# bd4sur/Nano

Hardware: AMD Instinct MI355X
Metric: decode_tokens_per_sec (higher is better)
Workload: dtype i8

## Files before the change

include/nano_mi355x.h:

```cpp
#ifndef NANO_MI355X_H
#define NANO_MI355X_H

#include <stddef.h>
#include <stdint.h>

#ifdef __cplusplus
extern "C" {
#endif

#define NANO_ARCH_NANO  0u
#define NANO_ARCH_QWEN2 2u
#define NANO_ARCH_QWEN3 3u

#define NANO_QUANT_F32 0x00u
#define NANO_QUANT_Q80 0x80u
#define NANO_QUANT_Q4K 0x42u

#define NANO_HIP_OK        0
#define NANO_HIP_EINVAL   -1
#define NANO_HIP_ERUNTIME -2
#define NANO_HIP_ENODEV   -3
#define NANO_HIP_ENOMEM   -4

#define NANO_MAX_BATCH 64u
// ... 117 lines not shown
    uint32_t chunk;
    uint32_t want_frag;
    uint32_t pool_rows;
    uint32_t pt_stride;
    const float *q;
    const float *k;
    const float *vraw;
    const uint32_t *pos;
    const float *q_norm, *k_norm;
    const float *rope_cos, *rope_sin;
    const uint32_t *pt_rows;
    void *k_cache, *v_cache;
    float *out;
    int8_t *xf;
    float *xsf;
    uint32_t *plan;
} NanoAttnDecodeDesc;
int nano_hip_op_attention_decode(int device, const NanoAttnDecodeDesc *d);
int nano_hip_op_swiglu(int device, float *hb, const float *hb2, uint32_t n);
int nano_hip_op_exact_rmsnorm(int device, float *out, const float *x, const float *w, uint32_t n);
typedef struct NanoExactAttnDesc {
    uint32_t n_head, n_kv_head, hd, S;
    uint32_t range;
    uint32_t is_causal;
    uint32_t long_form;
    uint32_t _pad;
    const float *q;
    const float *k_cache, *v_cache;
    float *out;
} NanoExactAttnDesc;
int nano_hip_op_exact_attention(int device, const NanoExactAttnDesc *d);

int nano_hip_op_argmax(int device, const float *x, uint32_t n, uint32_t *idx);

typedef struct NanoFusedGemvDesc {
    uint32_t quant;
    uint32_t gs;
    uint32_t kind;
    uint32_t n, nb, nseg;
    uint32_t rows[3];
    const void *w[3];
    const float *ws[3];
    const float *x;
    const float *norm_w;
    const float *attn_part;
    const float *attn_ml;
    uint32_t attn_nsplit, attn_n_head, attn_hd;
    uint32_t use_gemm;
    uint32_t ordered;
    uint32_t *route_out;
    float *out;
} NanoFusedGemvDesc;
int nano_hip_op_fused_gemv(int device, const NanoFusedGemvDesc *d);

typedef struct NanoBlobShare NanoBlobShare;
int nano_hip_blob_share(NanoBlobShare **out, const void *host_params, size_t bytes, int root_device, const int *devices, int n_devices);
const void *nano_hip_blob_ptr(const NanoBlobShare *s, int i);
void nano_hip_blob_stats(const NanoBlobShare *s, double *upload_s, double *share_s, char *how, size_t how_cap);
void nano_hip_blob_done(NanoBlobShare *s, int i);
void nano_hip_blob_release(NanoBlobShare *s);
int nano_hip_model_device(const NanoHipModel *m);

int nano_hip_stamps_begin(NanoHipModel *m);
int nano_hip_stamps_read(NanoHipModel *m, unsigned long long *out, uint32_t *kinds, uint32_t cap_launches, uint32_t *n_launches);

#ifdef __cplusplus
}
#endif
#endif
```

nano_amd/binding.py:

```python
from __future__ import annotations

import ctypes as C
import os
from typing import Optional, Sequence

import numpy as np

HERE = os.path.dirname(os.path.abspath(__file__))
LIB_PATH = os.environ.get("NANO_LIB") or os.path.join(HERE, "lib", "libnano_mi355x.so")

f32p = np.ctypeslib.ndpointer(dtype=np.float32, flags="C_CONTIGUOUS")
i8p = np.ctypeslib.ndpointer(dtype=np.int8, flags="C_CONTIGUOUS")
u8p = np.ctypeslib.ndpointer(dtype=np.uint8, flags="C_CONTIGUOUS")
u32p = np.ctypeslib.ndpointer(dtype=np.uint32, flags="C_CONTIGUOUS")


class NanoModelDesc(C.Structure):
    _fields_ = [(n, C.c_uint32) for n in (
        "arch", "block_size", "vocab_size", "n_layer", "n_embd", "n_head", "n_kv_head", "n_hidden",
        "is_shared_classifier", "head_dim", "quant_type", "group_size")]


class NanoFusedGemvDesc(C.Structure):
    _fields_ = [("quant", C.c_uint32), ("gs", C.c_uint32), ("kind", C.c_uint32), ("n", C.c_uint32), ("nb", C.c_uint32), ("nseg", C.c_uint32),
# ... 365 lines not shown
    q = np.empty(x.size, np.int8); s = np.empty(x.size // gs, np.float32)
    check(lib().nano_hip_op_quantize_q80(device, x, x.size, gs, q, s)); return q, s


def op_matmul_q80(xq, xs, wq, ws, n, d, gs, device=0):
    out = np.empty(d, np.float32)
    check(lib().nano_hip_op_matmul_q80(device, out, np.ascontiguousarray(xq), np.ascontiguousarray(xs),
                                       np.ascontiguousarray(wq), np.ascontiguousarray(ws), n, d, gs)); return out


def op_quantize_q4k(x, device=0):
    x = np.ascontiguousarray(x, np.float32)
    out = np.zeros(((x.size + 255) // 256) * 160, np.uint8)
    check(lib().nano_hip_op_quantize_q4k(device, x, x.size, out)); return out


def op_matmul_q4k(x_blocks, w_blocks, n, d, device=0):
    out = np.empty(d, np.float32)
    check(lib().nano_hip_op_matmul_q4k(device, out, np.ascontiguousarray(x_blocks), np.ascontiguousarray(w_blocks), n, d)); return out


def op_fused_gemv(quant, kind, n, weights, x=None, norm_w=None, *, gs=0, nb=1, resid=None, attn=None, use_gemm=False, ordered=False,
                  want_route=False, device=0):
    d = NanoFusedGemvDesc()
    d.quant, d.gs, d.kind, d.n, d.nb, d.nseg = quant, gs, kind, n, nb, len(weights)
    keep = []
    for i, (w, ws, rows) in enumerate(weights):
        w = np.ascontiguousarray(w); keep.append(w)
        d.rows[i] = rows; d.w[i] = w.ctypes.data
        if ws is not None:
            ws = np.ascontiguousarray(ws, np.float32); keep.append(ws); d.ws[i] = ws.ctypes.data
    rows_total = weights[0][2] if kind == 2 else sum(r for _, _, r in weights)
    if x is not None:
        x = np.ascontiguousarray(x, np.float32); keep.append(x); d.x = x.ctypes.data
    if norm_w is not None:
        norm_w = np.ascontiguousarray(norm_w, np.float32); keep.append(norm_w); d.norm_w = norm_w.ctypes.data
    if attn is not None:
        part, ml, n_head, hd = attn
        part = np.ascontiguousarray(part, np.float32); ml = np.ascontiguousarray(ml, np.float32); keep += [part, ml]
        d.attn_part, d.attn_ml = part.ctypes.data, ml.ctypes.data
        d.attn_nsplit, d.attn_n_head, d.attn_hd = part.shape[-2], n_head, hd
    out = np.zeros((nb, rows_total), np.float32) if resid is None else np.array(resid, np.float32, copy=True).reshape(nb, rows_total)
    d.use_gemm = 1 if use_gemm else 0
    d.ordered = 1 if ordered else 0
    route = C.c_uint32(0xffffffff)
    d.route_out = C.cast(C.pointer(route), C.c_void_p)
    d.out = out.ctypes.data
    check(lib().nano_hip_op_fused_gemv(device, C.byref(d)))
    if want_route:
        return out, (ROUTE_NAMES[route.value] if route.value < len(ROUTE_NAMES) else "?")
    return out


def op_attention_decode(q, k, pos, k_cache, v_cache, *, n_head, n_kv_head, hd, n_layer, layer, S, range_hint, rope_cos, rope_sin,
                        rope_qwen3, q_norm=None, k_norm=None, vraw=None, kv_half=False, chunk=False, nsplit=0, want_frag=False,
                        pt_rows=None, pool_rows=0, device=0):
    d = NanoAttnDecodeDesc()
    q = np.ascontiguousarray(q, np.float32); k = np.ascontiguousarray(k, np.float32); pos = np.ascontiguousarray(pos, np.uint32)
    nb_ = q.shape[0]
    cdt = np.float16 if kv_half else np.float32
    kc = np.array(k_cache, cdt, copy=True, order="C"); vc = np.array(v_cache, cdt, copy=True, order="C")
    rope_cos = np.ascontiguousarray(rope_cos, np.float32); rope_sin = np.ascontiguousarray(rope_sin, np.float32)
    out = np.zeros((nb_, n_head * hd), np.float32)
    plan = np.zeros((2, len(ATTN_PLAN_FIELDS)), np.uint32)
    keep = [q, k, pos, kc, vc, rope_cos, rope_sin, out, plan]
    d.nb, d.n_head, d.n_kv_head, d.hd, d.n_layer, d.layer, d.S = nb_, n_head, n_kv_head, hd, n_layer, layer, S
    d.range_hint, d.nsplit, d.rope_qwen3, d.kv_half, d.chunk, d.want_frag = range_hint, nsplit, int(rope_qwen3), int(kv_half), int(chunk), int(want_frag)
    d.q, d.k, d.pos, d.k_cache, d.v_cache, d.out, d.plan = (x.ctypes.data for x in (q, k, pos, kc, vc, out, plan))
    d.rope_cos, d.rope_sin = rope_cos.ctypes.data, rope_sin.ctypes.data
    if q_norm is not None:
        q_norm = np.ascontiguousarray(q_norm, np.float32); k_norm = np.ascontiguousarray(k_norm, np.float32); keep += [q_norm, k_norm]
        d.q_norm, d.k_norm = q_norm.ctypes.data, k_norm.ctypes.data
    if vraw is not None:
        vraw = np.ascontiguousarray(vraw, np.float32); keep.append(vraw); d.vraw = vraw.ctypes.data
    if pt_rows is not None:
        pt_rows = np.ascontiguousarray(pt_rows, np.uint32); keep.append(pt_rows)
        d.pt_rows, d.pt_stride, d.pool_rows = pt_rows.ctypes.data, pt_rows.shape[-1], pool_rows
    xf = xsf = None
    if want_frag:
        tiles, ng = (nb_ + 15) // 16, n_head * hd // 64
        xf = np.zeros((tiles, ng, 1024), np.int8); xsf = np.zeros((tiles, ng, 16), np.float32); keep += [xf, xsf]
        d.xf, d.xsf = xf.ctypes.data, xsf.ctypes.data
    check(lib().nano_hip_op_attention_decode(device, C.byref(d)))
    plans = [dict(zip(ATTN_PLAN_FIELDS, (int(v) for v in row))) for row in plan]
    res = {"out": out, "k_cache": kc, "v_cache": vc, "plan": plans if chunk else plans[0]}
    if want_frag:
        res["xf"], res["xsf"] = xf, xsf
    return res


def op_rope(head, fcr, fci, qwen3, device=0):
    h = np.array(head, np.float32, copy=True)
    check(lib().nano_hip_op_rope(device, h, h.size, np.ascontiguousarray(fcr, np.float32), np.ascontiguousarray(fci, np.float32), int(qwen3))); return h


def op_attention(q, k_cache, v_cache, n_head, n_kv_head, head_dim, device=0):
    rng = k_cache.shape[0]
    out = np.empty(n_head * head_dim, np.float32)
    check(lib().nano_hip_op_attention(device, out, np.ascontiguousarray(q, np.float32), np.ascontiguousarray(k_cache, np.float32),
                                      np.ascontiguousarray(v_cache, np.float32), n_head, n_kv_head, head_dim, rng)); return out


def op_exact_rmsnorm(x, w, device=0):
    x = np.ascontiguousarray(x, np.float32); w = np.ascontiguousarray(w, np.float32)
    out = np.empty_like(x)
    check(lib().nano_hip_op_exact_rmsnorm(device, out, x, w, x.size)); return out
# ... 132 lines not shown
```

nano_amd/csrc/gemv_common.h:

```cpp
#pragma once
#define NANO_GEMV_COMMON_H 1
#include <stdlib.h>
#include "device_common.h"
#include "kernels.h"

namespace nano {

namespace {

#define DPP_I(v, ctrl) __builtin_amdgcn_update_dpp(0, (v), (ctrl), 0xF, 0xF, true)
#define DPP_F(v, ctrl) __int_as_float(__builtin_amdgcn_update_dpp(0, __float_as_int(v), (ctrl), 0xF, 0xF, true))

template <int W> __device__ __forceinline__ int dpp_group_sum(int v) {
    if (W >= 2) v += DPP_I(v, 0xB1);
    if (W >= 4) v += DPP_I(v, 0x4E);
    if (W >= 8) v += DPP_I(v, 0x141);
    if (W >= 16) v += DPP_I(v, 0x140);
    return v;
}
template <int W> __device__ __forceinline__ float dpp_group_max(float v) {
    if (W >= 2) v = fmaxf(v, DPP_F(v, 0xB1));
    if (W >= 4) v = fmaxf(v, DPP_F(v, 0x4E));
    if (W >= 8) v = fmaxf(v, DPP_F(v, 0x141));
    if (W >= 16) v = fmaxf(v, DPP_F(v, 0x140));
    if (W >= 32) v = fmaxf(v, __shfl_xor(v, 16, 64));
    if (W >= 64) v = fmaxf(v, __shfl_xor(v, 32, 64));
    return v;
}
__device__ __forceinline__ float dpp_wave_sum(float v) {
    v += DPP_F(v, 0xB1); v += DPP_F(v, 0x4E); v += DPP_F(v, 0x141); v += DPP_F(v, 0x140);
    const float r0 = __int_as_float(__builtin_amdgcn_readlane(__float_as_int(v), 0));
    const float r1 = __int_as_float(__builtin_amdgcn_readlane(__float_as_int(v), 16));
    const float r2 = __int_as_float(__builtin_amdgcn_readlane(__float_as_int(v), 32));
    const float r3 = __int_as_float(__builtin_amdgcn_readlane(__float_as_int(v), 48));
    return (r0 + r1) + (r2 + r3);
}

typedef int i32x4 __attribute__((ext_vector_type(4)));
constexpr uint32_t OOB = 0x7ffffff0u;
__device__ __forceinline__ __amdgpu_buffer_rsrc_t mkrsrc(const void *p, uint32_t bytes) {
    return __builtin_amdgcn_make_buffer_rsrc(const_cast<void *>(p), 0, (int)bytes, 0x00020000);
}
__device__ __forceinline__ int4 bload_w(__amdgpu_buffer_rsrc_t r, uint32_t off) {
    const i32x4 v = __builtin_amdgcn_raw_buffer_load_b128(r, (int)off, 0, 2);
    return make_int4(v.x, v.y, v.z, v.w);
}
__device__ __forceinline__ float4 bload_f4(__amdgpu_buffer_rsrc_t r, uint32_t off) {
    const i32x4 v = __builtin_amdgcn_raw_buffer_load_b128(r, (int)off, 0, 0);
    return make_float4(__int_as_float(v.x), __int_as_float(v.y), __int_as_float(v.z), __int_as_float(v.w));
}
__device__ __forceinline__ float bload_f(__amdgpu_buffer_rsrc_t r, uint32_t off) {
    return __uint_as_float(__builtin_amdgcn_raw_buffer_load_b32(r, (int)off, 0, 0));
}

enum : uint32_t { F_NORM = 1u, F_PRE = 2u, F_COMBINE = 4u };

enum : int { R_GENERIC = 0, R_NORM_STORE = 1, R_RESID = 2, R_RESID_COMBINE = 3, R_NORM_SWIGLU = 4 };
struct GemvDev;
template <int ROLE> __device__ __forceinline__ bool has_flag(const GemvDev &a, uint32_t f);
template <int ROLE> __device__ __forceinline__ uint32_t role_epi(const GemvDev &a);

struct GemvDev {
    const int8_t *w[3]; const float *ws[3]; float *out[3];
    uint32_t rows[3], out_bstride[3], out_pstride[3];
    uint32_t n, ng, rw, log2_tiles, nchunk, magic_nchunk, units, epi, flags, nb;
    uint32_t tpw, magic_rw, wg_c0, wg_c1;
    const float *xin; const float *norm_w; const uint32_t *pos;
    uint32_t xin_bstride, nthr;
    const int8_t *xq_in; const float *xs_in;
    const float *attn_part; const float *attn_ml;
    uint32_t attn_nsplit, attn_n_head, attn_hd, ntiles;
    float *tile_max;
    const float *resid_add; uint32_t resid_add_bstride;
    uint32_t early;
    unsigned long long *stamps;
    uint32_t dbg;
    uint32_t canon;
    uint32_t *err;
};

template <int ROLE> __device__ __forceinline__ bool has_flag(const GemvDev &a, uint32_t f) {
    if (ROLE == R_GENERIC) return (a.flags & f) != 0;
    if (f == F_NORM) return ROLE == R_NORM_STORE || ROLE == R_NORM_SWIGLU;
    if (f == F_COMBINE) return ROLE == R_RESID_COMBINE;
    return false;
}
template <int ROLE> __device__ __forceinline__ uint32_t role_epi(const GemvDev &a) {
    if (ROLE == R_GENERIC) return a.epi;
    if (ROLE == R_NORM_STORE) return GEMV_EPI_STORE;
    if (ROLE == R_NORM_SWIGLU) return GEMV_EPI_SWIGLU;
    return GEMV_EPI_RESID;
}

template <int B, int NV>
struct Staged {
    float4 x[B][NV];
    float4 nw[NV];
    float4 pv[B == 1 ? NV : 1][B == 1 ? 8 : 1];
    float ml_m, ml_l;
};
template <int B>
struct Staged<B, 0> {};

template <int ROLE, int B, int NV>
__device__ __forceinline__ void stage_issue(const GemvDev &a, Staged<B, NV> &r) {
    if constexpr (NV == 0) { (void)a; (void)r; return; } else {
    const uint32_t tid = threadIdx.x, nthr = a.nthr, n = a.n;
    const bool plain = !has_flag<ROLE>(a, F_PRE) && !has_flag<ROLE>(a, F_COMBINE);
    const __amdgpu_buffer_rsrc_t rx = mkrsrc(a.xin, plain ? ((a.nb - 1) * a.xin_bstride + n) * 4u : 0u);
    const __amdgpu_buffer_rsrc_t rn = mkrsrc(a.norm_w, has_flag<ROLE>(a, F_NORM) ? n * 4u : 0u);
#pragma unroll
    for (int j = 0; j < NV; j++) {
        const uint32_t i = (tid + (uint32_t)j * nthr) * 4u;
        const uint32_t off = (i < n) ? i * 4u : OOB;
        if (plain) {
#pragma unroll
            for (int b = 0; b < B; b++) r.x[b][j] = bload_f4(rx, (b < (int)a.nb) ? off + (uint32_t)b * a.xin_bstride * 4u : OOB);
        }
        if (has_flag<ROLE>(a, F_NORM)) r.nw[j] = (NANO_STAMPS && (a.dbg & 1u)) ? make_float4(1.f, 1.f, 1.f, 1.f) : bload_f4(rn, off);
    }
    if constexpr (B == 1) {
      if (has_flag<ROLE>(a, F_COMBINE)) {
        const uint32_t ns = a.attn_nsplit, nh = a.attn_n_head;
        const __amdgpu_buffer_rsrc_t rp = mkrsrc(a.attn_part, ns * n * 4u);
        const __amdgpu_buffer_rsrc_t rm = mkrsrc(a.attn_ml, nh * ns * 8u);
#pragma unroll
        for (int j = 0; j < NV; j++) {
            const uint32_t i = (tid + (uint32_t)j * nthr) * 4u;
#pragma unroll
            for (int sp = 0; sp < 8; sp++) r.pv[j][sp] = bload_f4(rp, (i < n && (uint32_t)sp < ns) ? ((uint32_t)sp * n + i) * 4u : OOB);
        }
        const uint32_t sp = tid & 7u, h = tid >> 3;
        const uint32_t mo = (h < nh && sp < ns) ? (h * ns + sp) * 8u : OOB;
        r.ml_m = bload_f(rm, mo);
        r.ml_l = bload_f(rm, mo == OOB ? OOB : mo + 4u);
      }
    }
    }
}

template <int ROLE, int B, int NV>
__device__ __forceinline__ void stage_issue_nw(const GemvDev &a, Staged<B, NV> &r) {
    if constexpr (NV == 0) { (void)a; (void)r; return; } else {
    const uint32_t tid = threadIdx.x, nthr = a.nthr, n = a.n;
    const __amdgpu_buffer_rsrc_t rn = mkrsrc(a.norm_w, has_flag<ROLE>(a, F_NORM) ? n * 4u : 0u);
#pragma unroll
    for (int j = 0; j < NV; j++) {
        const uint32_t i = (tid + (uint32_t)j * nthr) * 4u;
        if (has_flag<ROLE>(a, F_NORM)) r.nw[j] = bload_f4(rn, (i < n) ? i * 4u : OOB);
    }
    }
}

template <int B, bool PRE>
__device__ __forceinline__ void combine_weights(const GemvDev &a, float *wgt , float pm, float pl) {
    const uint32_t tid = threadIdx.x, nthr = a.nthr;
    const uint32_t ns = a.attn_nsplit, nh = a.attn_n_head;
    for (uint32_t t = tid; t < (uint32_t)B * nh * 8u; t += nthr) {
        const uint32_t s = t & 7u, h = (t >> 3) % nh, b = (t >> 3) / nh;
        float m = -INFINITY, l = 0.0f;
        if constexpr (PRE) { m = pm; l = pl; (void)s; (void)h; (void)b; (void)ns; }
        else if (s < ns && b < a.nb) { const float *ml = a.attn_ml + (((size_t)b * nh + h) * ns + s) * 2; m = ml[0]; l = ml[1]; }
        const bool live = l > 0.0f;
        float M = live ? m : -INFINITY;
        M = fmaxf(M, DPP_F(M, 0xB1)); M = fmaxf(M, DPP_F(M, 0x4E)); M = fmaxf(M, DPP_F(M, 0x141));
        const float e = live ? expf(m - M) : 0.0f;
        float L = l * e;
        L += DPP_F(L, 0xB1); L += DPP_F(L, 0x4E); L += DPP_F(L, 0x141);
        wgt[t] = e / L;
        if constexpr (PRE) break;
    }
    __syncthreads();
}
__device__ __forceinline__ float4 combine4(const GemvDev &a, uint32_t b, uint32_t i, const float *wgt) {
    const uint32_t ns = a.attn_nsplit, n = a.n;
    const float *part = a.attn_part + (size_t)b * ns * n + i;
    const float *wg = wgt + ((size_t)b * a.attn_n_head + i / a.attn_hd) * 8u;
    float4 o[8];
#pragma unroll
    for (int s = 0; s < 8; s++) o[s] = ((uint32_t)s < ns) ? *reinterpret_cast<const float4 *>(part + (size_t)s * n) : make_float4(0.f, 0.f, 0.f, 0.f);
    float4 acc = make_float4(0.f, 0.f, 0.f, 0.f);
#pragma unroll
    for (int s = 0; s < 8; s++) {
        const float w = wg[s];
        acc.x += o[s].x * w; acc.y += o[s].y * w; acc.z += o[s].z * w; acc.w += o[s].w * w;
    }
    return acc;
}

__device__ __forceinline__ float finish_epi(uint32_t epi, float v0, float v1, float old) {
    if (epi == GEMV_EPI_STORE) return v0;
    if (epi == GEMV_EPI_RESID) return old + v0;
    float h = v0;
    h *= (1.0f / (1.0f + expf(-h)));
    h *= v1;
    return h;
}

static GemvDev to_dev(const GemvArgs &a) {
    GemvDev d{};
    for (int i = 0; i < 3; i++) {
        const bool live = i < (int)a.nseg;
        d.w[i] = live ? reinterpret_cast<const int8_t *>(a.seg[i].w) : nullptr;
        d.ws[i] = live ? a.seg[i].ws : nullptr;
        d.out[i] = live ? a.seg[i].out : nullptr;
        d.rows[i] = live ? a.seg[i].rows : 0;
        d.out_bstride[i] = live ? a.seg[i].out_bstride : 0;
        d.out_pstride[i] = live ? a.seg[i].out_pstride : 0;
    }
    if (a.epi == GEMV_EPI_SWIGLU) { d.rows[1] = 0; d.rows[2] = 0; }
    d.n = a.n; d.ng = a.gs ? a.n / a.gs : 0;
    d.nchunk = (a.n + 1023) / 1024;
    d.magic_nchunk = (65536 + d.nchunk - 1) / d.nchunk;
    d.epi = a.epi; d.nb = a.nb;
    d.flags = (a.norm_w ? F_NORM : 0) | (a.xq_in ? F_PRE : 0) | (a.attn_part ? F_COMBINE : 0);
    d.xin = a.xin; d.norm_w = a.norm_w; d.pos = a.pos; d.xin_bstride = a.xin_bstride;
    d.xq_in = a.xq_in; d.xs_in = a.xs_in;
    d.attn_part = a.attn_part; d.attn_ml = a.attn_ml; d.attn_nsplit = a.attn_nsplit; d.attn_n_head = a.attn_n_head; d.attn_hd = a.attn_hd;
    d.tile_max = a.tile_max;
    d.resid_add = a.resid_add; d.resid_add_bstride = a.resid_add_bstride;
    d.stamps = a.stamps;
    d.canon = q80_canonical(a) ? 1u : 0u;
    d.err = a.err;
#if NANO_STAMPS
    { static const uint32_t dbg = getenv("NANO_DBG") ? (uint32_t)strtoul(getenv("NANO_DBG"), nullptr, 0) : 0u; d.dbg = dbg; }
#endif
    return d;
}

}

}
```

nano_amd/csrc/gemv_f32.hip:

```cpp
#include "gemv_common.h"

namespace nano {

namespace {

template <int ROLE, int B, int NV>
__device__ __forceinline__ void stage_finish_f32(const GemvDev &a, Staged<B, NV> &r, float *xf, float *red, uint32_t n4) {
    const uint32_t tid = threadIdx.x, nthr = a.nthr, n = a.n;
    const uint32_t lane = tid & 63u, wid = tid >> 6, NW = nthr >> 6;
    const bool norm = has_flag<ROLE>(a, F_NORM), comb = has_flag<ROLE>(a, F_COMBINE);
    float *wgt = red + B * 16;
    if constexpr (NV == 0) {
        if (comb) combine_weights<B, false>(a, wgt, 0.0f, 0.0f);
        for (uint32_t b = 0; b < a.nb; b++) {
            const float *x = a.xin + (size_t)b * a.xin_bstride;
            float ss = 1.0f;
            if (norm) {
                float acc = 0.0f;
                for (uint32_t i = tid * 4u; i < n; i += nthr * 4u) {
                    const float4 v = comb ? combine4(a, b, i, wgt) : *reinterpret_cast<const float4 *>(x + i);
                    acc += v.x * v.x; acc += v.y * v.y; acc += v.z * v.z; acc += v.w * v.w;
                }
                acc = dpp_wave_sum(acc);
                __syncthreads();
                if (lane == 0) red[wid] = acc;
                __syncthreads();
                float t = 0.0f;
                for (uint32_t w = 0; w < NW; w++) t += red[w];
                t /= (float)n; t += 1e-5f;
                ss = 1.0f / sqrtf(t);
            }
            for (uint32_t i = tid * 4u; i < n; i += nthr * 4u) {
                float4 v = comb ? combine4(a, b, i, wgt) : *reinterpret_cast<const float4 *>(x + i);
                if (norm) {
                    const float4 w = *reinterpret_cast<const float4 *>(a.norm_w + i);
                    v.x = w.x * (ss * v.x); v.y = w.y * (ss * v.y); v.z = w.z * (ss * v.z); v.w = w.w * (ss * v.w);
                }
                *reinterpret_cast<float4 *>(xf + b * n4 + i) = v;
            }
        }
        __syncthreads();
    } else {
        if (comb) {
            if constexpr (B == 1) {
                const bool pre_ml = a.attn_n_head * 8u <= nthr;
                if (pre_ml) combine_weights<B, true>(a, wgt, r.ml_m, r.ml_l); else combine_weights<B, false>(a, wgt, 0.0f, 0.0f);
#pragma unroll
                for (int j = 0; j < NV; j++) {
                    const uint32_t i = (tid + (uint32_t)j * nthr) * 4u;
                    const float *wg = wgt + (size_t)((i < n ? i : 0u) / a.attn_hd) * 8u;
                    float4 acc = make_float4(0.f, 0.f, 0.f, 0.f);
#pragma unroll
                    for (int sp = 0; sp < 8; sp++) {
                        const float w = wg[sp];
                        acc.x += r.pv[j][sp].x * w; acc.y += r.pv[j][sp].y * w; acc.z += r.pv[j][sp].z * w; acc.w += r.pv[j][sp].w * w;
                    }
                    r.x[0][j] = acc;
                }
            } else {
                combine_weights<B, false>(a, wgt, 0.0f, 0.0f);
#pragma unroll
                for (int b = 0; b < B; b++)
#pragma unroll
                    for (int j = 0; j < NV; j++) {
                        const uint32_t i = (tid + (uint32_t)j * nthr) * 4u;
                        r.x[b][j] = (i < n && b < (int)a.nb) ? combine4(a, b, i, wgt) : make_float4(0.f, 0.f, 0.f, 0.f);
                    }
            }
        }
        float ss[B];
#pragma unroll
        for (int b = 0; b < B; b++) ss[b] = 1.0f;
        if (norm) {
#pragma unroll
            for (int b = 0; b < B; b++) {
                float acc = 0.0f;
#pragma unroll
                for (int j = 0; j < NV; j++) {
                    acc += r.x[b][j].x * r.x[b][j].x; acc += r.x[b][j].y * r.x[b][j].y;
                    acc += r.x[b][j].z * r.x[b][j].z; acc += r.x[b][j].w * r.x[b][j].w;
                }
                acc = dpp_wave_sum(acc);
                if (lane == 0) red[b * 16 + wid] = acc;
            }
            __syncthreads();
#pragma unroll
            for (int b = 0; b < B; b++) {
                float t = 0.0f;
                for (uint32_t w = 0; w < NW; w++) t += red[b * 16 + w];
                t /= (float)n; t += 1e-5f;
                ss[b] = 1.0f / sqrtf(t);
            }
        }
#pragma unroll
        for (int j = 0; j < NV; j++) {
            const uint32_t i = (tid + (uint32_t)j * nthr) * 4u;
#pragma unroll
            for (int b = 0; b < B; b++) {
                float4 v = r.x[b][j];
                if (norm) {
                    v.x = r.nw[j].x * (ss[b] * v.x); v.y = r.nw[j].y * (ss[b] * v.y);
                    v.z = r.nw[j].z * (ss[b] * v.z); v.w = r.nw[j].w * (ss[b] * v.w);
                }
                if (i < n) *reinterpret_cast<float4 *>(xf + b * n4 + i) = v;
            }
        }
        __syncthreads();
    }
}

__device__ __forceinline__ float4 bload_wf(__amdgpu_buffer_rsrc_t r, uint32_t off) {
    const i32x4 v = __builtin_amdgcn_raw_buffer_load_b128(r, (int)off, 0, 2);
    return make_float4(__int_as_float(v.x), __int_as_float(v.y), __int_as_float(v.z), __int_as_float(v.w));
}

template <int ROLE, int B, int NV, int UPW>
__global__ __launch_bounds__(1024) void gemv_f32_slab_kernel(const GemvDev a) {
    extern __shared__ __attribute__((aligned(16))) unsigned char smem[];
#define F32_A a
// ... 55 lines not shown
    if (want > 16) want = 16;
    if (nw < want) nw = want;
    if (nw * 64 < rw * (uint32_t)B) nw = (rw * (uint32_t)B + 63) / 64;
    if (nw < 2) nw = 2;
    uint32_t upw = (units + nw - 1) / nw;
    while (upw > 4 && nw < 16) { nw++; upw = (units + nw - 1) / nw; }
    return F32Plan{rw, nw, upw, (a.n + 256 * nw - 1) / (256 * nw)};
}

template <int ROLE, int B, int NV, int UPW>
static hipError_t launch_f32_t(const GemvDev &d, const F32Plan &p, uint32_t rows, hipStream_t st) {
    const uint32_t nmat = d.epi == GEMV_EPI_SWIGLU ? 2 : 1;
    const size_t n4 = (d.n + 3) & ~3u, pc = (d.nchunk + 3) & ~3u;
    const size_t lds = (B * n4 + B * 16 + ((d.flags & F_COMBINE) ? (size_t)B * d.attn_n_head * 8 : 0) + (size_t)B * nmat * p.rw * pc) * 4;
    auto kern = &gemv_f32_slab_kernel<ROLE, B, NV, UPW>;
    if (lds > 64 * 1024) (void)hipFuncSetAttribute(reinterpret_cast<const void *>(kern), hipFuncAttributeMaxDynamicSharedMemorySize, (int)lds);
    GemvDev dd = d; dd.nthr = 64 * p.nw;
    hipLaunchKernelGGL(kern, dim3((rows + p.rw - 1) / p.rw), dim3(64 * p.nw), lds, st, dd);
    return hipGetLastError();
}
template <int ROLE, int B>
static hipError_t launch_f32_r(const GemvDev &d, const F32Plan &p, uint32_t rows, hipStream_t st) {
    if (p.upw > 4) return hipErrorInvalidValue;
#define F32_GO(NV_, UPW_) do { if constexpr (B * NV_ <= 8) return launch_f32_t<ROLE, B, NV_, UPW_>(d, p, rows, st); } while (0)
    int nv = p.nv <= 1 ? 1 : p.nv <= 2 ? 2 : p.nv <= 4 ? 4 : 0;
    const int upw = p.upw <= 1 ? 1 : p.upw <= 2 ? 2 : 4;
    if (B * nv > 8) nv = 0;
    if (nv == 1) { if (upw == 1) F32_GO(1, 1); if (upw == 2) F32_GO(1, 2); F32_GO(1, 4); }
    if (nv == 2) { if (upw == 1) F32_GO(2, 1); if (upw == 2) F32_GO(2, 2); F32_GO(2, 4); }
    if (nv == 4) { if (upw == 1) F32_GO(4, 1); if (upw == 2) F32_GO(4, 2); F32_GO(4, 4); }
    if (upw == 1) F32_GO(0, 1);
    if (upw == 2) F32_GO(0, 2);
    F32_GO(0, 4);
    return hipErrorInvalidValue;
#undef F32_GO
}
template <int B>
static hipError_t launch_f32_b(const GemvArgs &a, hipStream_t st) {
    GemvDev d = to_dev(a);
    d.tile_max = nullptr;
    const F32Plan p = plan_f32(a, B);
    d.nchunk = (a.n + 255) / 256;
    d.magic_nchunk = (65536 + d.nchunk - 1) / d.nchunk;
    d.rw = p.rw;
    uint32_t l2 = 0; while ((1u << l2) < p.rw / 4) l2++;
    d.log2_tiles = l2;
    d.units = (p.rw / 4) * d.nchunk * (d.epi == GEMV_EPI_SWIGLU ? 2 : 1);
    uint32_t rows = 0;
    if (a.epi == GEMV_EPI_SWIGLU) rows = a.seg[0].rows; else for (uint32_t s = 0; s < a.nseg; s++) rows += a.seg[s].rows;
    if constexpr (B == 1) {
        const uint32_t f = d.flags;
        if (f == F_NORM && d.epi == GEMV_EPI_STORE) return launch_f32_r<R_NORM_STORE, B>(d, p, rows, st);
        if (f == 0 && d.epi == GEMV_EPI_RESID) return launch_f32_r<R_RESID, B>(d, p, rows, st);
        if (f == F_COMBINE && d.epi == GEMV_EPI_RESID) return launch_f32_r<R_RESID_COMBINE, B>(d, p, rows, st);
        if (f == F_NORM && d.epi == GEMV_EPI_SWIGLU) return launch_f32_r<R_NORM_SWIGLU, B>(d, p, rows, st);
    }
    return launch_f32_r<R_GENERIC, B>(d, p, rows, st);
}

static bool f32_fused_shape(const GemvArgs &ga, const AttnArgs &aa, F32Plan &p) {
    if (ga.nb != 1 || ga.nseg != 3 || ga.epi != GEMV_EPI_STORE || !ga.norm_w || ga.xq_in || ga.attn_part || ga.tile_max || ga.resid_add || ga.n % 4u) return false;
    if (ga.seg[0].out_pstride || ga.seg[1].out_pstride) return false;
    for (uint32_t s2 = 0; s2 < 3; s2++) if (ga.seg[s2].rows % 4u) return false;
    p = plan_f32(ga, 1);
    if (p.nw > 4u || p.upw > 4u || ga.n > 1024u) return false;
    p.nw = 4u; p.nv = 1u;
    const uint32_t units = (p.rw / 4) * ((ga.n + 255) / 256);
    p.upw = (units + 3u) / 4u;
    if (p.upw > 4u) return false;
    return fused_attn_side_ok_plain(aa, ga.seg[0].rows, ga.seg[1].rows, ga.seg[2].rows);
}

}

bool qkv_attn_fused_f32_supports(const GemvArgs &ga, const AttnArgs &aa) { F32Plan p; return f32_fused_shape(ga, aa, p); }

hipError_t launch_qkv_attn_fused_f32(const GemvArgs &ga, const AttnArgs &aa, unsigned long long *hand, uint32_t *tick, uint32_t layer1, hipStream_t st) {
    F32Plan p;
    if (!hand || !tick || !layer1 || layer1 > 127u || !f32_fused_shape(ga, aa, p)) return hipErrorInvalidValue;
    GemvDev d = to_dev(ga);
    d.tile_max = nullptr;
    d.nchunk = (ga.n + 255) / 256;
    d.magic_nchunk = (65536 + d.nchunk - 1) / d.nchunk;
    d.rw = p.rw;
    uint32_t l2 = 0; while ((1u << l2) < p.rw / 4) l2++;
    d.log2_tiles = l2;
    d.units = (p.rw / 4) * d.nchunk;
    d.nthr = 256;
    uint32_t rows = 0;
    for (uint32_t s2 = 0; s2 < 3; s2++) rows += ga.seg[s2].rows;
    const uint32_t ngemv = (rows + p.rw - 1) / p.rw;
    AttnArgs a = aa;
    { uint32_t k2 = 0; while ((1u << k2) < a.n_kv_head) k2++; a.kv_log2 = k2; }
    { const uint32_t kv_mul = a.n_head / a.n_kv_head; uint32_t k2 = 0; while ((1u << k2) < kv_mul) k2++; a.kvmul_log2 = k2; }
    SlabHand h{};
    h.buf = hand; h.tick = tick; h.layer1 = layer1;
    h.base[0] = 0; h.base[1] = a.q_dim; h.base[2] = a.q_dim + a.kv_dim;
    const size_t n4 = (d.n + 3) & ~3u, pc = (d.nchunk + 3) & ~3u;
    const size_t lds_g = (n4 + 16 + (size_t)p.rw * pc) * 4;
    const size_t hd4 = (a.hd + 3) & ~3u, lds_a = (hd4 + hd4 + 4 + 4 + 4 * hd4 + hd4) * sizeof(float);
    const size_t lds = lds_g > lds_a ? lds_g : lds_a;
    if (lds > 64 * 1024) return hipErrorInvalidValue;
    F32FusedArgs fa{};
    fa.g = d; fa.a = a; fa.hand = h; fa.n_attn = a.n_head * a.nsplit; fa.head_wgs = a.n_head; fa.ngemv = ngemv;
    fa.wait16 = 1u;
    const int upw = p.upw <= 1 ? 1 : p.upw <= 2 ? 2 : 4;
#define F32F_GO(UPW_) do { if (a.hd <= 32u) hipLaunchKernelGGL((f32_qkv_attn_fused_kernel<1, UPW_, 1>), dim3(fa.n_attn + ngemv), dim3(256), lds, st, fa); \
// ... 20 lines not shown
```

nano_amd/csrc/gemv_q4k.hip:

```cpp
#include <float.h>

#include "gemv_q4k_impl.h"

namespace nano {

__global__ __launch_bounds__(256) void quantize_q4k_kernel(const float *x, uint32_t n, uint8_t *blocks) {
    __shared__ float tmp[16];
    __shared__ uint8_t nibs[256];
    const int t = threadIdx.x;
    const uint32_t bpl = (n + 255) / 256;
    for (uint32_t j = 0; j < bpl; j++) {
        const uint32_t d = (n >= (j + 1) * 256) ? 256 : (n - j * 256);
        const bool valid = (uint32_t)t < d;
        const float v = valid ? x[(size_t)j * d + t] : 0.0f;
        Q4kBlockHdr hdr; float sq, bq;
        const uint32_t nib = q4k_quantize_block_coop(v, valid, tmp, hdr, sq, bq);
        nibs[t] = (uint8_t)nib;
        __syncthreads();
        uint8_t *blk = blocks + (size_t)j * 160;
        if (t < 128) blk[32 + t] = (uint8_t)((nibs[2 * t] & 0x0f) | (nibs[2 * t + 1] << 4));
        if (t == 0) {
            uint32_t *w = reinterpret_cast<uint32_t *>(blk);
            w[0] = 0x42u; w[1] = d; w[2] = 0u;
            w[3] = __float_as_uint(hdr.s_scale); w[4] = __float_as_uint(hdr.s_bias);
// ... 211 lines not shown
    if (lds > 64 * 1024) (void)hipFuncSetAttribute(reinterpret_cast<const void *>(kern), hipFuncAttributeMaxDynamicSharedMemorySize, (int)lds);
    GemvDev dd = d; dd.nthr = p.nthr;
    { const uint32_t GT = ((d.n + 255) / 256) * 8; dd.magic_nchunk = (uint32_t)(((1ull << 32) + GT - 1) / GT); dd.log2_tiles = 0; while ((1u << dd.log2_tiles) < p.rw) dd.log2_tiles++;
      dd.units = ((p.rw * GT) % 64u == 0u && p.nthr % 64u == 0u) ? 1u : 0u; }
    hipLaunchKernelGGL(kern, dim3((rows + p.rw - 1) / p.rw), dim3(p.nthr), lds, st, dd);
    return hipGetLastError();
}
template <int ROLE, int B>
static hipError_t launch_q4k_r(const GemvDev &d, const Q4kPlan &p, uint32_t rows, hipStream_t st) {
    if (p.ipt > 4) return hipErrorInvalidValue;
#define Q4K_GO(NV_, IPT_) do { if constexpr (B * NV_ <= 8) return launch_q4k_t<ROLE, B, NV_, IPT_>(d, p, rows, st); } while (0)
    int nv = p.nv <= 1 ? 1 : p.nv <= 2 ? 2 : p.nv <= 4 ? 4 : 0;
    const int ipt = p.ipt <= 1 ? 1 : p.ipt <= 2 ? 2 : 4;
    if (B * nv > 8) nv = 0;
    if (nv == 1) { if (ipt == 1) Q4K_GO(1, 1); if (ipt == 2) Q4K_GO(1, 2); Q4K_GO(1, 4); }
    if (nv == 2) { if (ipt == 1) Q4K_GO(2, 1); if (ipt == 2) Q4K_GO(2, 2); Q4K_GO(2, 4); }
    if (nv == 4) { if (ipt == 1) Q4K_GO(4, 1); if (ipt == 2) Q4K_GO(4, 2); Q4K_GO(4, 4); }
    if (ipt == 1) Q4K_GO(0, 1);
    if (ipt == 2) Q4K_GO(0, 2);
    Q4K_GO(0, 4);
    return hipErrorInvalidValue;
#undef Q4K_GO
}
}
bool gemv_q4k_chunk_takes(const GemvArgs &a) {
    if (a.nb <= 1) return gemv_q4k_chunk_supports(a);
    if (a.nb > 8 || !gemv_q4k_chunk_supports(a)) return false;
    return a.nb >= 5u || route_is_wide(a) || gemv_q4k_fit_batch(a) < a.nb;
}

uint32_t gemv_q4k_partials(const GemvArgs &a) {
    if (a.nb == 1 && gemv_q4k_chunk_supports(a)) return gemv_q4k_chunk_partials(a);
    if (a.nb > 1 && gemv_q4k_chunk_takes(a)) return 0;
    if (!a.tile_max || a.epi != GEMV_EPI_STORE || a.nseg != 1 || a.nb == 0 || a.nb > 8 || a.seg[0].out_pstride) return 0;
    const int B = a.nb <= 1 ? 1 : a.nb <= 2 ? 2 : a.nb <= 4 ? 4 : 8;
    const Q4kPlan p = plan_q4k(a, B);
    return (a.seg[0].rows + p.rw - 1) / p.rw;
}
namespace {
template <int B>
static hipError_t launch_q4k_b(const GemvArgs &a, hipStream_t st) {
    GemvDev d = to_dev(a);
    if (a.x4_in) { d.flags |= F_PRE; d.xq_in = reinterpret_cast<const int8_t *>(a.x4_in); }
    const Q4kPlan p = plan_q4k(a, B);
    d.rw = p.rw;
    uint32_t rows = 0;
    if (a.epi == GEMV_EPI_SWIGLU) rows = a.seg[0].rows; else for (uint32_t s = 0; s < a.nseg; s++) rows += a.seg[s].rows;
    d.ntiles = gemv_q4k_partials(a);
    if (!d.ntiles || d.ntiles != (rows + p.rw - 1) / p.rw) { d.tile_max = nullptr; d.ntiles = 0; }
    if constexpr (B == 1) {
        const uint32_t f = d.flags;
        if (f == F_NORM && d.epi == GEMV_EPI_STORE) return launch_q4k_r<R_NORM_STORE, B>(d, p, rows, st);
        if (f == 0 && d.epi == GEMV_EPI_RESID) return launch_q4k_r<R_RESID, B>(d, p, rows, st);
        if (f == F_COMBINE && d.epi == GEMV_EPI_RESID) return launch_q4k_r<R_RESID_COMBINE, B>(d, p, rows, st);
        const uint32_t GT = ((d.n + 255) / 256) * 8;
        if (f == F_NORM && d.epi == GEMV_EPI_SWIGLU && (p.rw * GT) % 64u == 0u && p.nthr % 64u == 0u) return launch_q4k_r<R_NORM_SWIGLU, B>(d, p, rows, st);
    }
    return launch_q4k_r<R_GENERIC, B>(d, p, rows, st);
}

}

uint32_t gemv_q4k_fit_batch(const GemvArgs &a) {
    for (uint32_t c = 8; c > 1; c >>= 1)
        if (q4k_lds_bytes(a.n, a.epi, a.attn_part != nullptr, a.attn_n_head, plan_q4k(a, (int)c).rw, c) <= 160 * 1024) return c;
    return 1;
}

hipError_t launch_gemv_q4k(GemvArgs &a, uint32_t max_wg, hipStream_t st) {
    (void)max_wg;
    if (a.nb >= 1 && a.nb <= 8 && gemv_q4k_chunk_takes(a)) return launch_gemv_q4k_chunk(a, st);
    if (a.nb == 0 || a.nb > 8 || a.n % 4 || a.nseg == 0 || a.nseg > 3) return hipErrorInvalidValue;
    if (a.attn_part && (a.norm_w || a.attn_nsplit > 8 || a.attn_hd % 4)) return hipErrorInvalidValue;
    if (a.epi != GEMV_EPI_SWIGLU && a.nseg > 1)
        for (uint32_t s = 0; s < a.nseg; s++) if (a.seg[s].rows % 4) return hipErrorInvalidValue;
    if (a.nb <= 1) return launch_q4k_b<1>(a, st);
    if (a.nb <= 2) return launch_q4k_b<2>(a, st);
    if (a.nb <= 4) return launch_q4k_b<4>(a, st);
    return launch_q4k_b<8>(a, st);
}

}
```

nano_amd/csrc/gemv_q4k_chunk.hip:

```cpp
#include "gemv_q4k_impl.h"
#include <hip/hip_ext.h>

namespace nano {

extern hipEvent_t g_q80_probe_start, g_q80_probe_stop;

namespace {

template <int ROLE, int NV, int D, bool LOOP, int NB = 1>
__global__ __launch_bounds__(1024) void gemv_q4k_chunk_kernel(const GemvDev a) {
    static_assert(NB == 1 || (ROLE == R_GENERIC && NV == 1), "several sequences: activations arrive quantized (q4k_quant_rows_kernel), generic role");
    extern __shared__ __attribute__((aligned(16))) unsigned char smem[];
#define CHUNK_A a
#define CHUNK_BID blockIdx.x
#define CHUNK_HAND 0
#define CHUNK_HANDV (SlabHand{})
#define CHUNK_PTAG 0u
#include "gemv_q4k_chunk_body.inc"
#undef CHUNK_A
#undef CHUNK_BID
#undef CHUNK_HAND
#undef CHUNK_HANDV
#undef CHUNK_PTAG
}
// ... 108 lines not shown
}

template <int ROLE, int NV, int D, bool LOOP>
hipError_t launch_chunk_t(const GemvDev &d, const ChunkPlan &p, hipStream_t st) {
    auto kern = &gemv_q4k_chunk_kernel<ROLE, NV, D, LOOP>;
    if (p.lds > 64 * 1024) (void)hipFuncSetAttribute(reinterpret_cast<const void *>(kern), hipFuncAttributeMaxDynamicSharedMemorySize, (int)p.lds);
    hipEvent_t e0 = LOOP ? g_q80_probe_start : nullptr, e1 = LOOP ? g_q80_probe_stop : nullptr;
    if (e0 && e1) {
        g_q80_probe_start = g_q80_probe_stop = nullptr;
        hipExtLaunchKernelGGL(kern, dim3(p.grid), dim3(p.nthr), (uint32_t)p.lds, st, e0, e1, 0, d);
    } else hipLaunchKernelGGL(kern, dim3(p.grid), dim3(p.nthr), p.lds, st, d);
    return hipGetLastError();
}
template <int ROLE, int NV>
hipError_t launch_chunk_d(const GemvDev &d, const ChunkPlan &p, hipStream_t st) {
    if (p.loop) return launch_chunk_t<ROLE, NV, 8, true>(d, p, st);
    if (p.d == 1) return launch_chunk_t<ROLE, NV, 1, false>(d, p, st);
    if (p.d == 2) return launch_chunk_t<ROLE, NV, 2, false>(d, p, st);
    if (p.d == 4) return launch_chunk_t<ROLE, NV, 4, false>(d, p, st);
    return launch_chunk_t<ROLE, NV, 8, false>(d, p, st);
}
template <int ROLE>
hipError_t launch_chunk_r(const GemvDev &d, const ChunkPlan &p, hipStream_t st) {
    if (p.nv <= 1) return launch_chunk_d<ROLE, 1>(d, p, st);
    if (p.nv <= 2) return launch_chunk_d<ROLE, 2>(d, p, st);
    return launch_chunk_d<ROLE, 4>(d, p, st);
}
template <int D, bool LOOP, int NB>
hipError_t launch_chunk_nb_t(const GemvDev &d, const ChunkPlan &p, hipStream_t st) {
    auto kern = &gemv_q4k_chunk_kernel<R_GENERIC, 1, D, LOOP, NB>;
    if (p.lds > 64 * 1024) (void)hipFuncSetAttribute(reinterpret_cast<const void *>(kern), hipFuncAttributeMaxDynamicSharedMemorySize, (int)p.lds);
    hipLaunchKernelGGL(kern, dim3(p.grid), dim3(p.nthr), p.lds, st, d);
    return hipGetLastError();
}
template <int NB>
hipError_t launch_chunk_nb(const GemvDev &d, const ChunkPlan &p, hipStream_t st) {
    if (p.loop) return launch_chunk_nb_t<8, true, NB>(d, p, st);
    if (p.d == 1) return launch_chunk_nb_t<1, false, NB>(d, p, st);
    if (p.d == 2) return launch_chunk_nb_t<2, false, NB>(d, p, st);
    if (p.d == 4) return launch_chunk_nb_t<4, false, NB>(d, p, st);
    return launch_chunk_nb_t<8, false, NB>(d, p, st);
}
template <int ROLE, int NV>
hipError_t launch_quant_rows_t(const GemvDev &d, XGroup *out, uint32_t nb, size_t lds, hipStream_t st) {
    auto kern = &q4k_quant_rows_kernel<ROLE, NV>;
    if (lds > 64 * 1024) (void)hipFuncSetAttribute(reinterpret_cast<const void *>(kern), hipFuncAttributeMaxDynamicSharedMemorySize, (int)lds);
    hipLaunchKernelGGL(kern, dim3(nb), dim3(d.nthr), lds, st, d, out);
    return hipGetLastError();
}
template <int NV>
hipError_t launch_quant_rows_r(const GemvDev &d, XGroup *out, uint32_t nb, size_t lds, hipStream_t st) {
    if (d.flags == F_NORM) return launch_quant_rows_t<R_NORM_STORE, NV>(d, out, nb, lds, st);
    if (d.flags == 0) return launch_quant_rows_t<R_RESID, NV>(d, out, nb, lds, st);
    if (d.flags == F_COMBINE) return launch_quant_rows_t<R_RESID_COMBINE, NV>(d, out, nb, lds, st);
    return launch_quant_rows_t<R_GENERIC, NV>(d, out, nb, lds, st);
}

}

bool gemv_q4k_chunk_supports(const GemvArgs &a) {
    ChunkPlan p;
    if (a.nb <= 1) return plan_chunk(a, p);
    GemvArgs one = a; one.nb = 1;
    return a.q4_scratch && (size_t)a.nb * (a.n >> 5) * sizeof(XGroup) <= a.q4_scratch_bytes && plan_chunk(one, p) && plan_chunk(a, p);
}
bool gemv_q4k_chunk_loops(const GemvArgs &a) { ChunkPlan p; return a.nb == 1 && plan_chunk(a, p) && p.loop; }
uint32_t gemv_q4k_chunk_partials(const GemvArgs &a) {
    ChunkPlan p;
    if (a.nb != 1 || !a.tile_max || a.epi != GEMV_EPI_STORE || a.nseg != 1 || a.seg[0].out_pstride || !plan_chunk(a, p)) return 0;
    return p.grid;
}

static hipError_t launch_gemv_q4k_chunk_batched(GemvArgs &a, hipStream_t st) {
    if (!gemv_q4k_chunk_supports(a)) return hipErrorInvalidValue;
    ChunkPlan p1, p;
    GemvArgs one = a; one.nb = 1;
    if (!plan_chunk(one, p1) || !plan_chunk(a, p)) return hipErrorInvalidValue;
    const uint32_t bpl = a.n >> 8, GT = bpl * 8u;
    XGroup *xg = reinterpret_cast<XGroup *>(a.q4_scratch);
    {
        GemvDev q = to_dev(a);
        q.nthr = p1.nthr; q.tile_max = nullptr;
        const size_t lds = (size_t)GT * sizeof(XGroup) + (16 + (a.attn_part ? (size_t)a.attn_n_head * 8 : 0)) * 4 + 16;
        const hipError_t e = p1.nv <= 1 ? launch_quant_rows_r<1>(q, xg, a.nb, lds, st) : p1.nv <= 2 ? launch_quant_rows_r<2>(q, xg, a.nb, lds, st) : launch_quant_rows_r<4>(q, xg, a.nb, lds, st);
        if (e != hipSuccess) return e;
    }
    GemvArgs g = a;
    g.norm_w = nullptr; g.attn_part = nullptr; g.attn_ml = nullptr; g.tile_max = nullptr;
    GemvDev d = to_dev(g);
    d.flags = F_PRE; d.xq_in = reinterpret_cast<const int8_t *>(xg);
    d.rw = p.rw; d.nthr = p.nthr; d.units = p.rounds;
    d.magic_nchunk = (uint32_t)(((1ull << 32) + bpl - 1) / bpl);
    const uint32_t nseg = a.epi == GEMV_EPI_SWIGLU ? 1u : a.nseg;
    d.wg_c0 = nseg > 1 ? p.wg[0] : 0xffffffffu;
    d.wg_c1 = nseg > 2 ? p.wg[0] + p.wg[1] : 0xffffffffu;
    d.ntiles = 0;
    if (a.nb <= 2) return launch_chunk_nb<2>(d, p, st);
    if (a.nb <= 4) return launch_chunk_nb<4>(d, p, st);
    return launch_chunk_nb<8>(d, p, st);
}

static bool q4k_fused_shape(const GemvArgs &ga, const AttnArgs &aa, ChunkPlan &p) {
    if (ga.nb != 1 || ga.nseg != 3 || ga.epi != GEMV_EPI_STORE || !ga.norm_w || ga.xq_in || ga.x4_in || ga.attn_part || ga.tile_max || ga.resid_add) return false;
    if (ga.seg[0].out_pstride || ga.seg[1].out_pstride) return false;
    if (ga.n > 1024u || !plan_chunk(ga, p, 4u) || p.loop || p.nthr != 256u || p.nv != 1u) return false;
    if (p.lds > 64u * 1024u) return false;
    return fused_attn_side_ok(aa, ga.seg[0].rows, ga.seg[1].rows, ga.seg[2].rows);
}
bool qkv_attn_fused_q4k_supports(const GemvArgs &ga, const AttnArgs &aa) { ChunkPlan p; return q4k_fused_shape(ga, aa, p); }

hipError_t launch_qkv_attn_fused_q4k(const GemvArgs &ga, const AttnArgs &aa, unsigned long long *hand, uint32_t *tick, uint32_t layer1, hipStream_t st) {
    ChunkPlan p;
    if (!hand || !tick || !layer1 || layer1 > 127u || !q4k_fused_shape(ga, aa, p)) return hipErrorInvalidValue;
    GemvDev d = to_dev(ga);
    d.tile_max = nullptr; d.ntiles = 0;
    const uint32_t bpl = ga.n >> 8;
    d.rw = p.rw; d.nthr = p.nthr; d.units = p.rounds;
    d.magic_nchunk = (uint32_t)(((1ull << 32) + bpl - 1) / bpl);
    d.wg_c0 = p.wg[0]; d.wg_c1 = p.wg[0] + p.wg[1];
    AttnArgs a = aa;
    { uint32_t l2 = 0; while ((1u << l2) < a.n_kv_head) l2++; a.kv_log2 = l2; }
    { const uint32_t kv_mul = a.n_head / a.n_kv_head; uint32_t l2 = 0; while ((1u << l2) < kv_mul) l2++; a.kvmul_log2 = l2; }
    SlabHand h{};
    h.buf = hand; h.tick = tick; h.layer1 = layer1;
    h.base[0] = 0; h.base[1] = a.q_dim; h.base[2] = a.q_dim + a.kv_dim;
    const size_t hd4 = a.hd, lds_a = (hd4 + hd4 + 4 + 4 + 4 * hd4 + hd4 + 4 + 4 * 8 * hd4) * sizeof(float);
    const size_t lds = p.lds > lds_a ? p.lds : lds_a;
    Q4FusedArgs fa{};
    fa.g = d; fa.a = a; fa.hand = h; fa.n_attn = a.n_head * a.nsplit; fa.head_wgs = a.n_head; fa.ngemv = p.grid;
    fa.wait16 = 0u;
#define Q4F_GO(NV_, D_) do { hipLaunchKernelGGL((q4k_qkv_attn_fused_kernel<NV_, D_>), dim3(fa.n_attn + fa.ngemv), dim3(p.nthr), lds, st, fa); return hipGetLastError(); } while (0)
#define Q4F_NV(NV_) do { if (p.d == 1) Q4F_GO(NV_, 1); if (p.d == 2) Q4F_GO(NV_, 2); if (p.d == 4) Q4F_GO(NV_, 4); Q4F_GO(NV_, 8); } while (0)
    if (p.nv <= 1) Q4F_NV(1);
    if (p.nv <= 2) Q4F_NV(2);
    Q4F_NV(4);
#undef Q4F_NV
#undef Q4F_GO
}

hipError_t launch_gemv_q4k_chunk(GemvArgs &a, hipStream_t st) {
    if (a.nb > 1) return launch_gemv_q4k_chunk_batched(a, st);
    ChunkPlan p;
    if (!plan_chunk(a, p)) return hipErrorInvalidValue;
    GemvDev d = to_dev(a);
    if (a.x4_in) { d.flags |= F_PRE; d.xq_in = reinterpret_cast<const int8_t *>(a.x4_in); }
    const uint32_t bpl = a.n >> 8;
    d.rw = p.rw; d.nthr = p.nthr; d.units = p.rounds;
    d.magic_nchunk = (uint32_t)(((1ull << 32) + bpl - 1) / bpl);
    const uint32_t nseg = a.epi == GEMV_EPI_SWIGLU ? 1u : a.nseg;
    d.wg_c0 = nseg > 1 ? p.wg[0] : 0xffffffffu;
    d.wg_c1 = nseg > 2 ? p.wg[0] + p.wg[1] : 0xffffffffu;
    d.ntiles = gemv_q4k_chunk_partials(a);
    if (!d.ntiles) d.tile_max = nullptr;
    const uint32_t f = d.flags;
    if (f == F_NORM && d.epi == GEMV_EPI_STORE) return launch_chunk_r<R_NORM_STORE>(d, p, st);
    if (f == 0 && d.epi == GEMV_EPI_RESID) return launch_chunk_r<R_RESID>(d, p, st);
    if (f == F_COMBINE && d.epi == GEMV_EPI_RESID) return launch_chunk_r<R_RESID_COMBINE>(d, p, st);
    if (f == F_NORM && d.epi == GEMV_EPI_SWIGLU) return launch_chunk_r<R_NORM_SWIGLU>(d, p, st);
    return launch_chunk_r<R_GENERIC>(d, p, st);
}

}
```

nano_amd/csrc/gemv_q4k_impl.h:

```cpp
#pragma once
#include <float.h>

#include "gemv_common.h"

namespace nano {

typedef unsigned int u32x2_q __attribute__((ext_vector_type(2)));

struct XGroup {
    uint32_t pk[4];
    float sq, bq;
    int sumq;
    int _pad;
};

struct Q4kBlockHdr { float s_scale, s_bias; uint32_t sb[3]; };

__device__ __forceinline__ uint32_t q4k_quantize_block_coop(float v, bool valid, float *tmp ,
                                                            Q4kBlockHdr &hdr, float &sq_f, float &bq_f) {
    const int t = threadIdx.x, g = t >> 5;
    float lo = valid ? v : FLT_MAX;
    float hi = valid ? v : FLT_TRUE_MIN;
    lo = (lo < FLT_MAX) ? lo : FLT_MAX;
    hi = (hi > FLT_TRUE_MIN) ? hi : FLT_TRUE_MIN;
    for (int o = 16; o > 0; o >>= 1) {
        lo = fminf(lo, __shfl_xor(lo, o, 64));
        hi = fmaxf(hi, __shfl_xor(hi, o, 64));
    }
    const float gsc = (lo <= 0.0f) ? div_const<15>(hi - lo) : div_const<15>(hi);
    const float gbi = (lo <= 0.0f) ? (-lo) : 0.0f;
    uint32_t nib = 0;
    if (valid && gsc != 0.0f) nib = (uint32_t)(nearest_int_magic((v + gbi) / gsc) & 0x0f);
    __syncthreads();
    if ((t & 31) == 0) { tmp[g] = gsc; tmp[8 + g] = gbi; }
    __syncthreads();
    float smax = FLT_TRUE_MIN, bmax = FLT_TRUE_MIN;
#pragma unroll
    for (int k = 0; k < 8; k++) { if (tmp[k] > smax) smax = tmp[k]; if (tmp[8 + k] > bmax) bmax = tmp[8 + k]; }
    const float s_scale = div_const<63>(smax), s_bias = div_const<63>(bmax);
    uint32_t s6[8], b6[8];
#pragma unroll
    for (int k = 0; k < 8; k++) {
        s6[k] = (s_scale == 0.0f) ? 0u : (uint32_t)(nearest_int_magic(tmp[k] / s_scale) & 0x3f);
        b6[k] = (s_bias == 0.0f) ? 0u : (uint32_t)(nearest_int_magic(tmp[8 + k] / s_bias) & 0x3f);
    }
    hdr.s_scale = s_scale; hdr.s_bias = s_bias;
    hdr.sb[0] = hdr.sb[1] = hdr.sb[2] = 0;
#pragma unroll
    for (int i = 0; i < 4; i++) {
        hdr.sb[0] |= ((((s6[4 + i] & 0x30) << 2) | (s6[i] & 0x3f)) & 0xffu) << (8 * i);
        hdr.sb[1] |= ((((b6[4 + i] & 0x30) << 2) | (b6[i] & 0x3f)) & 0xffu) << (8 * i);
        hdr.sb[2] |= ((((b6[4 + i] & 0x0f) << 4) | (s6[4 + i] & 0x0f)) & 0xffu) << (8 * i);
    }
    sq_f = (float)s6[g] * s_scale;
    bq_f = (float)b6[g] * s_bias;
    return nib;
}

namespace {

template <int ROLE, int B, int NV>
__device__ __forceinline__ void stage_xn(const GemvDev &a, Staged<B, NV> &r, float *xn, float *red, uint32_t n4, bool keep) {
    const uint32_t tid = threadIdx.x, nthr = a.nthr, n = a.n;
    const uint32_t lane = tid & 63u, wid = tid >> 6, NW = nthr >> 6;
    const bool norm = has_flag<ROLE>(a, F_NORM), comb = has_flag<ROLE>(a, F_COMBINE);
    float *wgt = red + B * 16;
    if constexpr (NV == 0) {
        if (comb) combine_weights<B, false>(a, wgt, 0.0f, 0.0f);
        for (uint32_t b = 0; b < a.nb; b++) {
            const float *x = a.xin + (size_t)b * a.xin_bstride;
            float ss = 1.0f;
            if (norm) {
                float acc = 0.0f;
                for (uint32_t i = tid * 4u; i < n; i += nthr * 4u) {
                    const float4 v = comb ? combine4(a, b, i, wgt) : *reinterpret_cast<const float4 *>(x + i);
                    acc += v.x * v.x; acc += v.y * v.y; acc += v.z * v.z; acc += v.w * v.w;
                }
                acc = dpp_wave_sum(acc);
                __syncthreads();
                if (lane == 0) red[wid] = acc;
                __syncthreads();
                float t = 0.0f;
                for (uint32_t w = 0; w < NW; w++) t += red[w];
                t /= (float)n; t += 1e-5f;
                ss = 1.0f / sqrtf(t);
            }
            for (uint32_t i = tid * 4u; i < n; i += nthr * 4u) {
                float4 v = comb ? combine4(a, b, i, wgt) : *reinterpret_cast<const float4 *>(x + i);
                if (norm) {
                    const float4 w = *reinterpret_cast<const float4 *>(a.norm_w + i);
                    v.x = w.x * (ss * v.x); v.y = w.y * (ss * v.y); v.z = w.z * (ss * v.z); v.w = w.w * (ss * v.w);
                }
                *reinterpret_cast<float4 *>(xn + b * n4 + i) = v;
            }
        }
        __syncthreads();
    } else {
        if (comb) {
            if constexpr (B == 1) {
                const bool pre_ml = a.attn_n_head * 8u <= nthr;
                if (pre_ml) combine_weights<B, true>(a, wgt, r.ml_m, r.ml_l); else combine_weights<B, false>(a, wgt, 0.0f, 0.0f);
#pragma unroll
                for (int j = 0; j < NV; j++) {
                    const uint32_t i = (tid + (uint32_t)j * nthr) * 4u;
                    const float *wg = wgt + (size_t)((i < n ? i : 0u) / a.attn_hd) * 8u;
                    float4 acc = make_float4(0.f, 0.f, 0.f, 0.f);
#pragma unroll
                    for (int sp = 0; sp < 8; sp++) {
                        const float w = wg[sp];
                        acc.x += r.pv[j][sp].x * w; acc.y += r.pv[j][sp].y * w; acc.z += r.pv[j][sp].z * w; acc.w += r.pv[j][sp].w * w;
                    }
                    r.x[0][j] = acc;
                }
            } else {
                combine_weights<B, false>(a, wgt, 0.0f, 0.0f);
#pragma unroll
                for (int b = 0; b < B; b++)
#pragma unroll
                    for (int j = 0; j < NV; j++) {
                        const uint32_t i = (tid + (uint32_t)j * nthr) * 4u;
                        r.x[b][j] = (i < n && b < (int)a.nb) ? combine4(a, b, i, wgt) : make_float4(0.f, 0.f, 0.f, 0.f);
                    }
            }
        }
        float ss[B];
#pragma unroll
        for (int b = 0; b < B; b++) ss[b] = 1.0f;
        if (norm) {
#pragma unroll
            for (int b = 0; b < B; b++) {
                float acc = 0.0f;
#pragma unroll
                for (int j = 0; j < NV; j++) {
                    acc += r.x[b][j].x * r.x[b][j].x; acc += r.x[b][j].y * r.x[b][j].y;
                    acc += r.x[b][j].z * r.x[b][j].z; acc += r.x[b][j].w * r.x[b][j].w;
                }
                acc = dpp_wave_sum(acc);
                if (lane == 0) red[b * 16 + wid] = acc;
            }
            __syncthreads();
#pragma unroll
            for (int b = 0; b < B; b++) {
                float t = 0.0f;
                for (uint32_t w = 0; w < NW; w++) t += red[b * 16 + w];
                t /= (float)n; t += 1e-5f;
                ss[b] = 1.0f / sqrtf(t);
            }
        }
#pragma unroll
        for (int j = 0; j < NV; j++) {
            const uint32_t i = (tid + (uint32_t)j * nthr) * 4u;
#pragma unroll
            for (int b = 0; b < B; b++) {
                float4 v = r.x[b][j];
                if (norm) {
                    v.x = r.nw[j].x * (ss[b] * v.x); v.y = r.nw[j].y * (ss[b] * v.y);
                    v.z = r.nw[j].z * (ss[b] * v.z); v.w = r.nw[j].w * (ss[b] * v.w);
                }
                if (keep) r.x[b][j] = v;
                else if (i < n) *reinterpret_cast<float4 *>(xn + b * n4 + i) = v;
            }
        }
        if (!keep) __syncthreads();
    }
}

template <int B, int NV, bool SYNC = true>
__device__ __forceinline__ void quantize_q4k_regs(const GemvDev &a, const Staged<B, NV> &r, XGroup *xg) {
    if constexpr (NV == 0) { (void)a; (void)r; (void)xg; } else {
    const uint32_t tid = threadIdx.x, nthr = a.nthr, n = a.n, GT = (n >> 8) * 8u;
#pragma unroll
    for (int j = 0; j < NV; j++) {
        const uint32_t i = (tid + (uint32_t)j * nthr) * 4u;
        const bool valid = i < n;
// ... 135 lines not shown
```

nano_amd/csrc/gemv_q80_impl.h:

```cpp
#include <string.h>
#include <stdio.h>
#include "gemv_common.h"
#include "gemv_q80_host.h"

namespace nano {

namespace {


__device__ __forceinline__ void quant_store4(float4 v, float scale, int8_t *dst) {
    const int q0 = q80_quant1(v.x, scale), q1 = q80_quant1(v.y, scale), q2 = q80_quant1(v.z, scale), q3 = q80_quant1(v.w, scale);
    *reinterpret_cast<uint32_t *>(dst) = (uint32_t)(q0 & 0xff) | ((uint32_t)(q1 & 0xff) << 8) | ((uint32_t)(q2 & 0xff) << 16) | ((uint32_t)(q3 & 0xff) << 24);
}

template <int ROLE, int GS, int B, int NV>
__device__ __forceinline__ void stage_finish(const GemvDev &a, Staged<B, NV> &r, int8_t *xq, float *xs, float *red, uint32_t n16, uint32_t ng4) {
    const uint32_t tid = threadIdx.x, nthr = a.nthr, n = a.n, ng = a.ng;
    const uint32_t lane = tid & 63u, wid = tid >> 6, NW = nthr >> 6;
    if (has_flag<ROLE>(a, F_PRE)) {
        for (uint32_t b = 0; b < a.nb; b++) {
            for (uint32_t i = tid * 16u; i < n; i += nthr * 16u) *reinterpret_cast<int4 *>(xq + b * n16 + i) = *reinterpret_cast<const int4 *>(a.xq_in + (size_t)b * n16 + i);
            for (uint32_t i = tid; i < ng; i += nthr) xs[b * ng4 + i] = a.xs_in[(size_t)b * ng + i];
        }
        __syncthreads();
        return;
    }
    const bool norm = has_flag<ROLE>(a, F_NORM), comb = has_flag<ROLE>(a, F_COMBINE);
    float *wgt = red + B * 16;
    if constexpr (NV == 0) {
        if (comb) combine_weights<B, false>(a, wgt, 0.0f, 0.0f);
        for (uint32_t b = 0; b < a.nb; b++) {
            const float *x = a.xin + (size_t)b * a.xin_bstride;
            float ss = 1.0f;
            if (norm) {
                float acc = 0.0f;
                for (uint32_t i = tid * 4u; i < n; i += nthr * 4u) {
                    const float4 v = comb ? combine4(a, b, i, wgt) : *reinterpret_cast<const float4 *>(x + i);
                    acc += v.x * v.x; acc += v.y * v.y; acc += v.z * v.z; acc += v.w * v.w;
                }
                acc = dpp_wave_sum(acc);
                __syncthreads();
                if (lane == 0) red[wid] = acc;
                __syncthreads();
                float t = 0.0f;
                for (uint32_t w = 0; w < NW; w++) t += red[w];
                t /= (float)n; t += 1e-5f;
                ss = 1.0f / sqrtf(t);
            }
            for (uint32_t i = tid * 4u; i < n; i += nthr * 4u) {
                float4 v = comb ? combine4(a, b, i, wgt) : *reinterpret_cast<const float4 *>(x + i);
                if (norm) {
                    const float4 w = *reinterpret_cast<const float4 *>(a.norm_w + i);
                    v.x = w.x * (ss * v.x); v.y = w.y * (ss * v.y); v.z = w.z * (ss * v.z); v.w = w.w * (ss * v.w);
                }
                float m = fmaxf(fmaxf(fabsf(v.x), fabsf(v.y)), fmaxf(fabsf(v.z), fabsf(v.w)));
                m = dpp_group_max<GS / 4>(m);
                const float scale = div_const<127>(m);
                quant_store4(v, scale, xq + b * n16 + i);
                if ((tid % (GS / 4)) == 0) xs[b * ng4 + i / GS] = scale;
            }
        }
        __syncthreads();
    } else {
        if (comb) {
            if constexpr (B == 1) {
                const bool pre_ml = a.attn_n_head * 8u <= nthr;
                if (pre_ml) combine_weights<B, true>(a, wgt, r.ml_m, r.ml_l); else combine_weights<B, false>(a, wgt, 0.0f, 0.0f);
#pragma unroll
                for (int j = 0; j < NV; j++) {
                    const uint32_t i = (tid + (uint32_t)j * nthr) * 4u;
                    const float *wg = wgt + (size_t)((i < n ? i : 0u) / a.attn_hd) * 8u;
                    float4 acc = make_float4(0.f, 0.f, 0.f, 0.f);
#pragma unroll
                    for (int sp = 0; sp < 8; sp++) {
                        const float w = wg[sp];
                        acc.x += r.pv[j][sp].x * w; acc.y += r.pv[j][sp].y * w; acc.z += r.pv[j][sp].z * w; acc.w += r.pv[j][sp].w * w;
                    }
                    r.x[0][j] = acc;
                }
            } else {
                combine_weights<B, false>(a, wgt, 0.0f, 0.0f);
#pragma unroll
                for (int b = 0; b < B; b++)
#pragma unroll
                    for (int j = 0; j < NV; j++) {
                        const uint32_t i = (tid + (uint32_t)j * nthr) * 4u;
                        r.x[b][j] = (i < n && b < (int)a.nb) ? combine4(a, b, i, wgt) : make_float4(0.f, 0.f, 0.f, 0.f);
                    }
            }
        }
        float ss[B];
#pragma unroll
        for (int b = 0; b < B; b++) ss[b] = 1.0f;
        if (norm) {
#pragma unroll
            for (int b = 0; b < B; b++) {
                float acc = 0.0f;
#pragma unroll
                for (int j = 0; j < NV; j++) {
                    acc += r.x[b][j].x * r.x[b][j].x; acc += r.x[b][j].y * r.x[b][j].y;
                    acc += r.x[b][j].z * r.x[b][j].z; acc += r.x[b][j].w * r.x[b][j].w;
                }
                acc = dpp_wave_sum(acc);
                if (lane == 0) red[b * 16 + wid] = acc;
            }
            __syncthreads();
#pragma unroll
            for (int b = 0; b < B; b++) {
                float t = 0.0f;
                for (uint32_t w = 0; w < NW; w++) t += red[b * 16 + w];
                t /= (float)n; t += 1e-5f;
                ss[b] = 1.0f / sqrtf(t);
            }
        }
        NANO_STAMP(a.stamps, 2, ss[0] + r.x[0][0].x);
#pragma unroll
        for (int j = 0; j < NV; j++) {
            const uint32_t i = (tid + (uint32_t)j * nthr) * 4u;
#pragma unroll
            for (int b = 0; b < B; b++) {
                float4 v = r.x[b][j];
                if (norm) {
                    v.x = r.nw[j].x * (ss[b] * v.x); v.y = r.nw[j].y * (ss[b] * v.y);
                    v.z = r.nw[j].z * (ss[b] * v.z); v.w = r.nw[j].w * (ss[b] * v.w);
                }
                float m = fmaxf(fmaxf(fabsf(v.x), fabsf(v.y)), fmaxf(fabsf(v.z), fabsf(v.w)));
                m = dpp_group_max<GS / 4>(m);
                const float scale = div_const<127>(m);
                if (i < n) {
                    quant_store4(v, scale, xq + b * n16 + i);
                    if ((tid % (GS / 4)) == 0) xs[b * ng4 + i / GS] = scale;
                }
            }
        }
        __syncthreads();
    }
}


template <int NQ> __device__ __forceinline__ float fold_row(const float *p) {
// ... 50 lines not shown
}
__device__ __forceinline__ float fold_row_canon_any(const float *p, uint32_t ng) {
    float v = 0.0f;
    for (uint32_t g0 = 0; g0 < ng; g0 += 16) {
        float4 t[4];
#pragma unroll
        for (int q = 0; q < 4; q++) t[q] = (g0 + 4u * (uint32_t)q < ng) ? *reinterpret_cast<const float4 *>(p + g0 + 4 * q) : make_float4(0.f, 0.f, 0.f, 0.f);
        float s = t[0].x; s += t[0].y; s += t[0].z; s += t[0].w;
        if (g0 + 4 < ng) { s += t[1].x; s += t[1].y; s += t[1].z; s += t[1].w; }
        v = g0 == 0 ? s : v + s;
        if (g0 + 8 < ng) {
            s = t[2].x; s += t[2].y; s += t[2].z; s += t[2].w;
            if (g0 + 12 < ng) { s += t[3].x; s += t[3].y; s += t[3].z; s += t[3].w; }
            v += s;
        }
    }
    return v;
}
template <int NQ> __device__ __forceinline__ void fold_row2_canon(const float *p0, const float *p1, float &v0, float &v1) {
    static_assert(NQ % 2 == 0, "whole units");
    float4 t[NQ], u[NQ];
#pragma unroll
    for (int q = 0; q < NQ; q++) { t[q] = *reinterpret_cast<const float4 *>(p0 + 4 * q); u[q] = *reinterpret_cast<const float4 *>(p1 + 4 * q); }
    __builtin_amdgcn_sched_barrier(0);
    float s0[NQ / 2], s1[NQ / 2];
    unit_sums<NQ / 2>(t, s0); unit_sums<NQ / 2>(u, s1);
    v0 = s0[0]; v1 = s1[0];
#pragma unroll
    for (int k = 1; k < NQ / 2; k++) { v0 = fadd(v0, s0[k]); v1 = fadd(v1, s1[k]); }
}
__device__ __forceinline__ void fold_row2_canon_ng(const float *p0, const float *p1, uint32_t ng, float &v0, float &v1) {
    if (ng == 16u) { fold_row2_canon<4>(p0, p1, v0, v1); return; }
    v0 = fold_row_canon_any(p0, ng); v1 = fold_row_canon_any(p1, ng);
}
__device__ __forceinline__ float fold_row_canon_ng(const float *p, uint32_t ng) {
    if (ng == 16u) return fold_row_canon<4>(p);
    if (ng == 32u) return fold_row_canon<8>(p);
    if (ng == 48u) return fold_row_canon<12>(p);
    return fold_row_canon_any(p, ng);
}

__device__ __forceinline__ float wave_fold_canon16(float p) {
    const float p1 = DPP_F(p, 0x104), p2 = DPP_F(p, 0x108), p3 = DPP_F(p, 0x10C);
    float s = fadd(p, p1); s = fadd(s, p2); s = fadd(s, p3);
    const uint32_t sb = __float_as_uint(s);
    const float c = __uint_as_float(__builtin_amdgcn_permlane16_swap(sb, sb, false, false)[0]);
    s = fadd(c, p); s = fadd(s, p1); s = fadd(s, p2); s = fadd(s, p3);
    const uint32_t tb = __float_as_uint(s);
    const float s0 = __uint_as_float(__builtin_amdgcn_permlane32_swap(tb, tb, false, false)[0]);
    return fadd(s0, s);
}
constexpr int WF_LANE0 = 48;

template <int ROLE, int GS, int B, int NV, int UPW, int EARLY = 0, int WF = 0>
__global__ __launch_bounds__(1024) void gemv_q80_slab_kernel(const GemvDev a) {
    extern __shared__ __attribute__((aligned(16))) unsigned char smem[];
#define SLAB_EARLY EARLY
#define SLAB_WF WF
#define SLAB_A a
#define SLAB_BID blockIdx.x
#define SLAB_HAND 0
#define SLAB_HANDV (SlabHand{})
#define SLAB_PTAG 0u
#define SLAB_XHAND 0
#define SLAB_XHANDV (SlabHand{})
#define SLAB_CTAG 0u
#define SLAB_PART 0
#include "gemv_q80_slab_body.inc"
#undef SLAB_A
#undef SLAB_BID
#undef SLAB_HAND
#undef SLAB_HANDV
#undef SLAB_PTAG
#undef SLAB_XHAND
#undef SLAB_XHANDV
#undef SLAB_CTAG
#undef SLAB_PART
#undef SLAB_EARLY
#undef SLAB_WF
}

#if NANO_Q80_GS == 64
}
}
#include "attn_impl.h"
namespace nano {
namespace {
struct FusedArgs { GemvDev g; AttnArgs a; SlabHand hand; uint32_t n_attn, head_wgs, wait16, ngemv; };
template <int NV, int UPW>
__global__ __launch_bounds__(256) void qkv_attn_fused_kernel(const FusedArgs fa) {
#define SLAB_WF 0
#include "qkv_attn_fused_body.inc"
#undef SLAB_WF
}
template <int NV, int UPW>
__global__ __launch_bounds__(256) void qkv_attn_fused_wf_kernel(const FusedArgs fa) {
#define SLAB_WF 1
#include "qkv_attn_fused_body.inc"
#undef SLAB_WF
}

struct Wo13Args { GemvDev wo; GemvDev w13; SlabHand hand; uint32_t wo_wgs, wait16; };
template <int ROLE_A, int NV_A, int UPW_A, int NV_B, int UPW_B, int NT, int WF = 0>
__global__ __launch_bounds__(NT) void wo_w13_fused_kernel(const Wo13Args fa) {
    extern __shared__ __attribute__((aligned(16))) unsigned char smem[];
    constexpr int GS = 64, B = 1;
    const uint2 tk_ = hand_tick(fa.hand);
    {
        constexpr int ROLE = ROLE_A, NV = NV_A, UPW = UPW_A;
#define SLAB_BID blockIdx.x
#define SLAB_A fa.wo
#define SLAB_HAND 1
#define SLAB_HANDV fa.hand
#define SLAB_PTAG hand_ptag(tk_, fa.hand)
#define SLAB_XHAND 0
#define SLAB_XHANDV (SlabHand{})
#define SLAB_CTAG 0u
#define SLAB_PART 1
#include "gemv_q80_slab_body.inc"
#undef SLAB_PART
        auto wo_rest = [&]() __attribute__((always_inline)) {
#define SLAB_PART 2
#include "gemv_q80_slab_body.inc"
#undef SLAB_PART
        };
#undef SLAB_A
#undef SLAB_HAND
#undef SLAB_HANDV
#undef SLAB_PTAG
#undef SLAB_XHAND
#undef SLAB_XHANDV
#undef SLAB_CTAG
        {
            constexpr int ROLE = R_NORM_SWIGLU, NV = NV_B, UPW = UPW_B;
#define SLAB_A fa.w13
#define SLAB_HAND 0
#define SLAB_HANDV (SlabHand{})
#define SLAB_PTAG 0u
#define SLAB_XHAND 1
#define SLAB_XHANDV fa.hand
#define SLAB_CTAG hand_ctag(tk_, fa.hand)
#define SLAB_XHAND_WAIT (blockIdx.x >= fa.wo_wgs ? fa.wait16 : 0u)
#define SLAB_XHAND_NAP 2
#define SLAB_WF WF
#define SLAB_PART 1
#include "gemv_q80_slab_body.inc"
#undef SLAB_PART
            if (blockIdx.x < fa.wo_wgs) wo_rest();
            __syncthreads();
#define SLAB_PART 2
#include "gemv_q80_slab_body.inc"
#undef SLAB_PART
#undef SLAB_A
#undef SLAB_HAND
#undef SLAB_HANDV
#undef SLAB_PTAG
#undef SLAB_XHAND
#undef SLAB_XHANDV
#undef SLAB_CTAG
#undef SLAB_XHAND_WAIT
#undef SLAB_XHAND_NAP
#undef SLAB_WF
        }
#undef SLAB_BID
    }
}

#endif

template <int ROLE, int GS, int B, int NV>
__global__ __launch_bounds__(256) void gemv_q80_stream_kernel(const GemvDev a) {
    extern __shared__ __attribute__((aligned(16))) unsigned char smem[];
    constexpr int LPG = GS / 16, GC = 1024 / GS, F = GC / 4;
    static_assert(F >= 1, "group size too large for the stream kernel");
    const uint32_t n = a.n, ng = a.ng;
    const int tid = threadIdx.x, lane = tid & 63;
    const int wid = __builtin_amdgcn_readfirstlane(tid >> 6);
    const uint32_t n16 = (n + 15) & ~15u, ng4 = (ng + 3) & ~3u;
// ... 121 lines not shown
    if (nseg > 1) for (uint32_t s = 0; s < nseg; s++) align |= a.seg[s].rows;
    const uint32_t rows = total_rows(a);
    uint32_t rw = 4;
    while (rw < 32 && (align % (rw * 2)) == 0 && (rw * 2 / 4) * nchunk <= 4 && rows / (rw * 2) >= 128) rw *= 2;
    while (rw < 64 && (align % (rw * 2)) == 0 && rows / (rw * 2) >= 256) rw *= 2;
    {
        const uint32_t ng = a.n / a.gs, pitch = ((ng + 47) / 64) * 64 + 16;
        while (rw > 4 && (size_t)B * nmat * rw * pitch * 4 > 64 * 1024) rw /= 2;
        while (rw > 4 && (rw / 4) * nchunk * nmat > 64) rw /= 2;
    }
    if (B == 1 && nseg == 1) {
        const uint32_t cus = a.cus ? a.cus : 256u, c = (rows + cus - 1) / cus;
        if (c >= 5 && c < rw && rows / rw < cus && ((c + 3) / 4) * nchunk * nmat <= 64) rw = c;
    }
    uint32_t large_nw = 0;
    if (B <= 2 && (uint64_t)rows * a.n * nmat >= (8u << 20)) {
        const uint32_t cus = a.cus ? a.cus : 256u;
        uint32_t best = 0, best_cost = ~0u;
        const uint32_t ng = a.n / a.gs, pitch = (1024 / a.gs == 16) ? (((ng + 47) / 64) * 64 + 16) : (((ng + 3) & ~3u) + 4);
        for (uint32_t c = 4; c <= 64; c++) {
            const uint32_t tpw = (c + 3) / 4;
            if (tpw * nchunk * nmat > 64) break;
            if ((size_t)B * nmat * tpw * 4 * pitch * 4 > 96 * 1024) break;
            uint32_t wgs = 0;
            if (nseg > 1) for (uint32_t s2 = 0; s2 < nseg; s2++) wgs += (a.seg[s2].rows + c - 1) / c; else wgs = (rows + c - 1) / c;
            uint32_t cost = ((wgs + cus - 1) / cus) * c * 100u;
            if (wgs > cus) cost += cost * 15u / 100u;
            if (cost <= best_cost) { best_cost = cost; best = c; }
        }
        if (best) {
            rw = best;
            const uint32_t u = ((rw + 3) / 4) * nchunk * nmat;
            large_nw = u / 2 < 8 ? 8 : (u / 2 > 16 ? 16 : u / 2);
        }
    }
    const uint32_t units = ((rw + 3) / 4) * nchunk * nmat;
    uint32_t nw = units < 4 ? units : 4;
    const uint32_t want_div = B == 1 ? 384u : 512u;
    uint32_t want = (a.n * (uint32_t)(B > 2 ? B / 2 : 1) + want_div - 1) / want_div;
    if (want > 16) want = 16;
    if (nw < want) nw = want;
    if (nw * 64 < rw * (uint32_t)B) nw = (rw * (uint32_t)B + 63) / 64;
    if (nw < 2) nw = 2;
    uint32_t upw = (units + nw - 1) / nw;
    while (upw > 4 && nw < 16) { nw++; upw = (units + nw - 1) / nw; }
    if (large_nw) { nw = large_nw; upw = (units + nw - 1) / nw; while (upw > 4 && nw < 16) { nw++; upw = (units + nw - 1) / nw; } }
    SlabPlan p{rw, nw, upw, (a.n + 256 * nw - 1) / (256 * nw)};
    return p;
}

static bool slab_wave_fold(const GemvDev &d) {
    return d.n == 1024u && d.ng == 16u && !d.early && (d.epi == GEMV_EPI_STORE || (d.epi == GEMV_EPI_SWIGLU && !d.out_pstride[0]));
}
template <int ROLE, int GS, int B, int NV, int UPW>
static hipError_t launch_slab_t(const GemvDev &d, const SlabPlan &p, uint32_t nwg, hipStream_t st) {
    const uint32_t nmat = d.epi == GEMV_EPI_SWIGLU ? 2 : 1;
    const size_t n16 = (d.n + 15) & ~15u, ng4 = (d.ng + 3) & ~3u;
    const size_t pitch = (1024 / GS == 16) ? (((d.ng + 47) / 64) * 64 + 16) : (ng4 + 4);
    const size_t lds = B * n16 + B * ng4 * 4 + B * 64 + ((d.flags & F_COMBINE) ? (size_t)B * d.attn_n_head * 32 : 0) + (size_t)B * nmat * (d.tpw * 4) * pitch * 4;
    GemvDev dd = d; dd.nthr = 64 * p.nw;
    if constexpr (GS == 64 && B <= 2 && UPW >= 2 && NV >= 1) if (d.early) {
        auto kern = &gemv_q80_slab_kernel<ROLE, GS, B, NV, UPW, 1>;
        if (lds > 64 * 1024) (void)hipFuncSetAttribute(reinterpret_cast<const void *>(kern), hipFuncAttributeMaxDynamicSharedMemorySize, (int)lds);
        hipLaunchKernelGGL(kern, dim3(nwg), dim3(64 * p.nw), lds, st, dd);
        return hipGetLastError();
    }
    if constexpr (GS == 64 && B == 1 && (ROLE == R_NORM_STORE || ROLE == R_NORM_SWIGLU) && (NV == 1 || NV == 2)) if (slab_wave_fold(d)) {
        if (ROLE == R_NORM_SWIGLU) dd.units = (d.rw + 1) / 2;
        hipLaunchKernelGGL((gemv_q80_slab_kernel<ROLE, GS, B, NV, UPW, 0, 1>), dim3(nwg), dim3(64 * p.nw), n16 + ng4 * 4 + 64, st, dd);
        return hipGetLastError();
    }
    auto kern = &gemv_q80_slab_kernel<ROLE, GS, B, NV, UPW>;
    if (lds > 64 * 1024) (void)hipFuncSetAttribute(reinterpret_cast<const void *>(kern), hipFuncAttributeMaxDynamicSharedMemorySize, (int)lds);
    hipLaunchKernelGGL(kern, dim3(nwg), dim3(64 * p.nw), lds, st, dd);
    return hipGetLastError();
}
template <int ROLE, int GS, int B>
static hipError_t launch_slab_r(const GemvDev &d, const SlabPlan &p, uint32_t rows, hipStream_t st) {
    if (p.upw > 4) return hipErrorInvalidValue;
#define SLAB_GO(NV_, UPW_) do { if constexpr (B * NV_ <= 8) return launch_slab_t<ROLE, GS, B, NV_, UPW_>(d, p, rows, st); } while (0)
    int nv = p.nv <= 1 ? 1 : p.nv <= 2 ? 2 : p.nv <= 4 ? 4 : 0;
    const int upw = p.upw <= 1 ? 1 : p.upw <= 2 ? 2 : 4;
    if (B * nv > 8) nv = 0;
    if (nv == 1) { if (upw == 1) SLAB_GO(1, 1); if (upw == 2) SLAB_GO(1, 2); SLAB_GO(1, 4); }
    if (nv == 2) { if (upw == 1) SLAB_GO(2, 1); if (upw == 2) SLAB_GO(2, 2); SLAB_GO(2, 4); }
    if (nv == 4) { if (upw == 1) SLAB_GO(4, 1); if (upw == 2) SLAB_GO(4, 2); SLAB_GO(4, 4); }
    if (upw == 1) SLAB_GO(0, 1);
    if (upw == 2) SLAB_GO(0, 2);
    SLAB_GO(0, 4);
    return hipErrorInvalidValue;
#undef SLAB_GO
}
template <int GS, int B>
static hipError_t launch_slab_b(GemvDev &d, const GemvArgs &a, hipStream_t st) {
    const SlabPlan p = plan_slab(a, B);
    d.rw = p.rw;
    d.early = (B <= 2 && p.upw >= 2 && (uint64_t)total_rows(a) * a.n * (a.epi == GEMV_EPI_SWIGLU ? 2 : 1) >= (8u << 20)) ? 1u : 0u;
    d.tpw = (p.rw + 3) / 4;
    d.magic_rw = 65536u / p.rw + 1u;
    d.log2_tiles = 0;
    const bool sw = d.epi == GEMV_EPI_SWIGLU;
    d.units = d.tpw * d.nchunk * (sw ? 2 : 1);
    uint32_t wg[3] = {0, 0, 0};
    const uint32_t nseg = sw ? 1u : a.nseg;
    for (uint32_t s2 = 0; s2 < nseg; s2++) wg[s2] = (a.seg[s2].rows + p.rw - 1) / p.rw;
    d.wg_c0 = nseg > 1 ? wg[0] : 0xffffffffu;
    d.wg_c1 = nseg > 2 ? wg[0] + wg[1] : 0xffffffffu;
    const uint32_t rows = wg[0] + wg[1] + wg[2];
    if constexpr (B == 1) if (GS != 64 || d.canon) {
        const uint32_t f = d.flags;
        if (f == F_NORM && d.epi == GEMV_EPI_STORE) return launch_slab_r<R_NORM_STORE, GS, B>(d, p, rows, st);
        if (f == 0 && d.epi == GEMV_EPI_RESID) return launch_slab_r<R_RESID, GS, B>(d, p, rows, st);
        if (f == F_COMBINE && d.epi == GEMV_EPI_RESID) return launch_slab_r<R_RESID_COMBINE, GS, B>(d, p, rows, st);
        if (f == F_NORM && d.epi == GEMV_EPI_SWIGLU) return launch_slab_r<R_NORM_SWIGLU, GS, B>(d, p, rows, st);
    }
    return launch_slab_r<R_GENERIC, GS, B>(d, p, rows, st);
}

template <int ROLE, int GS, int B>
static hipError_t launch_stream_r(GemvDev &d, hipStream_t st) {
    d.ntiles = STREAM_WGS * 4; d.nthr = 256;
    const size_t n16 = (d.n + 15) & ~15u, ng4 = (d.ng + 3) & ~3u;
    const size_t lds = B * n16 + B * ng4 * 4 + B * 64 + 4 * 16 * (1024 / GS) * 4;
    const uint32_t nv = (d.n + 1023) / 1024;
    hipEvent_t e0 = g_q80_probe_start, e1 = g_q80_probe_stop;
    g_q80_probe_start = g_q80_probe_stop = nullptr;
#define STREAM_GO(NV_) do { if (e0 && e1) hipExtLaunchKernelGGL((gemv_q80_stream_kernel<ROLE, GS, B, NV_>), dim3(STREAM_WGS), dim3(256), (uint32_t)lds, st, e0, e1, 0, d); \
                            else hipLaunchKernelGGL((gemv_q80_stream_kernel<ROLE, GS, B, NV_>), dim3(STREAM_WGS), dim3(256), lds, st, d); } while (0)
    bool done = false;
    if (nv <= 1) { STREAM_GO(1); done = true; }
    if constexpr (B <= 4) { if (!done && nv <= 2) { STREAM_GO(2); done = true; } }
    if constexpr (B <= 2) { if (!done && nv <= 4) { STREAM_GO(4); done = true; } }
    if (!done) { STREAM_GO(0); }
#undef STREAM_GO
    return hipGetLastError();
}
template <int GS, int B>
static hipError_t launch_stream_b(GemvDev &d, hipStream_t st) {
    if (d.flags == F_NORM) return launch_stream_r<R_NORM_STORE, GS, B>(d, st);
    return launch_stream_r<R_GENERIC, GS, B>(d, st);
}

#if NANO_Q80_GS == 64
static bool fused_shape(const GemvArgs &ga, const AttnArgs &aa, SlabPlan &p) {
    if (ga.gs != 64 || ga.nb != 1 || ga.nseg != 3 || ga.epi != GEMV_EPI_STORE || !ga.norm_w || ga.xq_in || ga.attn_part || ga.tile_max || ga.resid_add) return false;
    if (ga.n % 64u || ga.n > 4096u || use_stream(ga) || !q80_canonical(ga)) return false;
    if (ga.seg[0].out_pstride || ga.seg[1].out_pstride) return false;
    p = plan_slab(ga, 1);
    if (p.nw != 4u || p.upw > 4u || !(p.nv == 1u || p.nv == 2u || p.nv == 4u)) return false;
    if (!fused_attn_side_ok(aa, ga.seg[0].rows, ga.seg[1].rows, ga.seg[2].rows)) return false;
    return true;
}

struct Wo13Plan { SlabPlan a, b; uint32_t nw, nv_a, upw_a, wa, wb; int sig; };
static bool wo13_shape(const GemvArgs &wo, const GemvArgs &w13, Wo13Plan &q) {
    if (wo.gs != 64 || w13.gs != 64 || wo.nb != 1 || w13.nb != 1 || !q80_canonical(wo) || !q80_canonical(w13)) return false;
    if (wo.nseg != 1 || wo.epi != GEMV_EPI_RESID || wo.norm_w || wo.xq_in || wo.tile_max || wo.resid_add || wo.seg[0].out_pstride) return false;
    if (wo.attn_part && (wo.attn_nsplit > 8u || wo.attn_hd % 4u)) return false;
    if (w13.nseg != 2 || w13.epi != GEMV_EPI_SWIGLU || !w13.norm_w || w13.xq_in || w13.attn_part || w13.tile_max || w13.resid_add) return false;
    if (use_stream(wo) || use_stream(w13) || w13.n != wo.seg[0].rows || w13.xin != wo.seg[0].out || w13.n % 4u) return false;
    q.a = plan_slab(wo, 1); q.b = plan_slab(w13, 1);
    q.nw = q.b.nw;
    const uint32_t units_a = ((q.a.rw + 3) / 4) * ((wo.n + 1023) / 1024);
    q.upw_a = (units_a + q.nw - 1) / q.nw;
    q.nv_a = (wo.n / 4 + 64 * q.nw - 1) / (64 * q.nw);
    q.wa = (wo.seg[0].rows + q.a.rw - 1) / q.a.rw; q.wb = (w13.seg[0].rows + q.b.rw - 1) / q.b.rw;
    const uint32_t cus = w13.cus ? w13.cus : 256u;
    if (q.wa > q.wb || q.wb > cus) return false;
    if (q.a.rw > 64 * q.nw || q.b.rw > 64 * q.nw) return false;
    q.sig = 0;
    if (q.nw == 4u && q.nv_a == 2u && q.upw_a == 1u && q.b.nv == 1u && q.b.upw == 2u) q.sig = 1;
    if (q.sig == 1) {
        const uint32_t units_b = ((q.b.rw + 3) / 4) * ((w13.n + 1023) / 1024) * 2u;
        if ((units_a + 7u) / 8u == 1u && (wo.n / 4 + 511u) / 512u == 1u && (units_b + 7u) / 8u == 1u && (w13.n / 4 + 511u) / 512u == 1u) { q.sig = 3; q.nw = 8u; }
    }
    return q.sig != 0;
}
static void slab_dev_fill(GemvDev &d, const GemvArgs &a, const SlabPlan &p, uint32_t nthr) {
    d.tile_max = nullptr;
    d.rw = p.rw; d.tpw = (p.rw + 3) / 4; d.magic_rw = 65536u / p.rw + 1u; d.log2_tiles = 0;
    d.units = d.tpw * d.nchunk * (a.epi == GEMV_EPI_SWIGLU ? 2u : 1u);
    d.wg_c0 = 0xffffffffu; d.wg_c1 = 0xffffffffu;
    d.nthr = nthr;
}
static size_t slab_lds(const GemvDev &d, bool table = true) {
    const uint32_t nmat = d.epi == GEMV_EPI_SWIGLU ? 2 : 1;
    const size_t n16 = (d.n + 15) & ~15u, ng4 = (d.ng + 3) & ~3u, pitch = ((d.ng + 47) / 64) * 64 + 16;
    return n16 + ng4 * 4 + 64 + ((d.flags & F_COMBINE) ? (size_t)d.attn_n_head * 32 : 0) + (table ? (size_t)nmat * (d.tpw * 4) * pitch * 4 : 0);
}

#endif

template <int GS, int B>
static hipError_t launch_b(const GemvArgs &a, hipStream_t st) {
    GemvDev d = to_dev(a);
    if (use_stream(a)) return launch_stream_b<GS, B>(d, st);
    d.tile_max = nullptr;
    return launch_slab_b<GS, B>(d, a, st);
}
template <int GS>
static hipError_t launch_gs(const GemvArgs &a, hipStream_t st) {
    if (a.nb <= 1) return launch_b<GS, 1>(a, st);
    if (a.nb <= 2) return launch_b<GS, 2>(a, st);
    if (a.nb <= 4) return launch_b<GS, 4>(a, st);
    return launch_b<GS, 8>(a, st);
}

}

hipError_t NANO_Q80_ENTRY(const GemvArgs &a, hipStream_t st) { return launch_gs<NANO_Q80_GS>(a, st); }

// ... 8 lines not shown
    d.rw = p.rw; d.tpw = (p.rw + 3) / 4; d.magic_rw = 65536u / p.rw + 1u; d.log2_tiles = 0;
    d.units = d.tpw * d.nchunk;
    uint32_t wg[3];
    for (uint32_t s2 = 0; s2 < 3; s2++) wg[s2] = (ga.seg[s2].rows + p.rw - 1) / p.rw;
    d.wg_c0 = wg[0]; d.wg_c1 = wg[0] + wg[1];
    const uint32_t ngemv = wg[0] + wg[1] + wg[2];
    d.nthr = 256;
    AttnArgs a = aa;
    { uint32_t l2 = 0; while ((1u << l2) < a.n_kv_head) l2++; a.kv_log2 = l2; }
    { const uint32_t kv_mul = a.n_head / a.n_kv_head; uint32_t l2 = 0; while ((1u << l2) < kv_mul) l2++; a.kvmul_log2 = l2; }
    SlabHand h{};
    h.buf = hand; h.tick = tick; h.layer1 = layer1;
    h.base[0] = 0; h.base[1] = a.q_dim; h.base[2] = a.q_dim + a.kv_dim;
    const uint32_t n_attn = a.n_head * a.nsplit;
    const size_t n16 = (d.n + 15) & ~15u, ng4 = (d.ng + 3) & ~3u, pitch = ((d.ng + 47) / 64) * 64 + 16;
    const bool wf = slab_wave_fold(d);
    const size_t lds_g = n16 + ng4 * 4 + 64 + (wf ? 0 : (size_t)(d.tpw * 4) * pitch * 4);
    const size_t hd4 = a.hd, lds_a = (hd4 + hd4 + 4 + 4 + 4 * hd4 + hd4 + 4 + 4 * 8 * hd4) * sizeof(float);
    const size_t lds = lds_g > lds_a ? lds_g : lds_a;
    if (lds > 64 * 1024) return hipErrorInvalidValue;
    const int upw = p.upw <= 1 ? 1 : p.upw <= 2 ? 2 : 4;
    FusedArgs fa{};
    fa.g = d; fa.a = a; fa.hand = h; fa.n_attn = n_attn; fa.head_wgs = a.n_head; fa.ngemv = ngemv;
    fa.wait16 = 1u;
#define FUSED_GO(NV_, UPW_) do { if (wf && NV_ == 1) hipLaunchKernelGGL((qkv_attn_fused_wf_kernel<1, UPW_>), dim3(n_attn + ngemv), dim3(256), lds, st, fa); \
                                 else hipLaunchKernelGGL((qkv_attn_fused_kernel<NV_, UPW_>), dim3(n_attn + ngemv), dim3(256), lds, st, fa); return hipGetLastError(); } while (0)
#define FUSED_NV(NV_) do { if (upw == 1) FUSED_GO(NV_, 1); if (upw == 2) FUSED_GO(NV_, 2); FUSED_GO(NV_, 4); } while (0)
    if (p.nv == 1u) FUSED_NV(1);
    if (p.nv == 2u) FUSED_NV(2);
    FUSED_NV(4);
#undef FUSED_NV
#undef FUSED_GO
}

bool wo_w13_fused_supports(const GemvArgs &wo, const GemvArgs &w13) { Wo13Plan q; return wo13_shape(wo, w13, q); }

hipError_t launch_wo_w13_fused(const GemvArgs &wo, const GemvArgs &w13, unsigned long long *hand, uint32_t *tick, uint32_t layer1, hipStream_t st) {
    Wo13Plan q;
    if (!hand || !tick || !layer1 || layer1 > 127u || !wo13_shape(wo, w13, q)) return hipErrorInvalidValue;
    Wo13Args fa{};
    fa.wo = to_dev(wo); fa.w13 = to_dev(w13);
    slab_dev_fill(fa.wo, wo, q.a, 64 * q.nw); slab_dev_fill(fa.w13, w13, q.b, 64 * q.nw);
    fa.wo_wgs = q.wa;
    fa.wait16 = 4u;
    SlabHand h{};
    h.buf = hand; h.tick = tick; h.layer1 = layer1;
    h.base[0] = 0; h.base[1] = 0; h.base[2] = 0;
    fa.hand = h;
    const bool wf = slab_wave_fold(fa.w13);
    if (wf) fa.w13.units = (fa.w13.rw + 1) / 2;
    const size_t la = slab_lds(fa.wo), lb = slab_lds(fa.w13, !wf), lds = la > lb ? la : lb;
    if (lds > 64 * 1024) return hipErrorInvalidValue;
    const bool comb = (fa.wo.flags & F_COMBINE) != 0;
#define WO13_GO(RA_, NVA_, UA_, NVB_, UB_, NT_) do { if (wf) hipLaunchKernelGGL((wo_w13_fused_kernel<RA_, NVA_, UA_, NVB_, UB_, NT_, 1>), dim3(q.wb), dim3(NT_), lds, st, fa); \
                                                     else hipLaunchKernelGGL((wo_w13_fused_kernel<RA_, NVA_, UA_, NVB_, UB_, NT_>), dim3(q.wb), dim3(NT_), lds, st, fa); return hipGetLastError(); } while (0)
    if (q.sig == 1) { if (comb) WO13_GO(R_RESID_COMBINE, 2, 1, 1, 2, 256); WO13_GO(R_RESID, 2, 1, 1, 2, 256); }
    if (comb) WO13_GO(R_RESID_COMBINE, 1, 1, 1, 1, 512);
    WO13_GO(R_RESID, 1, 1, 1, 1, 512);
#undef WO13_GO
}
#endif

}
```

nano_amd/csrc/gemv_q80_slab_body.inc:

```
#ifndef SLAB_WF
#define SLAB_WF 0
#define SLAB_WF_DEFAULTED 1
#endif
#ifndef SLAB_EARLY
#define SLAB_EARLY 0
#define SLAB_EARLY_DEFAULTED 1
#endif
#ifndef SLAB_XHAND_WAIT
#define SLAB_XHAND_WAIT 0u
#define SLAB_XHAND_NAP 0
#define SLAB_XHAND_WAIT_DEFAULTED 1
#endif
#define SLAB_ISSUE_UNIT(k) do { \
      if constexpr (WFPAIR_) { \
         \
         \
        const uint32_t u = (uint32_t)wid + (uint32_t)k * NW; \
        const bool live = u < SLAB_A.units; \
        const __amdgpu_buffer_rsrc_t rw0_ = mkrsrc(w0, live ? rows0 * n : 0u), rw1_ = mkrsrc(SLAB_A.w[1], live ? rows0 * n : 0u); \
        const __amdgpu_buffer_rsrc_t rs0_ = mkrsrc(ws0, live ? rows0 * ng * 4u : 0u), rs1_ = mkrsrc(SLAB_A.ws[1], live ? rows0 * ng * 4u : 0u); \
        const uint32_t lrow = lrow0 + u * 2u, base = lrow * n + (uint32_t)lane * 16u; \
        _Pragma("unroll") \
        for (int r = 0; r < TR; r++) wv[k][r] = bload_w(r < 2 ? rw0_ : rw1_, (u * 2u + (uint32_t)(r & 1) < RW) ? base + (uint32_t)(r & 1) * n : OOB); \
        const uint32_t r_ = (uint32_t)lane & 3u, rr_ = r_ & 1u; \
        const uint32_t so_ = (u * 2u + rr_ < RW) ? ((lrow + rr_) * ng + ((uint32_t)lane >> 2)) * 4u : OOB; \
        const float s0_ = bload_f(rs0_, r_ < 2u ? so_ : OOB), s1_ = bload_f(rs1_, r_ < 2u ? OOB : so_); \
        sv[k][0] = __uint_as_float(__float_as_uint(s0_) | __float_as_uint(s1_)); \
      } else { \
        const uint32_t u = (uint32_t)wid + (uint32_t)k * NW; \
        const uint32_t t = (u * SLAB_A.magic_nchunk) >> 16; \
        const uint32_t c = u - t * SLAB_A.nchunk; \
        const uint32_t mat = t >= TPW ? 1u : 0u, tl = t - mat * TPW; \
        const bool live = u < SLAB_A.units; \
        const __amdgpu_buffer_rsrc_t rw_ = mkrsrc(mat ? SLAB_A.w[1] : w0, live ? rows0 * n : 0u); \
        const __amdgpu_buffer_rsrc_t rs_ = mkrsrc(mat ? SLAB_A.ws[1] : ws0, live ? rows0 * ng * 4u : 0u); \
        const uint32_t lrow = lrow0 + tl * TR; \
        const uint32_t col = (c << 10) + (uint32_t)lane * 16u; \
        const uint32_t base = (col < n) ? lrow * n + col : OOB; \
        _Pragma("unroll") \
        for (int r = 0; r < TR; r++) wv[k][r] = bload_w(rw_, base + ((tl * TR + (uint32_t)r < RW) ? (uint32_t)r * n : OOB)); \
        const uint32_t g = c * GC + (uint32_t)lane / LPG; \
        _Pragma("unroll") \
        for (int s = 0; s < NS; s++) { \
            const uint32_t r = ((uint32_t)lane % LPG) + s * LPG; \
            sv[k][s] = bload_f(rs_, (r < TR && tl * TR + r < RW && g < ng) ? ((lrow + r) * ng + g) * 4u : OOB); \
        } \
      } \
    } while (0)
#if SLAB_PART != 2
    constexpr int TR = 4;
    constexpr int LPG = GS / 16, GC = 1024 / GS;
    constexpr int NS = (TR + LPG - 1) / LPG;
    const int tid = threadIdx.x, lane = tid & 63;
    const int wid = __builtin_amdgcn_readfirstlane(tid >> 6);
    const int NW = (int)(SLAB_A.nthr >> 6);
    constexpr bool WF_ = (SLAB_WF) != 0, WFPAIR_ = WF_ && ROLE == R_NORM_SWIGLU;
    static_assert(!WF_ || (GS == 64 && B == 1 && (SLAB_EARLY) == 0 && (ROLE == R_NORM_STORE || ROLE == R_NORM_SWIGLU)), "SLAB_WF: one-chunk rows of the rmsnorm roles");
    const uint32_t n = WF_ ? 1024u : SLAB_A.n, ng = WF_ ? 16u : SLAB_A.ng;
    const uint32_t n16 = (n + 15) & ~15u, ng4 = (ng + 3) & ~3u;
    const uint32_t PITCH = (GC == 16) ? (((ng + 47) / 64) * 64 + 16) : (ng4 + 4);
    const uint32_t RW = SLAB_A.rw, TPW = SLAB_A.tpw, RWP = TPW * TR;
    const uint32_t epi = role_epi<ROLE>(SLAB_A);
    const bool swiglu = epi == GEMV_EPI_SWIGLU;
    const uint32_t nmat = swiglu ? 2 : 1;
    int8_t *xq = reinterpret_cast<int8_t *>(smem);
    float *xs = reinterpret_cast<float *>(smem + B * n16);
    float *red = xs + B * ng4;
    float *P = red + B * 16 + (has_flag<ROLE>(SLAB_A, F_COMBINE) ? B * SLAB_A.attn_n_head * 8 : 0);

    karg_touch(SLAB_A.out[0]); karg_touch(SLAB_A.out_bstride[0]); karg_touch(SLAB_A.out_pstride[0]); karg_touch(SLAB_A.rows[0]); karg_touch(SLAB_A.magic_rw); karg_touch(SLAB_A.nb);
    if (!(ROLE == R_RESID || ROLE == R_RESID_COMBINE || ROLE == R_NORM_SWIGLU)) {
        karg_touch(SLAB_A.out[1]); karg_touch(SLAB_A.out[2]); karg_touch(SLAB_A.out_bstride[1]); karg_touch(SLAB_A.out_bstride[2]);
        karg_touch(SLAB_A.out_pstride[1]); karg_touch(SLAB_A.out_pstride[2]); karg_touch(SLAB_A.rows[1]); karg_touch(SLAB_A.rows[2]);
    }
    karg_touch(SLAB_A.pos); karg_touch(SLAB_A.canon);
    if (ROLE == R_GENERIC || ROLE == R_RESID || ROLE == R_RESID_COMBINE) { karg_touch(SLAB_A.resid_add); karg_touch(SLAB_A.resid_add_bstride); }
    NANO_STAMP(SLAB_A.stamps, 0, tid);
    Staged<B, NV> sx;
    if constexpr (SLAB_XHAND) stage_issue_nw<ROLE, B, NV>(SLAB_A, sx);
    else if (!(NANO_STAMPS && (SLAB_A.dbg & 2u))) stage_issue<ROLE, B, NV>(SLAB_A, sx);

    constexpr bool ONESEG = ROLE == R_RESID || ROLE == R_RESID_COMBINE || ROLE == R_NORM_SWIGLU;
    const int sel = (ONESEG || swiglu) ? 0 : (int)(SLAB_BID >= SLAB_A.wg_c0) + (int)(SLAB_BID >= SLAB_A.wg_c1);
    const int8_t *w0 = sel == 0 ? SLAB_A.w[0] : sel == 1 ? SLAB_A.w[1] : SLAB_A.w[2];
    const float *ws0 = sel == 0 ? SLAB_A.ws[0] : sel == 1 ? SLAB_A.ws[1] : SLAB_A.ws[2];
    float *out0 = sel == 0 ? SLAB_A.out[0] : sel == 1 ? SLAB_A.out[1] : SLAB_A.out[2];
    const uint32_t rows0 = sel == 0 ? SLAB_A.rows[0] : sel == 1 ? SLAB_A.rows[1] : SLAB_A.rows[2];
    const uint32_t obs = sel == 0 ? SLAB_A.out_bstride[0] : sel == 1 ? SLAB_A.out_bstride[1] : SLAB_A.out_bstride[2];
    const uint32_t ops = sel == 0 ? SLAB_A.out_pstride[0] : sel == 1 ? SLAB_A.out_pstride[1] : SLAB_A.out_pstride[2];
    const uint32_t lrow0 = (SLAB_BID - (sel == 0 ? 0u : sel == 1 ? SLAB_A.wg_c0 : SLAB_A.wg_c1)) * RW;

    int4 wv[UPW][TR];
    float sv[UPW][NS];
    constexpr uint32_t early_ = (uint32_t)(SLAB_EARLY);
    static_assert(SLAB_PART == 0 || early_ == 0u, "SLAB_EARLY: the whole body only");
#pragma unroll
    for (int k = 0; k < UPW; k++) { if (early_ == 0u || (uint32_t)k < early_) SLAB_ISSUE_UNIT(k); }
    if (!SLAB_XHAND && NANO_STAMPS && (SLAB_A.dbg & 2u)) stage_issue<ROLE, B, NV>(SLAB_A, sx);
    const int fb = (int)(((uint32_t)tid * SLAB_A.magic_rw) >> 16);
    const int frl = tid - fb * (int)RW;
    const bool fold_live = tid < (int)(RW * B) && fb < (int)SLAB_A.nb && lrow0 + frl < rows0;
    uint32_t opos = 0;
    if constexpr (WF_) {
        if constexpr (ROLE == R_NORM_STORE) opos = __float_as_uint(bload_f(mkrsrc(SLAB_A.pos, ops ? 4u : 0u), ((uint32_t)lane & ~3u) == (uint32_t)WF_LANE0 ? 0u : OOB));
    } else
    if (ops && fold_live) opos = SLAB_A.pos[fb];
    float oldv = 0.0f;
    if (epi == GEMV_EPI_RESID && fold_live) oldv = out0[(size_t)fb * obs + lrow0 + frl];
    float addv = 0.0f;
    const bool has_add = epi == GEMV_EPI_RESID && SLAB_A.resid_add != nullptr;
    if (has_add && fold_live) addv = SLAB_A.resid_add[(size_t)fb * SLAB_A.resid_add_bstride + lrow0 + frl];

    NANO_STAMP(SLAB_A.stamps, 1, oldv);
#endif
#if SLAB_PART != 1
    if constexpr (SLAB_XHAND) {
        static_assert(!SLAB_XHAND || B == 1, "granule activations: one sequence");
        const unsigned long long *hb_ = SLAB_XHANDV.buf;
        const uint32_t ctag_ = SLAB_CTAG;
        bool got_ = false;
        for (uint32_t w_ = 0; w_ < SLAB_XHAND_WAIT; w_++) __builtin_amdgcn_s_sleep(16);
        for (uint32_t spin_ = 0; spin_ < (1u << 14) && !got_; spin_++) {
            if (spin_) __builtin_amdgcn_s_sleep(SLAB_XHAND_NAP);
            if ((spin_ & 63u) == 63u && hand_aborted(SLAB_XHANDV)) break;
            got_ = true;
#pragma unroll
            for (int j = 0; j < NV; j++) {
                const uint32_t i = ((uint32_t)tid + (uint32_t)j * SLAB_A.nthr) * 4u;
                if (i < n) {
                    const unsigned long long g0_ = __hip_atomic_load(hb_ + i, __ATOMIC_RELAXED, __HIP_MEMORY_SCOPE_AGENT);
                    const unsigned long long g1_ = __hip_atomic_load(hb_ + i + 1, __ATOMIC_RELAXED, __HIP_MEMORY_SCOPE_AGENT);
                    const unsigned long long g2_ = __hip_atomic_load(hb_ + i + 2, __ATOMIC_RELAXED, __HIP_MEMORY_SCOPE_AGENT);
                    const unsigned long long g3_ = __hip_atomic_load(hb_ + i + 3, __ATOMIC_RELAXED, __HIP_MEMORY_SCOPE_AGENT);
                    got_ = got_ && (uint32_t)(g0_ >> 32) == ctag_ && (uint32_t)(g1_ >> 32) == ctag_ && (uint32_t)(g2_ >> 32) == ctag_ && (uint32_t)(g3_ >> 32) == ctag_;
                    sx.x[0][j] = make_float4(__uint_as_float((uint32_t)g0_), __uint_as_float((uint32_t)g1_), __uint_as_float((uint32_t)g2_), __uint_as_float((uint32_t)g3_));
                } else sx.x[0][j] = make_float4(0.f, 0.f, 0.f, 0.f);
            }
        }
        if (!got_) hand_give_up(SLAB_XHANDV, SLAB_A.err);
    }
    stage_finish<ROLE, GS, B, NV>(SLAB_A, sx, xq, xs, red, n16, ng4);
    if constexpr (early_ != 0u) {
#pragma unroll
        for (int k = 1; k < UPW; k++) { if ((uint32_t)k >= early_) SLAB_ISSUE_UNIT(k); }
    }
    NANO_STAMP(SLAB_A.stamps, 3, xs[0]);

    if constexpr (WF_) {
    float pw_[UPW];
    const int4 xv_ = *reinterpret_cast<const int4 *>(xq + lane * 16);
    const float xsc_ = xs[lane >> 2];
    asm volatile("" :: "v"(xsc_));
#pragma unroll
    for (int k = 0; k < UPW; k++) {
        int iv[TR];
#pragma unroll
        for (int r = 0; r < TR; r++) {
            int d = __builtin_amdgcn_sdot4(wv[k][r].x, xv_.x, 0, false);
            d = __builtin_amdgcn_sdot4(wv[k][r].y, xv_.y, d, false);
            d = __builtin_amdgcn_sdot4(wv[k][r].z, xv_.z, d, false);
            d = __builtin_amdgcn_sdot4(wv[k][r].w, xv_.w, d, false);
            iv[r] = dpp_group_sum<LPG>(d);
        }
        int v = iv[0];
#pragma unroll
        for (int q = 1; q < TR; q++) v = (q == (lane & 3)) ? iv[q] : v;
        pw_[k] = ((float)v * sv[k][0]) * xsc_;
    }
    NANO_STAMP(SLAB_A.stamps, 4, pw_[UPW - 1]);
    NANO_STAMP(SLAB_A.stamps, 5, pw_[UPW - 1]);
#pragma unroll
    for (int k = 0; k < UPW; k++) {
        const uint32_t u = (uint32_t)wid + (uint32_t)k * NW;
        if (u < SLAB_A.units) {
            const float v0 = wave_fold_canon16(pw_[k]);
            const float v1 = WFPAIR_ ? DPP_F(v0, 0x102) : 0.0f;
            const uint32_t rl_ = WFPAIR_ ? u * 2u + ((uint32_t)lane & 1u) : u * (uint32_t)TR + ((uint32_t)lane & 3u);
            const bool mine_ = WFPAIR_ ? ((uint32_t)lane & ~1u) == (uint32_t)WF_LANE0 : ((uint32_t)lane & ~3u) == (uint32_t)WF_LANE0;
            if (mine_ && rl_ < RW && lrow0 + rl_ < rows0) {
                float *dst = out0 + (size_t)opos * ops + lrow0 + rl_;
                const float val = finish_epi(epi, v0, v1, 0.0f);
                if constexpr (SLAB_HAND == 1)
                    __hip_atomic_store(SLAB_HANDV.buf + (sel == 0 ? SLAB_HANDV.base[0] : sel == 1 ? SLAB_HANDV.base[1] : SLAB_HANDV.base[2]) + lrow0 + rl_,
                                       ((unsigned long long)(SLAB_PTAG) << 32) | (unsigned long long)__float_as_uint(val), __ATOMIC_RELAXED, __HIP_MEMORY_SCOPE_AGENT);
                if (NANO_STAMPS && (SLAB_A.dbg & 4u)) *dst = val; else __hip_atomic_store(dst, val, __ATOMIC_RELAXED, __HIP_MEMORY_SCOPE_AGENT);
            }
        }
    }
    } else {
#pragma unroll
    for (int k = 0; k < UPW; k++) {
        const uint32_t u = (uint32_t)wid + (uint32_t)k * NW;
        if (u < SLAB_A.units) {
            const uint32_t t = (u * SLAB_A.magic_nchunk) >> 16;
            const uint32_t c = u - t * SLAB_A.nchunk;
            const uint32_t mat = t >= TPW ? 1u : 0u, tl = t - mat * TPW;
            const uint32_t col = (c << 10) + (uint32_t)lane * 16u;
            const uint32_t g = c * GC + (uint32_t)lane / LPG;
#pragma unroll
            for (int b = 0; b < B; b++) {
                if (b < (int)SLAB_A.nb) {
                    const int4 xv = (col < n) ? *reinterpret_cast<const int4 *>(xq + b * n16 + col) : make_int4(0, 0, 0, 0);
                    int iv[TR];
#pragma unroll
                    for (int r = 0; r < TR; r++) {
                        int d = __builtin_amdgcn_sdot4(wv[k][r].x, xv.x, 0, false);
                        d = __builtin_amdgcn_sdot4(wv[k][r].y, xv.y, d, false);
                        d = __builtin_amdgcn_sdot4(wv[k][r].z, xv.z, d, false);
                        d = __builtin_amdgcn_sdot4(wv[k][r].w, xv.w, d, false);
                        iv[r] = dpp_group_sum<LPG>(d);
                    }
                    const float xsc = (g < ng) ? xs[b * ng4 + g] : 0.0f;
#pragma unroll
                    for (int s = 0; s < NS; s++) {
                        const uint32_t r = ((uint32_t)lane % LPG) + s * LPG;
                        int v = iv[0];
#pragma unroll
                        for (int q = 1; q < TR; q++) v = (q == (int)r) ? iv[q] : v;
                        if (r < TR && g < ng)
                            P[(((size_t)b * nmat + mat) * RWP + tl * TR + r) * PITCH + g] = ((float)v * sv[k][s]) * xsc;
                    }
                }
            }
        }
    }
    NANO_STAMP(SLAB_A.stamps, 4, wv[UPW - 1][TR - 1].w);
    __syncthreads();
    NANO_STAMP(SLAB_A.stamps, 5, P[0]);

    constexpr bool PFOLD = early_ != 0u && GS == 64;
    bool pfold_ = false;
    if constexpr (PFOLD) {
        pfold_ = (ROLE != R_GENERIC || SLAB_A.canon) && (ng & 7u) == 0u;
        if (pfold_) {
            const uint32_t nu_ = ng >> 3, rows_ = RW * (uint32_t)B * nmat, items_ = rows_ * nu_;
            for (uint32_t it = (uint32_t)tid; it < items_; it += SLAB_A.nthr) {
                const uint32_t rr_ = it / nu_, u_ = it - rr_ * nu_;
                const uint32_t bm_ = rr_ / RW, rl_ = rr_ - bm_ * RW;
                float *pu_ = P + ((size_t)bm_ * RWP + rl_) * PITCH + 8u * u_;
                const float4 t0_ = *reinterpret_cast<const float4 *>(pu_), t1_ = *reinterpret_cast<const float4 *>(pu_ + 4);
                pu_[0] = unit_sum(t0_, t1_);
            }
            __syncthreads();
        }
    }
    if (tid < (int)(RW * B)) {
        float v0 = 0.0f, v1 = 0.0f;
        const float *p0 = P + (((size_t)fb * nmat) * RWP + frl) * PITCH;
        const float *p1 = p0 + (size_t)RWP * PITCH;
        constexpr bool ROLE_CANON = ROLE != R_GENERIC && GS == 64;
        if (PFOLD && pfold_) {
            const uint32_t nu_ = ng >> 3;
            v0 = p0[0];
            for (uint32_t u_ = 1; u_ < nu_; u_++) v0 = fadd(v0, p0[8u * u_]);
// ... 15 lines not shown
                float4 t[4], u[4];
#pragma unroll
                for (int q = 0; q < 4; q++) { t[q] = *reinterpret_cast<const float4 *>(p0 + g0 + 4 * q); if (swiglu) u[q] = *reinterpret_cast<const float4 *>(p1 + g0 + 4 * q); }
#pragma unroll
                for (int q = 0; q < 4; q++) { v0 += t[q].x; v0 += t[q].y; v0 += t[q].z; v0 += t[q].w; }
                if (swiglu) {
#pragma unroll
                    for (int q = 0; q < 4; q++) { v1 += u[q].x; v1 += u[q].y; v1 += u[q].z; v1 += u[q].w; }
                }
            }
        } else {
        for (uint32_t g0 = 0; g0 < ng; g0 += 16) {
                float4 t[4], u[4];
#pragma unroll
                for (int q = 0; q < 4; q++) {
                    t[q] = (g0 + 4 * q < ng4) ? *reinterpret_cast<const float4 *>(p0 + g0 + 4 * q) : make_float4(0.f, 0.f, 0.f, 0.f);
                    if (swiglu) u[q] = (g0 + 4 * q < ng4) ? *reinterpret_cast<const float4 *>(p1 + g0 + 4 * q) : make_float4(0.f, 0.f, 0.f, 0.f);
                }
#pragma unroll
                for (int q = 0; q < 4; q++) {
                    const uint32_t g = g0 + 4 * q;
                    v0 += (g < ng) ? t[q].x : 0.0f; v0 += (g + 1 < ng) ? t[q].y : 0.0f; v0 += (g + 2 < ng) ? t[q].z : 0.0f; v0 += (g + 3 < ng) ? t[q].w : 0.0f;
                }
                if (swiglu) {
#pragma unroll
                    for (int q = 0; q < 4; q++) {
                        const uint32_t g = g0 + 4 * q;
                        v1 += (g < ng) ? u[q].x : 0.0f; v1 += (g + 1 < ng) ? u[q].y : 0.0f; v1 += (g + 2 < ng) ? u[q].z : 0.0f; v1 += (g + 3 < ng) ? u[q].w : 0.0f;
                    }
                }
            }
        }
        if (fold_live) {
            float *dst = out0 + (size_t)fb * obs + (size_t)opos * ops + lrow0 + frl;
            const float val = finish_epi(epi, has_add ? v0 + addv : v0, v1, oldv);
            if constexpr (SLAB_HAND == 1)
                __hip_atomic_store(SLAB_HANDV.buf + (sel == 0 ? SLAB_HANDV.base[0] : sel == 1 ? SLAB_HANDV.base[1] : SLAB_HANDV.base[2]) + lrow0 + (uint32_t)frl,
                                   ((unsigned long long)(SLAB_PTAG) << 32) | (unsigned long long)__float_as_uint(val), __ATOMIC_RELAXED, __HIP_MEMORY_SCOPE_AGENT);
            if (NANO_STAMPS && (SLAB_A.dbg & 4u)) *dst = val; else __hip_atomic_store(dst, val, __ATOMIC_RELAXED, __HIP_MEMORY_SCOPE_AGENT);
        }
    }
    }
    NANO_STAMP_END(SLAB_A.stamps, 6);
#endif
#undef SLAB_ISSUE_UNIT
#ifdef SLAB_WF_DEFAULTED
#undef SLAB_WF
#undef SLAB_WF_DEFAULTED
#endif
#ifdef SLAB_EARLY_DEFAULTED
#undef SLAB_EARLY
#undef SLAB_EARLY_DEFAULTED
#endif
#ifdef SLAB_XHAND_WAIT_DEFAULTED
#undef SLAB_XHAND_WAIT
#undef SLAB_XHAND_NAP
#undef SLAB_XHAND_WAIT_DEFAULTED
#endif
```

nano_amd/csrc/kernels.h:

```cpp
#pragma once

#include <hip/hip_runtime.h>
#include <stddef.h>
#include <stdint.h>
#include "../../include/nano_mi355x.h"
#include "device_common.h"

namespace nano {

enum : uint32_t { GEMV_EPI_STORE = 0, GEMV_EPI_RESID = 1, GEMV_EPI_SWIGLU = 2 };

struct GemvSeg {
    const void *w;
    const float *ws;
    float *out;
    uint32_t rows;
    uint32_t out_bstride;
    uint32_t out_pstride;
    uint32_t _pad;
};

struct GemvArgs {
    GemvSeg seg[3];
    uint32_t nseg;
// ... 70 lines not shown
    uint32_t quant; int cus;
    uint32_t mfma_min_nb;
    int8_t *gq; float *gxs;
    uint8_t *q4x; size_t q4x_bytes;
};
RouteKind route_kind(const Q80Route &r, const GemvArgs &a);
hipError_t route_projection(const Q80Route &r, GemvArgs &a, hipStream_t st);
uint32_t route_norm_order(const Q80Route &r, const GemvArgs &a);
bool route_is_wide(const GemvArgs &a);

constexpr uint32_t ATTN_MAX_NSPLIT = 64;
uint32_t attention_wide_from();
uint32_t attention_split_cap();
struct AttnArgs {
    const float *q;
    float *q_out;
    const float *kraw;
    float *kcache;
    float *vcache;
    const uint32_t *pos;
    const float *q_norm;
    const float *k_norm;
    const float *rope_cos;
    const float *rope_sin;
    const float *rope_cur;
    float *out;
    float *ml;
    float *xba_out;
    uint32_t nsplit;
    uint32_t range_hint;
    uint32_t layer, n_layer, S, hd, n_head, n_kv_head, q_dim, kv_dim;
    uint32_t rope_qwen3;
    uint32_t is_causal;
    uint32_t cache_bstride_rows;
    uint32_t fixed_range;
    uint32_t prep_only;
    uint32_t kv_half;
    const float *vraw;
    int8_t *xf_out; float *xsf_out;
    uint32_t kv_log2, kvmul_log2;
    const uint32_t *pt_rows;
    const uint32_t *kvrow;
    uint32_t pt_stride, pt_bstride;
    uint32_t pool_rows, _pad6;
    uint32_t *err;
    unsigned long long *stamps;
};
hipError_t launch_attention(const AttnArgs &a, uint32_t nb, hipStream_t st);
struct AttnPlan { uint32_t mode, lpr, qv, kvm, npt, w16, paged, kv_half, nsplit, kv_log2, kvmul_log2; };
bool attention_plan(const AttnArgs &a, uint32_t nb, AttnPlan *p);
bool qkv_attn_fused_supports(const GemvArgs &ga, const AttnArgs &aa);
hipError_t launch_qkv_attn_fused(const GemvArgs &ga, const AttnArgs &aa, unsigned long long *hand, uint32_t *tick, uint32_t layer1, hipStream_t st);
bool wo_w13_fused_supports(const GemvArgs &wo, const GemvArgs &w13);
hipError_t launch_wo_w13_fused(const GemvArgs &wo, const GemvArgs &w13, unsigned long long *hand, uint32_t *tick, uint32_t layer1, hipStream_t st);
inline bool fused_attn_side_ok(const AttnArgs &aa, uint32_t qr, uint32_t kr, uint32_t vr) {
    if (aa.hd != 128u || !aa.q_norm || !aa.k_norm || !aa.rope_qwen3 || !aa.rope_cos || !aa.rope_cur || !aa.kraw || aa.fixed_range || !aa.is_causal || aa.q_out) return false;
    if (aa.kv_half || aa.pt_rows || aa.prep_only || aa.xf_out || aa.nsplit == 0 || aa.nsplit > 8u) return false;
    const uint32_t kv_mul = aa.n_kv_head ? aa.n_head / aa.n_kv_head : 0u;
    if (!aa.n_kv_head || (aa.n_kv_head & (aa.n_kv_head - 1u)) || !kv_mul || (kv_mul & (kv_mul - 1u))) return false;
    if ((uint64_t)aa.n_head * aa.nsplit > 256u) return false;
    if (aa.range_hint > aa.nsplit * 2u * 32u) return false;
    return aa.q_dim == qr && aa.kv_dim == kr && aa.kv_dim == vr && aa.q_dim == aa.n_head * aa.hd;
}
inline bool fused_attn_side_ok_plain(const AttnArgs &aa, uint32_t qr, uint32_t kr, uint32_t vr) {
    if (aa.hd < 4u || aa.hd > 64u || aa.hd % 4u || aa.q_norm || aa.k_norm || aa.rope_qwen3 || !aa.rope_cos || !aa.rope_cur || !aa.kraw || aa.fixed_range || !aa.is_causal || aa.q_out) return false;
    if (aa.kv_half || aa.pt_rows || aa.prep_only || aa.xf_out || aa.nsplit == 0 || aa.nsplit > 8u) return false;
    const uint32_t kv_mul = aa.n_kv_head ? aa.n_head / aa.n_kv_head : 0u;
    if (!aa.n_kv_head || (aa.n_kv_head & (aa.n_kv_head - 1u)) || !kv_mul || (kv_mul & (kv_mul - 1u))) return false;
    if ((uint64_t)aa.n_head * aa.nsplit > 256u) return false;
    if (aa.range_hint > aa.nsplit * 2u * 32u) return false;
    return aa.q_dim == qr && aa.kv_dim == kr && aa.kv_dim == vr && aa.q_dim == aa.n_head * aa.hd;
}
bool qkv_attn_fused_f32_supports(const GemvArgs &ga, const AttnArgs &aa);
hipError_t launch_qkv_attn_fused_f32(const GemvArgs &ga, const AttnArgs &aa, unsigned long long *hand, uint32_t *tick, uint32_t layer1, hipStream_t st);
bool qkv_attn_fused_q4k_supports(const GemvArgs &ga, const AttnArgs &aa);
hipError_t launch_qkv_attn_fused_q4k(const GemvArgs &ga, const AttnArgs &aa, unsigned long long *hand, uint32_t *tick, uint32_t layer1, hipStream_t st);
uint32_t attention_nsplit(uint32_t range_hint, uint32_t hd);
hipError_t launch_attn_combine(const float *part, const float *ml, float *out, uint32_t n_head, uint32_t hd, uint32_t nsplit, hipStream_t st);
hipError_t launch_attn_combine_tokens(const float *part, const float *ml, float *out, uint32_t n_head, uint32_t hd, uint32_t nsplit, uint32_t nb,
                                      int8_t *xf_out, float *xsf_out, hipStream_t st);

struct StrictAttnArgs {
    float *q;
    const float *kraw;
    float *kcache, *vcache;
    const uint32_t *pos;
    const float *q_norm, *k_norm;
    const float *rope_cos, *rope_sin;
    float *att;
    float *xba;
    uint32_t n_head, n_kv_head, hd, q_dim, kv_dim, layer, n_layer, S;
    uint32_t slot0;
    uint32_t rope_qwen3, is_causal;
    uint32_t fold_prep;
};
hipError_t launch_strict_rmsnorm(float *o, const float *x, const float *w, uint32_t n, uint32_t nvec, uint32_t x_stride, uint32_t o_stride, hipStream_t st);
hipError_t launch_strict_qk(const StrictAttnArgs &a, uint32_t nb, hipStream_t st);
hipError_t launch_strict_attention(const StrictAttnArgs &a, uint32_t nb, hipStream_t st);
hipError_t launch_strict_swiglu(float *hb, const float *hb2, uint32_t n, uint32_t nb, uint32_t bstride, hipStream_t st);
hipError_t launch_strict_matmul_f32(float *out, const float *x, const float *w, uint32_t n, uint32_t d, uint32_t nb, uint32_t x_bstride,
                                    uint32_t out_bstride, uint32_t out_pstride, const uint32_t *pos, int resid, hipStream_t st);

hipError_t launch_exact_rmsnorm(float *o, const float *x, const float *w, uint32_t n, uint32_t nvec, uint32_t x_stride, uint32_t o_stride, hipStream_t st);
bool exact_attention_fits(uint32_t hd, uint32_t max_range);
hipError_t launch_exact_attention(const StrictAttnArgs &a, uint32_t nb, hipStream_t st);

// ... 98 lines not shown
```

nano_amd/csrc/ops.hip:

```cpp
#include <stdio.h>
#include <string.h>

#include <string>
#include <vector>

#include "../../include/nano_mi355x.h"
#include "kernels.h"

using namespace nano;

extern "C" const char *nano_hip_last_error(void);
namespace { thread_local std::string g_op_err; }

extern "C" void nano_hip_set_error_(const char *msg);

struct DevBufs {
    std::vector<void *> ptrs;
    ~DevBufs() { for (void *p : ptrs) (void)hipFree(p); }
    template <typename T> T *alloc(size_t n) {
        void *p = nullptr;
        if (hipMalloc(&p, n * sizeof(T) + 16) != hipSuccess) return nullptr;
        ptrs.push_back(p);
        return reinterpret_cast<T *>(p);
    }
// ... 123 lines not shown
    OP_HIP(hipMemcpy(out, dout, QD * 4, hipMemcpyDeviceToHost));
    return 0;
}

extern "C" int nano_hip_op_swiglu(int device, float *hb, const float *hb2, uint32_t n) {
    int rc; if ((rc = begin(device))) return rc;
    DevBufs B; float *d1 = B.upload(hb, n), *d2 = B.upload(hb2, n);
    OP_CHECK(d1 && d2, "device alloc failed");
    OP_HIP(launch_swiglu(d1, d2, n, 0));
    OP_HIP(hipMemcpy(hb, d1, (size_t)n * 4, hipMemcpyDeviceToHost));
    return 0;
}

extern "C" int nano_hip_op_exact_rmsnorm(int device, float *out, const float *x, const float *w, uint32_t n) {
    int rc; if ((rc = begin(device))) return rc;
    DevBufs B; float *dx = B.upload(x, n), *dw = B.upload(w, n), *dout = B.alloc<float>(n);
    OP_CHECK(dx && dw && dout, "device alloc failed");
    OP_HIP(launch_exact_rmsnorm(dout, dx, dw, n, 1, n, n, 0));
    OP_HIP(hipMemcpy(out, dout, (size_t)n * 4, hipMemcpyDeviceToHost));
    return 0;
}

extern "C" int nano_hip_op_exact_attention(int device, const NanoExactAttnDesc *d) {
    int rc; if ((rc = begin(device))) return rc;
    if (!d || !d->q || !d->k_cache || !d->v_cache || !d->out) { nano_hip_set_error_("null argument"); return NANO_HIP_EINVAL; }
    if (!d->n_head || !d->n_kv_head || d->n_head % d->n_kv_head || !d->hd || d->hd % 4 || d->hd > 256 || !d->S ||
        (d->is_causal && (d->range == 0 || d->range > d->S))) { nano_hip_set_error_("bad attention shape"); return NANO_HIP_EINVAL; }
    if (!d->long_form && !exact_attention_fits(d->hd, d->S)) { nano_hip_set_error_("S rows do not fit the one-launch kernel's LDS: set long_form"); return NANO_HIP_EINVAL; }
    const uint32_t qd = d->n_head * d->hd, kvd = d->n_kv_head * d->hd, pos = d->is_causal ? d->range - 1u : 0u;
    DevBufs B;
    float *dq = B.upload(d->q, qd), *dk = B.upload(d->k_cache, (size_t)d->S * kvd), *dv = B.upload(d->v_cache, (size_t)d->S * kvd);
    float *dout = B.alloc<float>(qd), *datt = d->long_form ? B.alloc<float>((size_t)d->n_head * d->S) : nullptr;
    uint32_t *dpos = B.upload(&pos, 1);
    OP_CHECK(dq && dk && dv && dout && dpos && (datt || !d->long_form), "device alloc failed");
    StrictAttnArgs sa{};
    sa.q = dq; sa.kcache = dk; sa.vcache = dv; sa.pos = dpos; sa.att = datt; sa.xba = dout;
    sa.n_head = d->n_head; sa.n_kv_head = d->n_kv_head; sa.hd = d->hd; sa.q_dim = qd; sa.kv_dim = kvd;
    sa.layer = 0; sa.n_layer = 1; sa.S = d->S; sa.slot0 = 0; sa.is_causal = d->is_causal ? 1u : 0u;
    OP_HIP(d->long_form ? launch_strict_attention(sa, 1, 0) : launch_exact_attention(sa, 1, 0));
    OP_HIP(hipMemcpy(d->out, dout, (size_t)qd * 4, hipMemcpyDeviceToHost));
    return 0;
}

extern "C" int nano_hip_op_argmax(int device, const float *x, uint32_t n, uint32_t *idx) {
    int rc; if ((rc = begin(device))) return rc;
    DevBufs B; float *dx = B.upload(x, n); uint32_t *di = B.alloc<uint32_t>(1);
    OP_CHECK(dx && di, "device alloc failed");
    ArgmaxArgs a{ dx, n, n, di, nullptr, nullptr, nullptr, nullptr, 1 };
    OP_HIP(launch_argmax(a, 1, 0));
    OP_HIP(hipMemcpy(idx, di, 4, hipMemcpyDeviceToHost));
    return 0;
}

extern "C" int nano_hip_op_fused_gemv(int device, const NanoFusedGemvDesc *dp) {
    int rc; if ((rc = begin(device))) return rc;
    if (!dp) { nano_hip_set_error_("null descriptor"); return NANO_HIP_EINVAL; }
    const NanoFusedGemvDesc &d = *dp;
    if (d.kind > 2 || d.nseg == 0 || d.nseg > 3 || (d.kind == 2 && d.nseg != 2) || d.nb == 0 || d.nb > NANO_MAX_BATCH || !d.out || d.n % 4) {
        nano_hip_set_error_("bad fused-gemv descriptor"); return NANO_HIP_EINVAL;
    }
    if (!d.x && !d.attn_part) { nano_hip_set_error_("no activation"); return NANO_HIP_EINVAL; }
    if (d.quant == NANO_QUANT_Q80 && (!(d.gs == 32 || d.gs == 64 || d.gs == 128 || d.gs == 256) || d.n % d.gs || d.n % 16)) { nano_hip_set_error_("bad n / group size"); return NANO_HIP_EINVAL; }
    DevBufs B;
    GemvArgs a{};
    const size_t bpl = (d.n + 255) / 256;
    uint32_t rows_total = 0;
    for (uint32_t s = 0; s < d.nseg; s++) {
        const size_t rows = d.rows[s];
        if (!d.w[s] || !rows) { nano_hip_set_error_("missing weight tensor"); return NANO_HIP_EINVAL; }
        if (d.quant == NANO_QUANT_Q80) {
            a.seg[s].w = B.upload(reinterpret_cast<const int8_t *>(d.w[s]), rows * d.n);
            a.seg[s].ws = B.upload(d.ws[s], rows * d.n / d.gs);
            OP_CHECK(a.seg[s].ws, "device alloc failed");
        } else if (d.quant == NANO_QUANT_Q4K) a.seg[s].w = B.upload(reinterpret_cast<const uint8_t *>(d.w[s]), rows * bpl * 160);
        else a.seg[s].w = B.upload(reinterpret_cast<const float *>(d.w[s]), rows * d.n);
        OP_CHECK(a.seg[s].w, "device alloc failed");
        a.seg[s].rows = d.rows[s];
        if (d.kind != 2 || s == 0) rows_total += d.rows[s];
    }
    if (d.kind == 2 && d.rows[0] != d.rows[1]) { nano_hip_set_error_("W1 / W3 row counts differ"); return NANO_HIP_EINVAL; }
    float *dout = B.upload(d.out, (size_t)d.nb * rows_total);
    OP_CHECK(dout, "device alloc failed");
    uint32_t off = 0;
    for (uint32_t s = 0; s < d.nseg; s++) {
        a.seg[s].out = d.kind == 2 ? dout : dout + off;
        a.seg[s].out_bstride = rows_total;
        if (d.kind != 2) off += d.rows[s];
    }
    a.nseg = d.nseg; a.n = d.n; a.gs = d.gs; a.nb = d.nb;
    a.epi = d.kind == 0 ? GEMV_EPI_STORE : d.kind == 1 ? GEMV_EPI_RESID : GEMV_EPI_SWIGLU;
    if (d.x) { a.xin = B.upload(d.x, (size_t)d.nb * d.n); OP_CHECK(a.xin, "device alloc failed"); a.xin_bstride = d.n; }
    if (d.norm_w) { a.norm_w = B.upload(d.norm_w, d.n); OP_CHECK(a.norm_w, "device alloc failed"); }
    if (d.attn_part) {
        if (!d.attn_ml || !d.attn_nsplit || d.attn_nsplit > 8 || !d.attn_n_head || d.attn_n_head * d.attn_hd != d.n || d.kind != 1 || d.nb > 8) { nano_hip_set_error_("bad attention partials"); return NANO_HIP_EINVAL; }
        a.attn_part = B.upload(d.attn_part, (size_t)d.nb * d.attn_nsplit * d.n);
        a.attn_ml = B.upload(d.attn_ml, (size_t)d.nb * d.attn_n_head * d.attn_nsplit * 2);
        OP_CHECK(a.attn_part && a.attn_ml, "device alloc failed");
        a.attn_nsplit = d.attn_nsplit; a.attn_n_head = d.attn_n_head; a.attn_hd = d.attn_hd;
        if (!a.xin) { a.xin = a.attn_part; a.xin_bstride = d.n; }
    }
    hipDeviceProp_t prop; OP_HIP(hipGetDeviceProperties(&prop, device));
    a.cus = (uint32_t)prop.multiProcessorCount;
    a.ordered = d.ordered ? 1u : 0u;
    Q80Route r{};
    r.quant = d.quant; r.cus = (int)a.cus; r.mfma_min_nb = d.use_gemm ? 1u : 9u;
    if (d.quant == NANO_QUANT_Q80) {
        const size_t n16 = (d.n + 15) & ~(size_t)15, tt = (d.nb + 15) / 16;
        r.gq = B.alloc<int8_t>(tt * 16 * n16); r.gxs = B.alloc<float>(tt * 16 * (d.n / d.gs));
        OP_CHECK(r.gq && r.gxs, "device alloc failed");
    }
    if (d.quant == NANO_QUANT_Q4K && d.nb > 1) {
        r.q4x_bytes = (size_t)8 * ((d.n + 255) & ~(size_t)255);
        r.q4x = B.alloc<uint8_t>(r.q4x_bytes);
        OP_CHECK(r.q4x, "device alloc failed");
    }
    if (d.use_gemm && (d.quant != NANO_QUANT_Q80 || !route_takes_fragments(route_kind(r, a)))) { nano_hip_set_error_("the batched GEMM route does not take this launch"); return NANO_HIP_EINVAL; }
    if (d.route_out) *d.route_out = (uint32_t)route_kind(r, a);
    const hipError_t e = route_projection(r, a, 0);
    OP_HIP(e);
    OP_HIP(hipDeviceSynchronize());
    OP_HIP(hipMemcpy(d.out, dout, (size_t)d.nb * rows_total * 4, hipMemcpyDeviceToHost));
    return 0;
}

extern "C" int nano_hip_op_attention_decode(int device, const NanoAttnDecodeDesc *dp) {
    int rc; if ((rc = begin(device))) return rc;
    if (!dp) { nano_hip_set_error_("null descriptor"); return NANO_HIP_EINVAL; }
    const NanoAttnDecodeDesc &d = *dp;
#define OP_ARG(cond, msg) do { if (!(cond)) { nano_hip_set_error_(msg); return NANO_HIP_EINVAL; } } while (0)
    OP_ARG(d.nb >= 1 && d.nb <= NANO_MAX_BATCH, "nb out of range");
    OP_ARG(d.n_kv_head && d.n_head && d.n_head % d.n_kv_head == 0 && d.hd >= 4 && d.hd % 4 == 0 && d.hd <= 256, "bad attention shape");
    OP_ARG(d.n_layer && d.layer < d.n_layer && d.S, "bad layer / S");
    OP_ARG(d.q && d.k && d.pos && d.rope_cos && d.rope_sin && d.k_cache && d.v_cache && d.out, "missing tensor");
    OP_ARG(!d.q_norm == !d.k_norm, "q_norm and k_norm go together");
    const uint32_t nb = d.nb, QD = d.n_head * d.hd, KD = d.n_kv_head * d.hd, half = d.hd / 2;
    uint32_t maxpos = 0;
    for (uint32_t b = 0; b < nb; b++) {
        maxpos = d.pos[b] > maxpos ? d.pos[b] : maxpos;
        OP_ARG(!d.chunk || d.pos[b] == d.pos[0] + b, "chunk: positions must be consecutive");
    }
    OP_ARG(d.range_hint >= maxpos + 1 && d.range_hint <= d.S, "range_hint must cover max(pos) + 1 and stay <= S");
    const uint32_t nsplit = d.nsplit ? d.nsplit : attention_nsplit(d.range_hint, d.hd);
    OP_ARG(nsplit >= 1 && nsplit <= ATTN_MAX_NSPLIT, "nsplit out of range");
    OP_ARG(!d.want_frag || (nsplit == 1 && d.hd % 64 == 0 && d.xf && d.xsf), "fragment output: nsplit 1 and hd % 64 == 0 only");
    const bool paged = d.pool_rows != 0;
    const uint32_t seqs = d.chunk ? 1u : nb;
    const size_t esz = d.kv_half ? 2 : 4;
    const size_t cache_elems = paged ? (size_t)d.n_layer * d.pool_rows * KD : (size_t)seqs * d.n_layer * d.S * KD;
    std::vector<uint32_t> kvrow(nb, 0u);
    if (paged) {
        OP_ARG(d.pool_rows % 64 == 0 && d.pt_rows && d.pt_stride, "paged: pool_rows % 64, page table");
        for (size_t i = 0; i < (size_t)seqs * d.pt_stride; i++)
            OP_ARG(d.pt_rows[i] == 0xffffffffu || (d.pt_rows[i] % 64 == 0 && d.pt_rows[i] < d.pool_rows && d.pool_rows - d.pt_rows[i] >= 64), "paged: a page-table entry lies outside the pool");
        for (uint32_t b = 0; b < nb; b++) {
            const uint32_t blk = d.pos[b] >> 6, e = d.pt_rows[(size_t)(d.chunk ? 0 : b) * d.pt_stride + (blk < d.pt_stride ? blk : 0)];
            OP_ARG(blk < d.pt_stride && e != 0xffffffffu, "paged: no page holds pos");
            kvrow[b] = e + (d.pos[b] & 63u);
        }
    }
    std::vector<float> rope_cur((size_t)nb * 2 * half);
    for (uint32_t b = 0; b < nb; b++)
        for (uint32_t i = 0; i < half; i++) {
            rope_cur[(size_t)b * 2 * half + i] = d.rope_cos[(size_t)d.pos[b] * half + i];
            rope_cur[(size_t)b * 2 * half + half + i] = d.rope_sin[(size_t)d.pos[b] * half + i];
        }
    DevBufs B;
    float *dq = B.upload(d.q, (size_t)nb * QD), *dk = B.upload(d.k, (size_t)nb * KD);
    uint32_t *dpos = B.upload(d.pos, nb);
    float *dcos = B.upload(d.rope_cos, (size_t)d.S * half), *dsin = B.upload(d.rope_sin, (size_t)d.S * half), *dcur = B.upload(rope_cur.data(), rope_cur.size());
    unsigned char *dkc = B.upload(reinterpret_cast<const unsigned char *>(d.k_cache), cache_elems * esz);
    unsigned char *dvc = B.upload(reinterpret_cast<const unsigned char *>(d.v_cache), cache_elems * esz);
    float *dout = B.alloc<float>((size_t)nb * QD), *dpart = B.alloc<float>((size_t)nb * nsplit * QD), *dml = B.alloc<float>((size_t)nb * d.n_head * nsplit * 2);
    OP_CHECK(dq && dk && dpos && dcos && dsin && dcur && dkc && dvc && dout && dpart && dml, "device alloc failed");
    AttnArgs a{};
// ... 49 lines not shown
```

Baseline: 1989.

## Specialise combine staging by split count and head shift; add fused Wo+W13 test ops

Templates the staged attention-combine on the number of split slots (2/4/8), replaces the per-element division by head dim with a shift when head dim is a power of two, and adds a single-sequence (ONE) path that drops batch bound checks in the slab kernel. It also adds test entry points for the fused Wo + W1|W3 launch and a standalone combine-weights kernel. The aim is fewer loads and integer ops in the residual-combine GEMV prologue during decode. Shapes whose head dim is not a power of two now fall back to the generic role.

Result: no change. 1996, median of 5 (+0.4%).

```diff
diff --git a/include/nano_mi355x.h b/include/nano_mi355x.h
--- a/include/nano_mi355x.h
+++ b/include/nano_mi355x.h
@@ -193,6 +193,8 @@
     float *out;
 } NanoFusedGemvDesc;
 int nano_hip_op_fused_gemv(int device, const NanoFusedGemvDesc *d);
+int nano_hip_op_wo_w13_fused(int device, const NanoFusedGemvDesc *wo, const NanoFusedGemvDesc *w13);
+int nano_hip_op_combine_weights(int device, const float *ml, uint32_t n_head, uint32_t nsplit, float *out);
 
 typedef struct NanoBlobShare NanoBlobShare;
 int nano_hip_blob_share(NanoBlobShare **out, const void *host_params, size_t bytes, int root_device, const int *devices, int n_devices);
diff --git a/nano_amd/binding.py b/nano_amd/binding.py
--- a/nano_amd/binding.py
+++ b/nano_amd/binding.py
@@ -441,6 +441,48 @@
     return out
 
 
+def _fused_gemv_desc(quant, kind, n, weights, x, norm_w, gs, resid, attn, keep):
+    d = NanoFusedGemvDesc()
+    d.quant, d.gs, d.kind, d.n, d.nb, d.nseg = quant, gs, kind, n, 1, len(weights)
+    for i, (w, ws, rows) in enumerate(weights):
+        w = np.ascontiguousarray(w); ws = np.ascontiguousarray(ws, np.float32); keep += [w, ws]
+        d.rows[i] = rows; d.w[i] = w.ctypes.data; d.ws[i] = ws.ctypes.data
+    if x is not None:
+        x = np.ascontiguousarray(x, np.float32); keep.append(x); d.x = x.ctypes.data
+    if norm_w is not None:
+        norm_w = np.ascontiguousarray(norm_w, np.float32); keep.append(norm_w); d.norm_w = norm_w.ctypes.data
+    if attn is not None:
+        part, ml, n_head, hd = attn
+        part = np.ascontiguousarray(part, np.float32); ml = np.ascontiguousarray(ml, np.float32); keep += [part, ml]
+        d.attn_part, d.attn_ml = part.ctypes.data, ml.ctypes.data
+        d.attn_nsplit, d.attn_n_head, d.attn_hd = part.shape[-2], n_head, hd
+    rows_total = weights[0][2] if kind == 2 else sum(r for _, _, r in weights)
+    out = np.zeros((1, rows_total), np.float32) if resid is None else np.array(resid, np.float32, copy=True).reshape(1, rows_total)
+    keep.append(out)
+    d.out = out.ctypes.data
+    return d, out
+
+
+def op_wo_w13_fused(n, wo, w1, w3, norm_w, resid, *, x=None, attn=None, device=0):
+    keep = []
+    da, xo = _fused_gemv_desc(0x80, 1, n, [wo], None if x is None else np.asarray(x, np.float32).reshape(1, n), None, 64, resid, attn, keep)
+    db, hb = _fused_gemv_desc(0x80, 2, wo[2], [w1, w3], None, norm_w, 64, None, None, keep)
+    f = lib().nano_hip_op_wo_w13_fused
+    f.restype, f.argtypes = C.c_int, [C.c_int, C.POINTER(NanoFusedGemvDesc), C.POINTER(NanoFusedGemvDesc)]
+    check(f(device, C.byref(da), C.byref(db)))
+    return xo[0], hb[0]
+
+
+def op_combine_weights(ml, device=0):
+    ml = np.ascontiguousarray(ml, np.float32)
+    n_head, nsplit = ml.shape[0], ml.shape[1]
+    out = np.empty((n_head, 8), np.float32)
+    f = lib().nano_hip_op_combine_weights
+    f.restype, f.argtypes = C.c_int, [C.c_int, C.c_void_p, C.c_uint32, C.c_uint32, C.c_void_p]
+    check(f(device, ml.ctypes.data, n_head, nsplit, out.ctypes.data))
+    return out
+
+
 def op_attention_decode(q, k, pos, k_cache, v_cache, *, n_head, n_kv_head, hd, n_layer, layer, S, range_hint, rope_cos, rope_sin,
                         rope_qwen3, q_norm=None, k_norm=None, vraw=None, kv_half=False, chunk=False, nsplit=0, want_frag=False,
                         pt_rows=None, pool_rows=0, device=0):
diff --git a/nano_amd/csrc/gemv_common.h b/nano_amd/csrc/gemv_common.h
--- a/nano_amd/csrc/gemv_common.h
+++ b/nano_amd/csrc/gemv_common.h
@@ -65,6 +65,7 @@
     uint32_t rows[3], out_bstride[3], out_pstride[3];
     uint32_t n, ng, rw, log2_tiles, nchunk, magic_nchunk, units, epi, flags, nb;
     uint32_t tpw, magic_rw, wg_c0, wg_c1;
+    uint32_t attn_hd_log2;
     const float *xin; const float *norm_w; const uint32_t *pos;
     uint32_t xin_bstride, nthr;
     const int8_t *xq_in; const float *xs_in;
@@ -92,22 +93,24 @@
     return GEMV_EPI_RESID;
 }
 
-template <int B, int NV>
+template <int B, int NV, int NSP = 8>
 struct Staged {
     float4 x[B][NV];
     float4 nw[NV];
-    float4 pv[B == 1 ? NV : 1][B == 1 ? 8 : 1];
+    float4 pv[B == 1 ? NV : 1][B == 1 ? NSP : 1];
     float ml_m, ml_l;
 };
-template <int B>
-struct Staged<B, 0> {};
-
-template <int ROLE, int B, int NV>
-__device__ __forceinline__ void stage_issue(const GemvDev &a, Staged<B, NV> &r) {
+template <int B, int NSP>
+struct Staged<B, 0, NSP> {};
+
+template <int ROLE, int B, int NV, bool ONE = false, int NSP>
+__device__ __forceinline__ void stage_issue(const GemvDev &a, Staged<B, NV, NSP> &r) {
+    static_assert(NSP == 2 || NSP == 4 || NSP == 8, "split slots of the staged combine");
+    static_assert(!ONE || B == 1, "ONE: kernels of one sequence");
     if constexpr (NV == 0) { (void)a; (void)r; return; } else {
     const uint32_t tid = threadIdx.x, nthr = a.nthr, n = a.n;
     const bool plain = !has_flag<ROLE>(a, F_PRE) && !has_flag<ROLE>(a, F_COMBINE);
-    const __amdgpu_buffer_rsrc_t rx = mkrsrc(a.xin, plain ? ((a.nb - 1) * a.xin_bstride + n) * 4u : 0u);
+    const __amdgpu_buffer_rsrc_t rx = mkrsrc(a.xin, plain ? (ONE ? n : (a.nb - 1) * a.xin_bstride + n) * 4u : 0u);
     const __amdgpu_buffer_rsrc_t rn = mkrsrc(a.norm_w, has_flag<ROLE>(a, F_NORM) ? n * 4u : 0u);
 #pragma unroll
     for (int j = 0; j < NV; j++) {
@@ -115,20 +118,21 @@
         const uint32_t off = (i < n) ? i * 4u : OOB;
         if (plain) {
 #pragma unroll
-            for (int b = 0; b < B; b++) r.x[b][j] = bload_f4(rx, (b < (int)a.nb) ? off + (uint32_t)b * a.xin_bstride * 4u : OOB);
+            for (int b = 0; b < B; b++) r.x[b][j] = bload_f4(rx, (ONE || b < (int)a.nb) ? off + (uint32_t)b * a.xin_bstride * 4u : OOB);
         }
         if (has_flag<ROLE>(a, F_NORM)) r.nw[j] = (NANO_STAMPS && (a.dbg & 1u)) ? make_float4(1.f, 1.f, 1.f, 1.f) : bload_f4(rn, off);
     }
     if constexpr (B == 1) {
       if (has_flag<ROLE>(a, F_COMBINE)) {
         const uint32_t ns = a.attn_nsplit, nh = a.attn_n_head;
+        if (ROLE != R_GENERIC) karg_touch(a.attn_hd_log2);
         const __amdgpu_buffer_rsrc_t rp = mkrsrc(a.attn_part, ns * n * 4u);
         const __amdgpu_buffer_rsrc_t rm = mkrsrc(a.attn_ml, nh * ns * 8u);
 #pragma unroll
         for (int j = 0; j < NV; j++) {
             const uint32_t i = (tid + (uint32_t)j * nthr) * 4u;
 #pragma unroll
-            for (int sp = 0; sp < 8; sp++) r.pv[j][sp] = bload_f4(rp, (i < n && (uint32_t)sp < ns) ? ((uint32_t)sp * n + i) * 4u : OOB);
+            for (int sp = 0; sp < NSP; sp++) r.pv[j][sp] = bload_f4(rp, (i < n && (uint32_t)sp < ns) ? ((uint32_t)sp * n + i) * 4u : OOB);
         }
         const uint32_t sp = tid & 7u, h = tid >> 3;
         const uint32_t mo = (h < nh && sp < ns) ? (h * ns + sp) * 8u : OOB;
@@ -139,8 +143,8 @@
     }
 }
 
-template <int ROLE, int B, int NV>
-__device__ __forceinline__ void stage_issue_nw(const GemvDev &a, Staged<B, NV> &r) {
+template <int ROLE, int B, int NV, int NSP>
+__device__ __forceinline__ void stage_issue_nw(const GemvDev &a, Staged<B, NV, NSP> &r) {
     if constexpr (NV == 0) { (void)a; (void)r; return; } else {
     const uint32_t tid = threadIdx.x, nthr = a.nthr, n = a.n;
     const __amdgpu_buffer_rsrc_t rn = mkrsrc(a.norm_w, has_flag<ROLE>(a, F_NORM) ? n * 4u : 0u);
@@ -157,7 +161,7 @@
     const uint32_t tid = threadIdx.x, nthr = a.nthr;
     const uint32_t ns = a.attn_nsplit, nh = a.attn_n_head;
     for (uint32_t t = tid; t < (uint32_t)B * nh * 8u; t += nthr) {
-        const uint32_t s = t & 7u, h = (t >> 3) % nh, b = (t >> 3) / nh;
+        const uint32_t s = t & 7u, h = B == 1 ? t >> 3 : (t >> 3) % nh, b = B == 1 ? 0u : (t >> 3) / nh;
         float m = -INFINITY, l = 0.0f;
         if constexpr (PRE) { m = pm; l = pl; (void)s; (void)h; (void)b; (void)ns; }
         else if (s < ns && b < a.nb) { const float *ml = a.attn_ml + (((size_t)b * nh + h) * ns + s) * 2; m = ml[0]; l = ml[1]; }
@@ -172,10 +176,28 @@
     }
     __syncthreads();
 }
+template <int NSP>
+__device__ __forceinline__ float4 combine_staged(const float4 (&pv)[NSP], const float *wg ) {
+    float4 acc = make_float4(0.f, 0.f, 0.f, 0.f);
+#pragma unroll
+    for (int sp = 0; sp < NSP; sp++) {
+        const float w = wg[sp];
+        acc.x += pv[sp].x * w; acc.y += pv[sp].y * w; acc.z += pv[sp].z * w; acc.w += pv[sp].w * w;
+    }
+    return acc;
+}
+template <int ROLE> __device__ __forceinline__ uint32_t combine_head(const GemvDev &a, uint32_t i) {
+    if (ROLE == R_GENERIC) return i / a.attn_hd;
+    return i >> a.attn_hd_log2;
+}
+static uint32_t combine_nsp(uint32_t nsplit) { return nsplit <= 2u ? 2u : nsplit <= 4u ? 4u : 8u; }
+static uint32_t log2_or_none(uint32_t v) { uint32_t l = 0; while ((1u << l) < v && l < 31u) l++; return (v && (1u << l) == v) ? l : 0xffffffffu; }
+
+template <int ROLE>
 __device__ __forceinline__ float4 combine4(const GemvDev &a, uint32_t b, uint32_t i, const float *wgt) {
     const uint32_t ns = a.attn_nsplit, n = a.n;
     const float *part = a.attn_part + (size_t)b * ns * n + i;
-    const float *wg = wgt + ((size_t)b * a.attn_n_head + i / a.attn_hd) * 8u;
+    const float *wg = wgt + ((size_t)b * a.attn_n_head + combine_head<ROLE>(a, i)) * 8u;
     float4 o[8];
 #pragma unroll
     for (int s = 0; s < 8; s++) o[s] = ((uint32_t)s < ns) ? *reinterpret_cast<const float4 *>(part + (size_t)s * n) : make_float4(0.f, 0.f, 0.f, 0.f);
@@ -217,6 +239,7 @@
     d.xin = a.xin; d.norm_w = a.norm_w; d.pos = a.pos; d.xin_bstride = a.xin_bstride;
     d.xq_in = a.xq_in; d.xs_in = a.xs_in;
     d.attn_part = a.attn_part; d.attn_ml = a.attn_ml; d.attn_nsplit = a.attn_nsplit; d.attn_n_head = a.attn_n_head; d.attn_hd = a.attn_hd;
+    d.attn_hd_log2 = log2_or_none(a.attn_hd);
     d.tile_max = a.tile_max;
     d.resid_add = a.resid_add; d.resid_add_bstride = a.resid_add_bstride;
     d.stamps = a.stamps;
diff --git a/nano_amd/csrc/gemv_f32.hip b/nano_amd/csrc/gemv_f32.hip
--- a/nano_amd/csrc/gemv_f32.hip
+++ b/nano_amd/csrc/gemv_f32.hip
@@ -18,7 +18,7 @@
             if (norm) {
                 float acc = 0.0f;
                 for (uint32_t i = tid * 4u; i < n; i += nthr * 4u) {
-                    const float4 v = comb ? combine4(a, b, i, wgt) : *reinterpret_cast<const float4 *>(x + i);
+                    const float4 v = comb ? combine4<ROLE>(a, b, i, wgt) : *reinterpret_cast<const float4 *>(x + i);
                     acc += v.x * v.x; acc += v.y * v.y; acc += v.z * v.z; acc += v.w * v.w;
                 }
                 acc = dpp_wave_sum(acc);
@@ -31,7 +31,7 @@
                 ss = 1.0f / sqrtf(t);
             }
             for (uint32_t i = tid * 4u; i < n; i += nthr * 4u) {
-                float4 v = comb ? combine4(a, b, i, wgt) : *reinterpret_cast<const float4 *>(x + i);
+                float4 v = comb ? combine4<ROLE>(a, b, i, wgt) : *reinterpret_cast<const float4 *>(x + i);
                 if (norm) {
                     const float4 w = *reinterpret_cast<const float4 *>(a.norm_w + i);
                     v.x = w.x * (ss * v.x); v.y = w.y * (ss * v.y); v.z = w.z * (ss * v.z); v.w = w.w * (ss * v.w);
@@ -48,14 +48,7 @@
 #pragma unroll
                 for (int j = 0; j < NV; j++) {
                     const uint32_t i = (tid + (uint32_t)j * nthr) * 4u;
-                    const float *wg = wgt + (size_t)((i < n ? i : 0u) / a.attn_hd) * 8u;
-                    float4 acc = make_float4(0.f, 0.f, 0.f, 0.f);
-#pragma unroll
-                    for (int sp = 0; sp < 8; sp++) {
-                        const float w = wg[sp];
-                        acc.x += r.pv[j][sp].x * w; acc.y += r.pv[j][sp].y * w; acc.z += r.pv[j][sp].z * w; acc.w += r.pv[j][sp].w * w;
-                    }
-                    r.x[0][j] = acc;
+                    r.x[0][j] = combine_staged<8>(r.pv[j], wgt + (size_t)combine_head<ROLE>(a, i < n ? i : 0u) * 8u);
                 }
             } else {
                 combine_weights<B, false>(a, wgt, 0.0f, 0.0f);
@@ -64,7 +57,7 @@
 #pragma unroll
                     for (int j = 0; j < NV; j++) {
                         const uint32_t i = (tid + (uint32_t)j * nthr) * 4u;
-                        r.x[b][j] = (i < n && b < (int)a.nb) ? combine4(a, b, i, wgt) : make_float4(0.f, 0.f, 0.f, 0.f);
+                        r.x[b][j] = (i < n && b < (int)a.nb) ? combine4<ROLE>(a, b, i, wgt) : make_float4(0.f, 0.f, 0.f, 0.f);
                     }
             }
         }
@@ -226,7 +219,7 @@
         const uint32_t f = d.flags;
         if (f == F_NORM && d.epi == GEMV_EPI_STORE) return launch_f32_r<R_NORM_STORE, B>(d, p, rows, st);
         if (f == 0 && d.epi == GEMV_EPI_RESID) return launch_f32_r<R_RESID, B>(d, p, rows, st);
-        if (f == F_COMBINE && d.epi == GEMV_EPI_RESID) return launch_f32_r<R_RESID_COMBINE, B>(d, p, rows, st);
+        if (f == F_COMBINE && d.epi == GEMV_EPI_RESID && d.attn_hd_log2 != 0xffffffffu) return launch_f32_r<R_RESID_COMBINE, B>(d, p, rows, st);
         if (f == F_NORM && d.epi == GEMV_EPI_SWIGLU) return launch_f32_r<R_NORM_SWIGLU, B>(d, p, rows, st);
     }
     return launch_f32_r<R_GENERIC, B>(d, p, rows, st);
diff --git a/nano_amd/csrc/gemv_q4k.hip b/nano_amd/csrc/gemv_q4k.hip
--- a/nano_amd/csrc/gemv_q4k.hip
+++ b/nano_amd/csrc/gemv_q4k.hip
@@ -287,7 +287,7 @@
         const uint32_t f = d.flags;
         if (f == F_NORM && d.epi == GEMV_EPI_STORE) return launch_q4k_r<R_NORM_STORE, B>(d, p, rows, st);
         if (f == 0 && d.epi == GEMV_EPI_RESID) return launch_q4k_r<R_RESID, B>(d, p, rows, st);
-        if (f == F_COMBINE && d.epi == GEMV_EPI_RESID) return launch_q4k_r<R_RESID_COMBINE, B>(d, p, rows, st);
+        if (f == F_COMBINE && d.epi == GEMV_EPI_RESID && d.attn_hd_log2 != 0xffffffffu) return launch_q4k_r<R_RESID_COMBINE, B>(d, p, rows, st);
         const uint32_t GT = ((d.n + 255) / 256) * 8;
         if (f == F_NORM && d.epi == GEMV_EPI_SWIGLU && (p.rw * GT) % 64u == 0u && p.nthr % 64u == 0u) return launch_q4k_r<R_NORM_SWIGLU, B>(d, p, rows, st);
     }
diff --git a/nano_amd/csrc/gemv_q4k_chunk.hip b/nano_amd/csrc/gemv_q4k_chunk.hip
--- a/nano_amd/csrc/gemv_q4k_chunk.hip
+++ b/nano_amd/csrc/gemv_q4k_chunk.hip
@@ -184,7 +184,7 @@
 hipError_t launch_quant_rows_r(const GemvDev &d, XGroup *out, uint32_t nb, size_t lds, hipStream_t st) {
     if (d.flags == F_NORM) return launch_quant_rows_t<R_NORM_STORE, NV>(d, out, nb, lds, st);
     if (d.flags == 0) return launch_quant_rows_t<R_RESID, NV>(d, out, nb, lds, st);
-    if (d.flags == F_COMBINE) return launch_quant_rows_t<R_RESID_COMBINE, NV>(d, out, nb, lds, st);
+    if (d.flags == F_COMBINE && d.attn_hd_log2 != 0xffffffffu) return launch_quant_rows_t<R_RESID_COMBINE, NV>(d, out, nb, lds, st);
     return launch_quant_rows_t<R_GENERIC, NV>(d, out, nb, lds, st);
 }
 
@@ -287,7 +287,7 @@
     const uint32_t f = d.flags;
     if (f == F_NORM && d.epi == GEMV_EPI_STORE) return launch_chunk_r<R_NORM_STORE>(d, p, st);
     if (f == 0 && d.epi == GEMV_EPI_RESID) return launch_chunk_r<R_RESID>(d, p, st);
-    if (f == F_COMBINE && d.epi == GEMV_EPI_RESID) return launch_chunk_r<R_RESID_COMBINE>(d, p, st);
+    if (f == F_COMBINE && d.epi == GEMV_EPI_RESID && d.attn_hd_log2 != 0xffffffffu) return launch_chunk_r<R_RESID_COMBINE>(d, p, st);
     if (f == F_NORM && d.epi == GEMV_EPI_SWIGLU) return launch_chunk_r<R_NORM_SWIGLU>(d, p, st);
     return launch_chunk_r<R_GENERIC>(d, p, st);
 }
diff --git a/nano_amd/csrc/gemv_q4k_impl.h b/nano_amd/csrc/gemv_q4k_impl.h
--- a/nano_amd/csrc/gemv_q4k_impl.h
+++ b/nano_amd/csrc/gemv_q4k_impl.h
@@ -73,7 +73,7 @@
             if (norm) {
                 float acc = 0.0f;
                 for (uint32_t i = tid * 4u; i < n; i += nthr * 4u) {
-                    const float4 v = comb ? combine4(a, b, i, wgt) : *reinterpret_cast<const float4 *>(x + i);
+                    const float4 v = comb ? combine4<ROLE>(a, b, i, wgt) : *reinterpret_cast<const float4 *>(x + i);
                     acc += v.x * v.x; acc += v.y * v.y; acc += v.z * v.z; acc += v.w * v.w;
                 }
                 acc = dpp_wave_sum(acc);
@@ -86,7 +86,7 @@
                 ss = 1.0f / sqrtf(t);
             }
             for (uint32_t i = tid * 4u; i < n; i += nthr * 4u) {
-                float4 v = comb ? combine4(a, b, i, wgt) : *reinterpret_cast<const float4 *>(x + i);
+                float4 v = comb ? combine4<ROLE>(a, b, i, wgt) : *reinterpret_cast<const float4 *>(x + i);
                 if (norm) {
                     const float4 w = *reinterpret_cast<const float4 *>(a.norm_w + i);
                     v.x = w.x * (ss * v.x); v.y = w.y * (ss * v.y); v.z = w.z * (ss * v.z); v.w = w.w * (ss * v.w);
@@ -103,14 +103,7 @@
 #pragma unroll
                 for (int j = 0; j < NV; j++) {
                     const uint32_t i = (tid + (uint32_t)j * nthr) * 4u;
-                    const float *wg = wgt + (size_t)((i < n ? i : 0u) / a.attn_hd) * 8u;
-                    float4 acc = make_float4(0.f, 0.f, 0.f, 0.f);
-#pragma unroll
-                    for (int sp = 0; sp < 8; sp++) {
-                        const float w = wg[sp];
-                        acc.x += r.pv[j][sp].x * w; acc.y += r.pv[j][sp].y * w; acc.z += r.pv[j][sp].z * w; acc.w += r.pv[j][sp].w * w;
-                    }
-                    r.x[0][j] = acc;
+                    r.x[0][j] = combine_staged<8>(r.pv[j], wgt + (size_t)combine_head<ROLE>(a, i < n ? i : 0u) * 8u);
                 }
             } else {
                 combine_weights<B, false>(a, wgt, 0.0f, 0.0f);
@@ -119,7 +112,7 @@
 #pragma unroll
                     for (int j = 0; j < NV; j++) {
                         const uint32_t i = (tid + (uint32_t)j * nthr) * 4u;
-                        r.x[b][j] = (i < n && b < (int)a.nb) ? combine4(a, b, i, wgt) : make_float4(0.f, 0.f, 0.f, 0.f);
+                        r.x[b][j] = (i < n && b < (int)a.nb) ? combine4<ROLE>(a, b, i, wgt) : make_float4(0.f, 0.f, 0.f, 0.f);
                     }
             }
         }
diff --git a/nano_amd/csrc/gemv_q80_impl.h b/nano_amd/csrc/gemv_q80_impl.h
--- a/nano_amd/csrc/gemv_q80_impl.h
+++ b/nano_amd/csrc/gemv_q80_impl.h
@@ -13,8 +13,8 @@
     *reinterpret_cast<uint32_t *>(dst) = (uint32_t)(q0 & 0xff) | ((uint32_t)(q1 & 0xff) << 8) | ((uint32_t)(q2 & 0xff) << 16) | ((uint32_t)(q3 & 0xff) << 24);
 }
 
-template <int ROLE, int GS, int B, int NV>
-__device__ __forceinline__ void stage_finish(const GemvDev &a, Staged<B, NV> &r, int8_t *xq, float *xs, float *red, uint32_t n16, uint32_t ng4) {
+template <int ROLE, int GS, int B, int NV, int NSP>
+__device__ __forceinline__ void stage_finish(const GemvDev &a, Staged<B, NV, NSP> &r, int8_t *xq, float *xs, float *red, uint32_t n16, uint32_t ng4) {
     const uint32_t tid = threadIdx.x, nthr = a.nthr, n = a.n, ng = a.ng;
     const uint32_t lane = tid & 63u, wid = tid >> 6, NW = nthr >> 6;
     if (has_flag<ROLE>(a, F_PRE)) {
@@ -35,7 +35,7 @@
             if (norm) {
                 float acc = 0.0f;
                 for (uint32_t i = tid * 4u; i < n; i += nthr * 4u) {
-                    const float4 v = comb ? combine4(a, b, i, wgt) : *reinterpret_cast<const float4 *>(x + i);
+                    const float4 v = comb ? combine4<ROLE>(a, b, i, wgt) : *reinterpret_cast<const float4 *>(x + i);
                     acc += v.x * v.x; acc += v.y * v.y; acc += v.z * v.z; acc += v.w * v.w;
                 }
                 acc = dpp_wave_sum(acc);
@@ -48,7 +48,7 @@
                 ss = 1.0f / sqrtf(t);
             }
             for (uint32_t i = tid * 4u; i < n; i += nthr * 4u) {
-                float4 v = comb ? combine4(a, b, i, wgt) : *reinterpret_cast<const float4 *>(x + i);
+                float4 v = comb ? combine4<ROLE>(a, b, i, wgt) : *reinterpret_cast<const float4 *>(x + i);
                 if (norm) {
                     const float4 w = *reinterpret_cast<const float4 *>(a.norm_w + i);
                     v.x = w.x * (ss * v.x); v.y = w.y * (ss * v.y); v.z = w.z * (ss * v.z); v.w = w.w * (ss * v.w);
@@ -69,14 +69,7 @@
 #pragma unroll
                 for (int j = 0; j < NV; j++) {
                     const uint32_t i = (tid + (uint32_t)j * nthr) * 4u;
-                    const float *wg = wgt + (size_t)((i < n ? i : 0u) / a.attn_hd) * 8u;
-                    float4 acc = make_float4(0.f, 0.f, 0.f, 0.f);
-#pragma unroll
-                    for (int sp = 0; sp < 8; sp++) {
-                        const float w = wg[sp];
-                        acc.x += r.pv[j][sp].x * w; acc.y += r.pv[j][sp].y * w; acc.z += r.pv[j][sp].z * w; acc.w += r.pv[j][sp].w * w;
-                    }
-                    r.x[0][j] = acc;
+                    r.x[0][j] = combine_staged<NSP>(r.pv[j], wgt + (size_t)combine_head<ROLE>(a, i < n ? i : 0u) * 8u);
                 }
             } else {
                 combine_weights<B, false>(a, wgt, 0.0f, 0.0f);
@@ -85,7 +78,7 @@
 #pragma unroll
                     for (int j = 0; j < NV; j++) {
                         const uint32_t i = (tid + (uint32_t)j * nthr) * 4u;
-                        r.x[b][j] = (i < n && b < (int)a.nb) ? combine4(a, b, i, wgt) : make_float4(0.f, 0.f, 0.f, 0.f);
+                        r.x[b][j] = (i < n && b < (int)a.nb) ? combine4<ROLE>(a, b, i, wgt) : make_float4(0.f, 0.f, 0.f, 0.f);
                     }
             }
         }
@@ -242,11 +235,12 @@
 }
 constexpr int WF_LANE0 = 48;
 
-template <int ROLE, int GS, int B, int NV, int UPW, int EARLY = 0, int WF = 0>
+template <int ROLE, int GS, int B, int NV, int UPW, int EARLY = 0, int WF = 0, int NSP = 8>
 __global__ __launch_bounds__(1024) void gemv_q80_slab_kernel(const GemvDev a) {
     extern __shared__ __attribute__((aligned(16))) unsigned char smem[];
 #define SLAB_EARLY EARLY
 #define SLAB_WF WF
+#define SLAB_NSP NSP
 #define SLAB_A a
 #define SLAB_BID blockIdx.x
 #define SLAB_HAND 0
@@ -268,6 +262,7 @@
 #undef SLAB_PART
 #undef SLAB_EARLY
 #undef SLAB_WF
+#undef SLAB_NSP
 }
 
 #if NANO_Q80_GS == 64
@@ -291,7 +286,7 @@
 }
 
 struct Wo13Args { GemvDev wo; GemvDev w13; SlabHand hand; uint32_t wo_wgs, wait16; };
-template <int ROLE_A, int NV_A, int UPW_A, int NV_B, int UPW_B, int NT, int WF = 0>
+template <int ROLE_A, int NV_A, int UPW_A, int NV_B, int UPW_B, int NT, int WF = 0, int NSP = 8>
 __global__ __launch_bounds__(NT) void wo_w13_fused_kernel(const Wo13Args fa) {
     extern __shared__ __attribute__((aligned(16))) unsigned char smem[];
     constexpr int GS = 64, B = 1;
@@ -306,6 +301,8 @@
 #define SLAB_XHAND 0
 #define SLAB_XHANDV (SlabHand{})
 #define SLAB_CTAG 0u
+#define SLAB_NSP NSP
+#define SLAB_XLIVE (blockIdx.x < fa.wo_wgs)
 #define SLAB_PART 1
 #include "gemv_q80_slab_body.inc"
 #undef SLAB_PART
@@ -314,6 +311,8 @@
 #include "gemv_q80_slab_body.inc"
 #undef SLAB_PART
         };
+#undef SLAB_NSP
+#undef SLAB_XLIVE
 #undef SLAB_A
 #undef SLAB_HAND
 #undef SLAB_HANDV
@@ -541,7 +540,7 @@
 static bool slab_wave_fold(const GemvDev &d) {
     return d.n == 1024u && d.ng == 16u && !d.early && (d.epi == GEMV_EPI_STORE || (d.epi == GEMV_EPI_SWIGLU && !d.out_pstride[0]));
 }
-template <int ROLE, int GS, int B, int NV, int UPW>
+template <int ROLE, int GS, int B, int NV, int UPW, int NSP = 8>
 static hipError_t launch_slab_t(const GemvDev &d, const SlabPlan &p, uint32_t nwg, hipStream_t st) {
     const uint32_t nmat = d.epi == GEMV_EPI_SWIGLU ? 2 : 1;
     const size_t n16 = (d.n + 15) & ~15u, ng4 = (d.ng + 3) & ~3u;
@@ -549,7 +548,7 @@
     const size_t lds = B * n16 + B * ng4 * 4 + B * 64 + ((d.flags & F_COMBINE) ? (size_t)B * d.attn_n_head * 32 : 0) + (size_t)B * nmat * (d.tpw * 4) * pitch * 4;
     GemvDev dd = d; dd.nthr = 64 * p.nw;
     if constexpr (GS == 64 && B <= 2 && UPW >= 2 && NV >= 1) if (d.early) {
-        auto kern = &gemv_q80_slab_kernel<ROLE, GS, B, NV, UPW, 1>;
+        auto kern = &gemv_q80_slab_kernel<ROLE, GS, B, NV, UPW, 1, 0, NSP>;
         if (lds > 64 * 1024) (void)hipFuncSetAttribute(reinterpret_cast<const void *>(kern), hipFuncAttributeMaxDynamicSharedMemorySize, (int)lds);
         hipLaunchKernelGGL(kern, dim3(nwg), dim3(64 * p.nw), lds, st, dd);
         return hipGetLastError();
@@ -559,18 +558,29 @@
         hipLaunchKernelGGL((gemv_q80_slab_kernel<ROLE, GS, B, NV, UPW, 0, 1>), dim3(nwg), dim3(64 * p.nw), n16 + ng4 * 4 + 64, st, dd);
         return hipGetLastError();
     }
-    auto kern = &gemv_q80_slab_kernel<ROLE, GS, B, NV, UPW>;
+    if constexpr (ROLE == R_RESID_COMBINE && NV == 2 && UPW == 4 && NSP == 8) return hipErrorInvalidValue;
+    else {
+    auto kern = &gemv_q80_slab_kernel<ROLE, GS, B, NV, UPW, 0, 0, NSP>;
     if (lds > 64 * 1024) (void)hipFuncSetAttribute(reinterpret_cast<const void *>(kern), hipFuncAttributeMaxDynamicSharedMemorySize, (int)lds);
     hipLaunchKernelGGL(kern, dim3(nwg), dim3(64 * p.nw), lds, st, dd);
     return hipGetLastError();
+    }
 }
 template <int ROLE, int GS, int B>
 static hipError_t launch_slab_r(const GemvDev &d, const SlabPlan &p, uint32_t rows, hipStream_t st) {
     if (p.upw > 4) return hipErrorInvalidValue;
-#define SLAB_GO(NV_, UPW_) do { if constexpr (B * NV_ <= 8) return launch_slab_t<ROLE, GS, B, NV_, UPW_>(d, p, rows, st); } while (0)
+    const uint32_t nsp = combine_nsp(d.attn_nsplit);
+#define SLAB_GO(NV_, UPW_) do { if constexpr (B * NV_ <= 8 && !(ROLE == R_RESID_COMBINE && NV_ == 4)) { \
+        if constexpr (ROLE == R_RESID_COMBINE && B == 1 && NV_ > 0) { \
+            if (nsp == 2u) return launch_slab_t<ROLE, GS, B, NV_, UPW_, 2>(d, p, rows, st); \
+            if (nsp == 4u) return launch_slab_t<ROLE, GS, B, NV_, UPW_, 4>(d, p, rows, st); \
+        } \
+        return launch_slab_t<ROLE, GS, B, NV_, UPW_>(d, p, rows, st); } } while (0)
     int nv = p.nv <= 1 ? 1 : p.nv <= 2 ? 2 : p.nv <= 4 ? 4 : 0;
     const int upw = p.upw <= 1 ? 1 : p.upw <= 2 ? 2 : 4;
     if (B * nv > 8) nv = 0;
+    if (ROLE == R_RESID_COMBINE && nv == 4) nv = 0;
+    if (ROLE == R_RESID_COMBINE && nv == 2 && upw == 4 && nsp == 8u && !(GS == 64 && d.early)) nv = 0;
     if (nv == 1) { if (upw == 1) SLAB_GO(1, 1); if (upw == 2) SLAB_GO(1, 2); SLAB_GO(1, 4); }
     if (nv == 2) { if (upw == 1) SLAB_GO(2, 1); if (upw == 2) SLAB_GO(2, 2); SLAB_GO(2, 4); }
     if (nv == 4) { if (upw == 1) SLAB_GO(4, 1); if (upw == 2) SLAB_GO(4, 2); SLAB_GO(4, 4); }
@@ -600,7 +610,7 @@
         const uint32_t f = d.flags;
         if (f == F_NORM && d.epi == GEMV_EPI_STORE) return launch_slab_r<R_NORM_STORE, GS, B>(d, p, rows, st);
         if (f == 0 && d.epi == GEMV_EPI_RESID) return launch_slab_r<R_RESID, GS, B>(d, p, rows, st);
-        if (f == F_COMBINE && d.epi == GEMV_EPI_RESID) return launch_slab_r<R_RESID_COMBINE, GS, B>(d, p, rows, st);
+        if (f == F_COMBINE && d.epi == GEMV_EPI_RESID && d.attn_hd_log2 != 0xffffffffu) return launch_slab_r<R_RESID_COMBINE, GS, B>(d, p, rows, st);
         if (f == F_NORM && d.epi == GEMV_EPI_SWIGLU) return launch_slab_r<R_NORM_SWIGLU, GS, B>(d, p, rows, st);
     }
     return launch_slab_r<R_GENERIC, GS, B>(d, p, rows, st);
@@ -645,7 +655,7 @@
 static bool wo13_shape(const GemvArgs &wo, const GemvArgs &w13, Wo13Plan &q) {
     if (wo.gs != 64 || w13.gs != 64 || wo.nb != 1 || w13.nb != 1 || !q80_canonical(wo) || !q80_canonical(w13)) return false;
     if (wo.nseg != 1 || wo.epi != GEMV_EPI_RESID || wo.norm_w || wo.xq_in || wo.tile_max || wo.resid_add || wo.seg[0].out_pstride) return false;
-    if (wo.attn_part && (wo.attn_nsplit > 8u || wo.attn_hd % 4u)) return false;
+    if (wo.attn_part && (wo.attn_nsplit > 8u || wo.attn_hd % 4u || log2_or_none(wo.attn_hd) == 0xffffffffu)) return false;
     if (w13.nseg != 2 || w13.epi != GEMV_EPI_SWIGLU || !w13.norm_w || w13.xq_in || w13.attn_part || w13.tile_max || w13.resid_add) return false;
     if (use_stream(wo) || use_stream(w13) || w13.n != wo.seg[0].rows || w13.xin != wo.seg[0].out || w13.n % 4u) return false;
     q.a = plan_slab(wo, 1); q.b = plan_slab(w13, 1);
@@ -760,12 +770,39 @@
     const size_t la = slab_lds(fa.wo), lb = slab_lds(fa.w13, !wf), lds = la > lb ? la : lb;
     if (lds > 64 * 1024) return hipErrorInvalidValue;
     const bool comb = (fa.wo.flags & F_COMBINE) != 0;
-#define WO13_GO(RA_, NVA_, UA_, NVB_, UB_, NT_) do { if (wf) hipLaunchKernelGGL((wo_w13_fused_kernel<RA_, NVA_, UA_, NVB_, UB_, NT_, 1>), dim3(q.wb), dim3(NT_), lds, st, fa); \
-                                                     else hipLaunchKernelGGL((wo_w13_fused_kernel<RA_, NVA_, UA_, NVB_, UB_, NT_>), dim3(q.wb), dim3(NT_), lds, st, fa); return hipGetLastError(); } while (0)
-    if (q.sig == 1) { if (comb) WO13_GO(R_RESID_COMBINE, 2, 1, 1, 2, 256); WO13_GO(R_RESID, 2, 1, 1, 2, 256); }
-    if (comb) WO13_GO(R_RESID_COMBINE, 1, 1, 1, 1, 512);
-    WO13_GO(R_RESID, 1, 1, 1, 1, 512);
-#undef WO13_GO
+    const uint32_t nsp = comb ? combine_nsp(fa.wo.attn_nsplit) : 8u;
+#define WO13_GO_(RA_, NVA_, UA_, NVB_, UB_, NT_, NSP_) do { if (wf) hipLaunchKernelGGL((wo_w13_fused_kernel<RA_, NVA_, UA_, NVB_, UB_, NT_, 1, NSP_>), dim3(q.wb), dim3(NT_), lds, st, fa); \
+                                                     else hipLaunchKernelGGL((wo_w13_fused_kernel<RA_, NVA_, UA_, NVB_, UB_, NT_, 0, NSP_>), dim3(q.wb), dim3(NT_), lds, st, fa); return hipGetLastError(); } while (0)
+#define WO13_COMB(NVA_, UA_, NVB_, UB_, NT_) do { if (nsp == 2u) WO13_GO_(R_RESID_COMBINE, NVA_, UA_, NVB_, UB_, NT_, 2); if (nsp == 4u) WO13_GO_(R_RESID_COMBINE, NVA_, UA_, NVB_, UB_, NT_, 4); \
+                                                  WO13_GO_(R_RESID_COMBINE, NVA_, UA_, NVB_, UB_, NT_, 8); } while (0)
+    if (q.sig == 1) { if (comb) WO13_COMB(2, 1, 1, 2, 256); WO13_GO_(R_RESID, 2, 1, 1, 2, 256, 8); }
+    if (comb) WO13_COMB(1, 1, 1, 1, 512);
+    WO13_GO_(R_RESID, 1, 1, 1, 1, 512, 8);
+#undef WO13_COMB
+#undef WO13_GO_
+}
+
+namespace {
+__global__ __launch_bounds__(256) void combine_weights_probe_kernel(const GemvDev a, float *out) {
+    extern __shared__ __attribute__((aligned(16))) unsigned char smem[];
+    float *wgt = reinterpret_cast<float *>(smem);
+    const uint32_t tid = threadIdx.x, nh = a.attn_n_head, ns = a.attn_nsplit;
+    if (nh * 8u <= a.nthr) {
+        const __amdgpu_buffer_rsrc_t rm = mkrsrc(a.attn_ml, nh * ns * 8u);
+        const uint32_t sp = tid & 7u, h = tid >> 3;
+        const uint32_t mo = (h < nh && sp < ns) ? (h * ns + sp) * 8u : OOB;
+        const float m = bload_f(rm, mo), l = bload_f(rm, mo == OOB ? OOB : mo + 4u);
+        combine_weights<1, true>(a, wgt, m, l);
+    } else combine_weights<1, false>(a, wgt, 0.0f, 0.0f);
+    for (uint32_t t = tid; t < nh * 8u; t += a.nthr) out[t] = wgt[t];
+}
+}
+hipError_t launch_combine_weights(const float *ml, uint32_t n_head, uint32_t nsplit, float *out, hipStream_t st) {
+    if (!ml || !out || !n_head || !nsplit || nsplit > 8u || (size_t)n_head * 32 > 48 * 1024) return hipErrorInvalidValue;
+    GemvDev d{};
+    d.attn_ml = ml; d.attn_n_head = n_head; d.attn_nsplit = nsplit; d.nb = 1; d.nthr = 256;
+    hipLaunchKernelGGL(combine_weights_probe_kernel, dim3(1), dim3(256), (size_t)n_head * 32, st, d, out);
+    return hipGetLastError();
 }
 #endif
 
diff --git a/nano_amd/csrc/gemv_q80_slab_body.inc b/nano_amd/csrc/gemv_q80_slab_body.inc
--- a/nano_amd/csrc/gemv_q80_slab_body.inc
+++ b/nano_amd/csrc/gemv_q80_slab_body.inc
@@ -5,6 +5,14 @@
 #ifndef SLAB_EARLY
 #define SLAB_EARLY 0
 #define SLAB_EARLY_DEFAULTED 1
+#endif
+#ifndef SLAB_NSP
+#define SLAB_NSP 8
+#define SLAB_NSP_DEFAULTED 1
+#endif
+#ifndef SLAB_XLIVE
+#define SLAB_XLIVE true
+#define SLAB_XLIVE_DEFAULTED 1
 #endif
 #ifndef SLAB_XHAND_WAIT
 #define SLAB_XHAND_WAIT 0u
@@ -68,17 +76,25 @@
     float *red = xs + B * ng4;
     float *P = red + B * 16 + (has_flag<ROLE>(SLAB_A, F_COMBINE) ? B * SLAB_A.attn_n_head * 8 : 0);
 
-    karg_touch(SLAB_A.out[0]); karg_touch(SLAB_A.out_bstride[0]); karg_touch(SLAB_A.out_pstride[0]); karg_touch(SLAB_A.rows[0]); karg_touch(SLAB_A.magic_rw); karg_touch(SLAB_A.nb);
+    karg_touch(SLAB_A.out[0]); karg_touch(SLAB_A.out_bstride[0]); karg_touch(SLAB_A.out_pstride[0]); karg_touch(SLAB_A.rows[0]); karg_touch(SLAB_A.magic_rw);
+    if (B > 1 || ROLE == R_GENERIC) karg_touch(SLAB_A.nb);
     if (!(ROLE == R_RESID || ROLE == R_RESID_COMBINE || ROLE == R_NORM_SWIGLU)) {
         karg_touch(SLAB_A.out[1]); karg_touch(SLAB_A.out[2]); karg_touch(SLAB_A.out_bstride[1]); karg_touch(SLAB_A.out_bstride[2]);
         karg_touch(SLAB_A.out_pstride[1]); karg_touch(SLAB_A.out_pstride[2]); karg_touch(SLAB_A.rows[1]); karg_touch(SLAB_A.rows[2]);
     }
-    karg_touch(SLAB_A.pos); karg_touch(SLAB_A.canon);
+    karg_touch(SLAB_A.pos); karg_touch(SLAB_A.canon); karg_touch(SLAB_A.nthr);
+    if (ROLE == R_RESID_COMBINE) karg_touch(SLAB_A.attn_hd_log2);
     if (ROLE == R_GENERIC || ROLE == R_RESID || ROLE == R_RESID_COMBINE) { karg_touch(SLAB_A.resid_add); karg_touch(SLAB_A.resid_add_bstride); }
     NANO_STAMP(SLAB_A.stamps, 0, tid);
-    Staged<B, NV> sx;
+    Staged<B, NV, SLAB_NSP> sx;
     if constexpr (SLAB_XHAND) stage_issue_nw<ROLE, B, NV>(SLAB_A, sx);
-    else if (!(NANO_STAMPS && (SLAB_A.dbg & 2u))) stage_issue<ROLE, B, NV>(SLAB_A, sx);
+    else if (!(NANO_STAMPS && (SLAB_A.dbg & 2u))) {
+#ifndef SLAB_XLIVE_DEFAULTED
+        karg_touch(SLAB_A.xin); karg_touch(SLAB_A.n);
+        if (ROLE == R_RESID_COMBINE) { karg_touch(SLAB_A.attn_part); karg_touch(SLAB_A.attn_ml); karg_touch(SLAB_A.attn_nsplit); karg_touch(SLAB_A.attn_n_head); }
+#endif
+        if (SLAB_XLIVE) stage_issue<ROLE, B, NV, B == 1>(SLAB_A, sx);
+    }
 
     constexpr bool ONESEG = ROLE == R_RESID || ROLE == R_RESID_COMBINE || ROLE == R_NORM_SWIGLU;
     const int sel = (ONESEG || swiglu) ? 0 : (int)(SLAB_BID >= SLAB_A.wg_c0) + (int)(SLAB_BID >= SLAB_A.wg_c1);
@@ -99,7 +115,7 @@
     if (!SLAB_XHAND && NANO_STAMPS && (SLAB_A.dbg & 2u)) stage_issue<ROLE, B, NV>(SLAB_A, sx);
     const int fb = (int)(((uint32_t)tid * SLAB_A.magic_rw) >> 16);
     const int frl = tid - fb * (int)RW;
-    const bool fold_live = tid < (int)(RW * B) && fb < (int)SLAB_A.nb && lrow0 + frl < rows0;
+    const bool fold_live = tid < (int)(RW * B) && (B == 1 || fb < (int)SLAB_A.nb) && lrow0 + frl < rows0;
     uint32_t opos = 0;
     if constexpr (WF_) {
         if constexpr (ROLE == R_NORM_STORE) opos = __float_as_uint(bload_f(mkrsrc(SLAB_A.pos, ops ? 4u : 0u), ((uint32_t)lane & ~3u) == (uint32_t)WF_LANE0 ? 0u : OOB));
@@ -199,7 +215,7 @@
             const uint32_t g = c * GC + (uint32_t)lane / LPG;
 #pragma unroll
             for (int b = 0; b < B; b++) {
-                if (b < (int)SLAB_A.nb) {
+                if (B == 1 || b < (int)SLAB_A.nb) {
                     const int4 xv = (col < n) ? *reinterpret_cast<const int4 *>(xq + b * n16 + col) : make_int4(0, 0, 0, 0);
                     int iv[TR];
 #pragma unroll
@@ -321,6 +337,14 @@
 #undef SLAB_EARLY
 #undef SLAB_EARLY_DEFAULTED
 #endif
+#ifdef SLAB_NSP_DEFAULTED
+#undef SLAB_NSP
+#undef SLAB_NSP_DEFAULTED
+#endif
+#ifdef SLAB_XLIVE_DEFAULTED
+#undef SLAB_XLIVE
+#undef SLAB_XLIVE_DEFAULTED
+#endif
 #ifdef SLAB_XHAND_WAIT_DEFAULTED
 #undef SLAB_XHAND_WAIT
 #undef SLAB_XHAND_NAP
diff --git a/nano_amd/csrc/kernels.h b/nano_amd/csrc/kernels.h
--- a/nano_amd/csrc/kernels.h
+++ b/nano_amd/csrc/kernels.h
@@ -146,6 +146,7 @@
 bool qkv_attn_fused_supports(const GemvArgs &ga, const AttnArgs &aa);
 hipError_t launch_qkv_attn_fused(const GemvArgs &ga, const AttnArgs &aa, unsigned long long *hand, uint32_t *tick, uint32_t layer1, hipStream_t st);
 bool wo_w13_fused_supports(const GemvArgs &wo, const GemvArgs &w13);
+hipError_t launch_combine_weights(const float *ml, uint32_t n_head, uint32_t nsplit, float *out, hipStream_t st);
 hipError_t launch_wo_w13_fused(const GemvArgs &wo, const GemvArgs &w13, unsigned long long *hand, uint32_t *tick, uint32_t layer1, hipStream_t st);
 inline bool fused_attn_side_ok(const AttnArgs &aa, uint32_t qr, uint32_t kr, uint32_t vr) {
     if (aa.hd != 128u || !aa.q_norm || !aa.k_norm || !aa.rope_qwen3 || !aa.rope_cos || !aa.rope_cur || !aa.kraw || aa.fixed_range || !aa.is_causal || aa.q_out) return false;
diff --git a/nano_amd/csrc/ops.hip b/nano_amd/csrc/ops.hip
--- a/nano_amd/csrc/ops.hip
+++ b/nano_amd/csrc/ops.hip
@@ -199,19 +199,14 @@
     return 0;
 }
 
-extern "C" int nano_hip_op_fused_gemv(int device, const NanoFusedGemvDesc *dp) {
-    int rc; if ((rc = begin(device))) return rc;
-    if (!dp) { nano_hip_set_error_("null descriptor"); return NANO_HIP_EINVAL; }
-    const NanoFusedGemvDesc &d = *dp;
+static int fused_gemv_args(const NanoFusedGemvDesc &d, DevBufs &B, GemvArgs &a, float *&dout, uint32_t &rows_total) {
     if (d.kind > 2 || d.nseg == 0 || d.nseg > 3 || (d.kind == 2 && d.nseg != 2) || d.nb == 0 || d.nb > NANO_MAX_BATCH || !d.out || d.n % 4) {
         nano_hip_set_error_("bad fused-gemv descriptor"); return NANO_HIP_EINVAL;
     }
     if (!d.x && !d.attn_part) { nano_hip_set_error_("no activation"); return NANO_HIP_EINVAL; }
     if (d.quant == NANO_QUANT_Q80 && (!(d.gs == 32 || d.gs == 64 || d.gs == 128 || d.gs == 256) || d.n % d.gs || d.n % 16)) { nano_hip_set_error_("bad n / group size"); return NANO_HIP_EINVAL; }
-    DevBufs B;
-    GemvArgs a{};
     const size_t bpl = (d.n + 255) / 256;
-    uint32_t rows_total = 0;
+    rows_total = 0;
     for (uint32_t s = 0; s < d.nseg; s++) {
         const size_t rows = d.rows[s];
         if (!d.w[s] || !rows) { nano_hip_set_error_("missing weight tensor"); return NANO_HIP_EINVAL; }
@@ -226,7 +221,7 @@
         if (d.kind != 2 || s == 0) rows_total += d.rows[s];
     }
     if (d.kind == 2 && d.rows[0] != d.rows[1]) { nano_hip_set_error_("W1 / W3 row counts differ"); return NANO_HIP_EINVAL; }
-    float *dout = B.upload(d.out, (size_t)d.nb * rows_total);
+    dout = B.upload(d.out, (size_t)d.nb * rows_total);
     OP_CHECK(dout, "device alloc failed");
     uint32_t off = 0;
     for (uint32_t s = 0; s < d.nseg; s++) {
@@ -246,6 +241,17 @@
         a.attn_nsplit = d.attn_nsplit; a.attn_n_head = d.attn_n_head; a.attn_hd = d.attn_hd;
         if (!a.xin) { a.xin = a.attn_part; a.xin_bstride = d.n; }
     }
+    return 0;
+}
+
+extern "C" int nano_hip_op_fused_gemv(int device, const NanoFusedGemvDesc *dp) {
+    int rc; if ((rc = begin(device))) return rc;
+    if (!dp) { nano_hip_set_error_("null descriptor"); return NANO_HIP_EINVAL; }
+    const NanoFusedGemvDesc &d = *dp;
+    DevBufs B;
+    GemvArgs a{};
+    float *dout = nullptr; uint32_t rows_total = 0;
+    if ((rc = fused_gemv_args(d, B, a, dout, rows_total))) return rc;
     hipDeviceProp_t prop; OP_HIP(hipGetDeviceProperties(&prop, device));
     a.cus = (uint32_t)prop.multiProcessorCount;
     a.ordered = d.ordered ? 1u : 0u;
@@ -267,6 +273,49 @@
     OP_HIP(e);
     OP_HIP(hipDeviceSynchronize());
     OP_HIP(hipMemcpy(d.out, dout, (size_t)d.nb * rows_total * 4, hipMemcpyDeviceToHost));
+    return 0;
+}
+
+extern "C" int nano_hip_op_wo_w13_fused(int device, const NanoFusedGemvDesc *wop, const NanoFusedGemvDesc *w13p) {
+    int rc; if ((rc = begin(device))) return rc;
+    if (!wop || !w13p) { nano_hip_set_error_("null descriptor"); return NANO_HIP_EINVAL; }
+    NanoFusedGemvDesc wo = *wop, w13 = *w13p;
+    if (wo.quant != NANO_QUANT_Q80 || w13.quant != NANO_QUANT_Q80 || wo.kind != 1 || w13.kind != 2 || wo.nb != 1 || w13.nb != 1 || wo.nseg != 1 || !w13.norm_w ||
+        w13.n != wo.rows[0] || w13.attn_part || wo.ordered || w13.ordered) { nano_hip_set_error_("not a Wo + W1|W3 pair"); return NANO_HIP_EINVAL; }
+    DevBufs B;
+    GemvArgs a{}, b{};
+    float *dx = nullptr, *dh = nullptr; uint32_t rows_a = 0, rows_b = 0;
+    if ((rc = fused_gemv_args(wo, B, a, dx, rows_a))) return rc;
+    w13.x = wo.out;
+    if ((rc = fused_gemv_args(w13, B, b, dh, rows_b))) return rc;
+    b.xin = dx; b.xin_bstride = w13.n;
+    hipDeviceProp_t prop; OP_HIP(hipGetDeviceProperties(&prop, device));
+    a.cus = b.cus = (uint32_t)prop.multiProcessorCount;
+    if (!wo_w13_fused_supports(a, b)) { nano_hip_set_error_("the fused Wo + W1|W3 launch does not take these shapes"); return NANO_HIP_EINVAL; }
+    unsigned long long *hand = B.alloc<unsigned long long>(w13.n);
+    uint32_t *tick = B.alloc<uint32_t>(16);
+    OP_CHECK(hand && tick, "device alloc failed");
+    const uint32_t words[16] = { 1u };
+    OP_HIP(hipMemset(hand, 0, (size_t)w13.n * 8)); OP_HIP(hipMemcpy(tick, words, sizeof words, hipMemcpyHostToDevice));
+    OP_HIP(launch_wo_w13_fused(a, b, hand, tick, 1u, 0));
+    OP_HIP(hipDeviceSynchronize());
+    uint32_t abort_word = 0;
+    OP_HIP(hipMemcpy(&abort_word, tick + 2, 4, hipMemcpyDeviceToHost));
+    OP_CHECK(!abort_word, "a W1|W3 workgroup gave up waiting for Wo's granules");
+    OP_HIP(hipMemcpy(wo.out, dx, (size_t)rows_a * 4, hipMemcpyDeviceToHost));
+    OP_HIP(hipMemcpy(w13.out, dh, (size_t)rows_b * 4, hipMemcpyDeviceToHost));
+    return 0;
+}
+
+extern "C" int nano_hip_op_combine_weights(int device, const float *ml, uint32_t n_head, uint32_t nsplit, float *out) {
+    int rc; if ((rc = begin(device))) return rc;
+    if (!ml || !out || !n_head || n_head > 512u || !nsplit || nsplit > 8u) { nano_hip_set_error_("bad combine-weights arguments"); return NANO_HIP_EINVAL; }
+    DevBufs B;
+    float *dml = B.upload(ml, (size_t)n_head * nsplit * 2), *dout = B.alloc<float>((size_t)n_head * 8);
+    OP_CHECK(dml && dout, "device alloc failed");
+    OP_HIP(launch_combine_weights(dml, n_head, nsplit, dout, 0));
+    OP_HIP(hipDeviceSynchronize());
+    OP_HIP(hipMemcpy(out, dout, (size_t)n_head * 8 * 4, hipMemcpyDeviceToHost));
     return 0;
 }
 
```
